# posgraph/coupe.DVSG

Hardware: AMD Instinct MI355X
Metric: stabilized frames/sec (1280x720 RGB) (higher is better)
Workload: dtype f32

## Files before the change

### coupe/dvsg_amd/_lib.py

```python
import ctypes
import os

_HERE = os.path.dirname(os.path.abspath(__file__))
LIB_PATH = os.environ.get("DVSG_AMD_LIB") or os.path.join(_HERE, "libdvsg_amd.so")
ABI_VERSION = 1

c_float_p = ctypes.POINTER(ctypes.c_float)
_vp = ctypes.c_void_p
_i = ctypes.c_int

SIGNATURES = {
    "dvsg_tps_solve_f32": [_vp, _vp, _i, _i, _i, _vp, _vp],
    "dvsg_tps_solve_checked_f32": [_vp, _vp, _i, _i, _i, _vp, _vp, _vp],
    "dvsg_tps_warp_f32": [_vp, _vp, _vp, _i, _i, _i, _i, _i, _i, _i, _vp, _vp, _vp, _vp],
    "dvsg_flow_warp_f32": [_vp, _vp, _i, _i, _i, _i, _vp, _vp],
    "dvsg_stn_sample_f32": [_vp, _vp, _vp, _i, _i, _i, _i, _i, _i, _vp, _vp],
    "dvsg_grid_affine_f32": [_vp, _vp, _i, _i, _i, _i, _i, _i, _vp, _vp, _vp, _vp],
    "dvsg_grid_projective_f32": [_vp, _vp, _i, _i, _i, _i, _i, _i, _vp, _vp, _vp, _vp],
    "dvsg_elastic_constants_f32": [_i, _vp, _vp],
    "dvsg_grid_elastic_f32": [_vp, _vp, _vp, _i, _vp, _i, _i, _i, _i, _i, _i, _vp, _vp, _vp, _vp],
    "dvsg_scale_rgb_f32": [_vp, _i, _i, _i, _i, _vp, _vp],
    "dvsg_locnet_create": [_i, ctypes.POINTER(ctypes.c_char_p), ctypes.POINTER(_vp),
                           ctypes.POINTER(_i), ctypes.POINTER(ctypes.c_int64), ctypes.POINTER(_vp)],
    "dvsg_locnet_destroy": [_vp],
    "dvsg_locnet_in_channels": [_vp],
    "dvsg_locnet_workspace_bytes": [_vp, _i, _i, _i, ctypes.POINTER(ctypes.c_size_t)],
    "dvsg_locnet_forward_f32": [_vp, _vp, _i, _i, _i, _vp, _vp, ctypes.c_size_t, _vp],
    "dvsg_locnet_forward_tap_f32": [_vp, _vp, _i, _i, _i, _i, _vp, ctypes.c_size_t,
                                    ctypes.POINTER(_i), _vp, ctypes.c_size_t, _vp],
    "dvsg_stabilize_f32": [_vp, _vp, _vp, _i, _i, _i, _vp, _vp, _vp, _vp, _vp, ctypes.c_size_t, _vp],
    "dvsg_locnet_forward_f32s": [_vp, _vp, _i, _i, _i, _vp, _vp, ctypes.c_size_t, _vp],
    "dvsg_locnet_forward_tap_f32s": [_vp, _vp, _i, _i, _i, _i, _vp, ctypes.c_size_t,
                                     ctypes.POINTER(_i), _vp, ctypes.c_size_t, _vp],
    "dvsg_stabilize_f32s": [_vp, _vp, _vp, _i, _i, _i, _vp, _vp, _vp, _vp, _vp, ctypes.c_size_t, _vp],
    "dvsg_conv_gemm_f32s": [_vp, _vp, _vp, _vp, _vp, _i, _i, _i, _i, _i, _i, _i, _i, _i, _vp, ctypes.c_size_t, _vp],
    "dvsg_locnet_forward_f32x3": [_vp, _vp, _i, _i, _i, _vp, _vp, ctypes.c_size_t, _vp],
    "dvsg_locnet_forward_tap_f32x3": [_vp, _vp, _i, _i, _i, _i, _vp, ctypes.c_size_t,
                                      ctypes.POINTER(_i), _vp, ctypes.c_size_t, _vp],
    "dvsg_stabilize_f32x3": [_vp, _vp, _vp, _i, _i, _i, _vp, _vp, _vp, _vp, _vp, ctypes.c_size_t, _vp],
    "dvsg_conv_gemm_f32x3": [_vp, _vp, _vp, _vp, _vp, _i, _i, _i, _i, _i, _i, _i, _i, _i, _vp, ctypes.c_size_t, _vp],
    "dvsg_pack_weights_f32x3": [_vp, _vp, _i, _i, _vp],
    "dvsg_conv3x3_1x1_f32x3": [_vp, _vp, _vp, _vp, _vp, _vp, _vp, _i, _i, _i, _i, _i, _i, _i, _vp],
    "dvsg_f32_to_pieces": [_vp, _vp, ctypes.c_size_t, _vp],
    "dvsg_pieces_to_f32": [_vp, _vp, ctypes.c_size_t, _vp],
    "dvsg_locnet_forward_f16": [_vp, _vp, _i, _i, _i, _vp, _vp, ctypes.c_size_t, _vp],
    "dvsg_locnet_forward_tap_f16": [_vp, _vp, _i, _i, _i, _i, _vp, ctypes.c_size_t,
                                    ctypes.POINTER(_i), _vp, ctypes.c_size_t, _vp],
    "dvsg_stabilize_f16": [_vp, _vp, _vp, _i, _i, _i, _vp, _vp, _vp, _vp, _vp, ctypes.c_size_t, _vp],
    "dvsg_conv_gemm_f16": [_vp, _vp, _vp, _vp, _vp, _i, _i, _i, _i, _i, _i, _i, _i, _i, _vp, ctypes.c_size_t, _vp],
    "dvsg_conv_gemm_f16s": [_vp, _vp, _vp, _vp, _vp, _i, _i, _i, _i, _i, _i, _i, _i, _i, _vp, ctypes.c_size_t, _vp],
    "dvsg_conv_gemm_f32": [_vp, _vp, _vp, _vp, _vp, _i, _i, _i, _i, _i, _i, _i, _i, _i, _vp, ctypes.c_size_t, _vp],
    "dvsg_conv3x3_1x1_f32": [_vp, _vp, _vp, _vp, _vp, _vp, _vp, _i, _i, _i, _i, _i, _i, _i, _vp],
    "dvsg_frames_u8_to_f32": [_vp, ctypes.c_size_t, _i, _vp, _vp],
    "dvsg_frames_resize_u8_f32": [_vp, _i, _i, _i, _i, _vp, _i, _i, _vp, _i, _i, _vp],
    "dvsg_window_gather_f32": [_vp, _i, _i, _i, _vp, _i, _i, _vp, _vp],
    "dvsg_stabilize_ring_f32": [_vp, _i, _vp, _i, _vp, _i, _i, _i, _vp, _vp, _vp, _vp, _vp, ctypes.c_size_t, _vp],
    "dvsg_stabilize_ring_u8": [_vp, _i, _vp, _i, _vp, _i, _i, _i, _vp, _vp, _vp, _vp, _vp, ctypes.c_size_t, _vp],
    "dvsg_locnet_forward_ring": [_vp, _i, _vp, _i, _i, _vp, _i, _i, _i, _i, _vp, ctypes.c_size_t, ctypes.POINTER(_i), _vp,
                                 ctypes.c_size_t, _vp],
    "dvsg_random_mask_plane_f32": [_vp, _i, _i, _i, _vp, _vp],
    "dvsg_stabilize_masked_f32": [_vp, _i, _vp, _vp, _vp, _i, _i, _i, _vp, _vp, _vp, _vp, _vp, ctypes.c_size_t, _vp],
    "dvsg_stabilize_ring_masked_f32": [_vp, _i, _vp, _i, _vp, _vp, _i, _i, _i, _vp, _vp, _vp, _vp, _vp, ctypes.c_size_t, _vp],
    "dvsg_stabilize_ring_masked_u8": [_vp, _i, _vp, _i, _vp, _vp, _i, _i, _i, _vp, _vp, _vp, _vp, _vp, ctypes.c_size_t, _vp],
    "dvsg_locnet_forward_masked": [_vp, _i, _vp, _i, _i, _vp, _vp, _i, _i, _i, _i, _vp, ctypes.c_size_t, ctypes.POINTER(_i),
                                   _vp, ctypes.c_size_t, _vp],
    "dvsg_frames_f32_to_u8": [_vp, _i, _i, _i, _i, _vp, _i, _i, _vp],
    "dvsg_frames_f64_to_u8": [_vp, _i, _i, _i, _i, _vp, _i, _i, _vp],
    "dvsg_debug_set_option": [ctypes.c_char_p, _i],
    "dvsg_debug_calibrate_f16_weights": [_vp, _vp, _i, _i, _i, _i, _vp, ctypes.c_size_t, _vp],
    "dvsg_locnet_calibrate_f16": [_vp, _vp, _i, _i, _i, _vp, ctypes.c_size_t, _vp],
    "dvsg_markers_enabled": [],
    "dvsg_prof_begin": [_i],
    "dvsg_prof_end": [ctypes.POINTER(ctypes.c_double), ctypes.POINTER(_i), ctypes.POINTER(ctypes.c_double),
                      ctypes.POINTER(ctypes.c_double)],
}
QUERIES = ("dvsg_abi_version", "dvsg_last_error_string", "dvsg_target_arch")

_lib = None


class DvsgError(RuntimeError):
    pass


def load():
    global _lib
    if _lib is not None:
        return _lib
    if not os.path.isfile(LIB_PATH):
        raise DvsgError(
            "libdvsg_amd.so not found at %s: build it with ./build.sh (hipcc --offload-arch=gfx950). "
            "coupe.dvsg_amd has no CPU or PyTorch fallback." % LIB_PATH)
    lib = ctypes.CDLL(LIB_PATH)
    lib.dvsg_abi_version.restype = ctypes.c_int
    lib.dvsg_last_error_string.restype = ctypes.c_char_p
    lib.dvsg_target_arch.restype = ctypes.c_char_p
    if lib.dvsg_abi_version() != ABI_VERSION:
        raise DvsgError("libdvsg_amd.so ABI %d != expected %d" % (lib.dvsg_abi_version(), ABI_VERSION))
    for name, argtypes in SIGNATURES.items():
        fn = getattr(lib, name)
        fn.argtypes = argtypes
        fn.restype = ctypes.c_int
    _lib = lib
    for env, opt in (("DVSG_CONV_VARIANT", b"conv_variant"), ("DVSG_FUSE_CONV", b"fuse_conv"),
                     ("DVSG_F16_SPLIT", b"f16_split"), ("DVSG_FUSE_SHORTCUT", b"fuse_shortcut"),
                     ("DVSG_CONV1_VARIANT", b"conv1_variant"), ("DVSG_F16_PAIR_MASK", b"f16_pair_mask"),
                     ("DVSG_WIDE16_PACKED", b"wide16_packed"), ("DVSG_WIDE16_AROWS", b"wide16_arows"),
                     ("DVSG_WIDE16_HREUSE", b"wide16_hreuse"), ("DVSG_FUSED_HREUSE", b"fused_hreuse"),
                     ("DVSG_CONCAT_SC", b"concat_sc"), ("DVSG_FLOW_TILED", b"flow_tiled")):
        if os.environ.get(env) and os.environ.get("DVSG_DEBUG") == "1":
            check(lib.dvsg_debug_set_option(opt, int(os.environ[env])), "dvsg_debug_set_option")
    return lib


def check(status, what):
    if status != 0:
        msg = load().dvsg_last_error_string().decode("utf-8", "replace")
        raise DvsgError("%s failed (status %d): %s" % (what, status, msg))


def call(name, *args):
    check(getattr(load(), name)(*args), name)
```

### coupe/dvsg_amd/csrc/cnn_kernels.h

```cpp
#pragma once
#include "common.h"

namespace dvsg {

enum Precision { kF32 = 0, kF16 = 1, kF32S = 2, kF32X = 3 };
inline size_t elem_size(int prec) { return prec == kF16 ? 2 : 4; }

struct ConvGemm {
  int prec;
  const void *x;
  const void *wt;
  const float *bias;
  const void *res;
  void *y;
  int B, H, W, Cin, Ho, Wo, Cout;
  int ksize, stride, pad;
  int res_H, res_W, res_stride;
  int relu;
  int ldx = 0, res_ld = 0, relu_from = -1;
  const void *wt_packed = nullptr;
  const void *wt_packed_a = nullptr;
  const void *wt_packed_h = nullptr;
  int x3 = 0;
  int wsplit = 0;
  void *splitk_scratch = nullptr;
  size_t splitk_scratch_bytes = 0;
  int *splitk_counters = nullptr;
};
constexpr int kSplitKMaxTiles = 512;
constexpr size_t kSplitKSlabBytes = (size_t)512 * 2 * 128 * 128 * 4;
int launch_conv_gemm(const ConvGemm &p, hipStream_t s);
inline size_t x3_packed_bytes(int rows, int K) { return (size_t)rows * K * 6; }
int launch_pack_x3(const float *wt, void *out, int rows, int K, hipStream_t s);
int launch_conv_wide16(const ConvGemm &p, hipStream_t s);
void set_wide16_min_tiles(int v);
size_t wide16_packed_bytes(int rows, int Cin, int ksize);
int launch_pack_wide16(const void *wt, void *out, int rows, int Cin, int ksize, int order, hipStream_t s);
void set_wide16_arows(int v);
void set_wide16_hreuse(int v);
void set_wide16_packed(int v);
int launch_zero_tickets(int *tickets, size_t n, hipStream_t s);
struct ConvFused {
  const float *x;
  const float *wt2;
  const float *bias2;
  const float *wt3;
  const float *bias3;
  const float *res;
  float *y;
  int B, H, W, Cin, Ho, Wo, Cout;
  int stride;
  int res_H, res_W, res_stride;
  const float *sc_x = nullptr;
  const float *sc_wt = nullptr;
  const float *sc_bias = nullptr;
  int sc_cin = 0;
  int pieces = 0;
  int f16 = 0;
  int x3 = 0;
};
int launch_conv3x3_1x1_x3(const ConvFused &p, hipStream_t s);
bool conv_fusable(int prec, int Cin, int Cmid, int Cout, int ksize);
int launch_conv3x3_1x1(const ConvFused &p, hipStream_t s);
void set_fuse_conv(int v);
int get_fuse_conv();
void set_fused_hreuse(int v);
void set_conv_variant(int v);
void set_conv1_variant(int v);

constexpr int kConv1Cin = 21;
constexpr int kConv1K = 7 * kConv1Cin;
constexpr int kConv1Kpad = 148;
constexpr int kConv1Ld = 150;
constexpr int kConv1LdH = 168;
constexpr int kConv1X3Ld = 88;
constexpr int kConv1X3StageElems = 3 * 64 * kConv1X3Ld;
enum Conv1SrcKind { kSrcWindow = 0, kSrcRingF32 = 1, kSrcRingU8 = 2 };
struct Conv1Src {
  const void *base;
  const int *table;
  int n_pool;
  const float *mask = nullptr;
};
int launch_conv1(int out_prec, const Conv1Src &src, int src_kind, const float *wt1, const void *wt1h, const void *wt1s,
                 const void *wt1x, const float *bias, void *y, int B, int H, int W, int Ho, int Wo, hipStream_t s);

int launch_maxpool(int prec, const void *x, void *y, int B, int H, int W, int C, int Ho, int Wo, int pad_top,
                   int pad_left, hipStream_t s);

constexpr int kPoolSplits = 8;
int launch_avgpool_partial(int prec, const void *x, float *part, int B, int HW, int C, hipStream_t s);

int launch_f16_to_f32(const void *x, float *y, size_t n, hipStream_t s);
int launch_p_to_f32(const void *x, float *y, size_t n, hipStream_t s);
int launch_f32_to_p(const float *x, void *y, size_t n, hipStream_t s);

constexpr int kDenseSplits = 8;
int launch_dense(const float *xin, int s_in, const float *bias_in, float scale_in, int lrelu_in,
                 const float *W, float *out_part, int B, int K, int N, hipStream_t s);
int launch_dense_finalize(const float *part, int s_in, float scale, const float *bias, float *out, int B,
                          int N, hipStream_t s);

}
```

### coupe/dvsg_amd/csrc/conv1_pool.hip

```cpp
#include <cstdint>
#include <type_traits>

#include "cnn_device.h"
#include "cnn_kernels.h"

namespace dvsg {
namespace {

constexpr int C1_TILE = 128;
constexpr int C1_SEG_PAD = 5488;
constexpr int C1_WELEMS = 64 * kConv1Ld;
constexpr int C1_LDC = 68;

template <int NT, int GROUPS, bool ALIGNED, bool MASKED = false>
struct Conv1Row {
  static constexpr bool kRing = false;
  typedef float floatx4_u __attribute__((ext_vector_type(4), aligned(4)));
  floatx4 nmean[GROUPS];
  long idx[GROUPS];
  unsigned col_ok, full;
  bool fast;
  struct Data {
    floatx4 reg[GROUPS];
    float m0[MASKED ? GROUPS : 1], m1[MASKED ? GROUPS : 1];
    bool row_ok;
  };
  const float *img;
  long row_elems;
  int H;
  const float *mplane;
  int mW;
  int mcol0[MASKED ? GROUPS : 1], mcol1[MASKED ? GROUPS : 1];
  unsigned m_first, m_second;

  __device__ __forceinline__ void init(const Conv1Src &src, int tid, int b, int wo0, int H_, int W, int seg_elems) {
    H = H_;
    row_elems = (long)W * kConv1Cin;
    img = static_cast<const float *>(src.base) + (long)b * H * row_elems;
    const long seg0 = (long)(2 * wo0 - 3) * kConv1Cin - 1;
    col_ok = full = 0;
    if constexpr (MASKED) {
      mplane = src.mask + (long)b * H * W;
      mW = W;
      m_first = m_second = 0;
    }
    bool mine = true;
#pragma unroll
    for (int i = 0; i < GROUPS; ++i) {
      const int e0 = 4 * (tid + NT * i);
      unsigned m = 0;
      if constexpr (MASKED) {
        const long ge0 = seg0 + e0;
        const int c0 = (int)(ge0 >= 0 ? ge0 / kConv1Cin : -((-ge0 + kConv1Cin - 1) / kConv1Cin));
        mcol0[i] = c0 < 0 ? 0 : (c0 >= W ? W - 1 : c0);
        mcol1[i] = c0 + 1 < 0 ? 0 : (c0 + 1 >= W ? W - 1 : c0 + 1);
#pragma unroll
        for (int j = 0; j < 4; ++j) {
          const long ge = ge0 + j;
          if (ge < 0 || ge >= row_elems) continue;
          const int col = (int)(ge / kConv1Cin), ch = (int)(ge - (long)col * kConv1Cin);
          if (ch >= kConv1Cin - 3) continue;
          if (col == c0) m_first |= 1u << (4 * i + j); else m_second |= 1u << (4 * i + j);
        }
      }
#pragma unroll
      for (int j = 0; j < 4; ++j) {
        const int e = e0 + j;
        const long ge = seg0 + e;
        const int g = ((e + kConv1Cin - 1) % kConv1Cin) / (kConv1Cin / 3);
        nmean[i][j] = g == 0 ? -123.68f : (g == 1 ? -116.779f : -103.939f);
        if (e < seg_elems && ge >= 0 && ge < row_elems) m |= 1u << j;
        if (e < seg_elems && !(ge >= 0 && ge < row_elems)) mine = false;
      }
      col_ok |= m << (4 * i);
      if (m == 15u) full |= 1u << i;
      idx[i] = (ALIGNED && m != 15u) ? 0 : seg0 + e0;
    }
    fast = ALIGNED && __builtin_amdgcn_ballot_w64(!mine) == 0;
  }
  __device__ __forceinline__ void load(Data &d, int hi) const {
    d.row_ok = hi >= 0 && hi < H;
    const int hc = hi < 0 ? 0 : (hi >= H ? H - 1 : hi);
    const float *xrow = img + (long)hc * row_elems;
    if constexpr (MASKED) {
      const float *mrow = mplane + (long)hc * mW;
#pragma unroll
      for (int i = 0; i < GROUPS; ++i) {
        d.m0[i] = mrow[mcol0[i]];
        d.m1[i] = mrow[mcol1[i]];
      }
    }
#pragma unroll
    for (int i = 0; i < GROUPS; ++i) {
      if constexpr (ALIGNED) {
        d.reg[i] = *reinterpret_cast<const floatx4 *>(xrow + idx[i]);
      } else if ((full >> i) & 1u) {
        d.reg[i] = *reinterpret_cast<const floatx4_u *>(xrow + idx[i]);
      } else {
#pragma unroll
        for (int j = 0; j < 4; ++j) d.reg[i][j] = ((col_ok >> (4 * i + j)) & 1u) ? xrow[idx[i] + j] : 0.f;
      }
    }
  }
  __device__ __forceinline__ floatx4 scaled(const Data &d, int i) const {
    floatx4 x = d.reg[i];
    if constexpr (MASKED) {
      floatx4 m4;
#pragma unroll
      for (int j = 0; j < 4; ++j)
        m4[j] = ((m_first >> (4 * i + j)) & 1u) ? d.m0[i] : (((m_second >> (4 * i + j)) & 1u) ? d.m1[i] : 1.0f);
      x = x * m4;
    }
    if (fast) {
      if (!d.row_ok) return floatx4{0.f, 0.f, 0.f, 0.f};
      return x * 255.0f + nmean[i];
    }
    const unsigned ok = d.row_ok ? col_ok : 0u;
    floatx4 v;
#pragma unroll
    for (int j = 0; j < 4; ++j) v[j] = ((ok >> (4 * i + j)) & 1u) ? x[j] * 255.0f + nmean[i][j] : 0.f;
    return v;
  }
};

constexpr int C1_RING_PX = 2 * (C1_TILE - 1) + 7;
constexpr int C1_RING_RG = (3 * (C1_RING_PX + 1) + 3) / 4;
constexpr int C1_RING_GROUPS = 7 * C1_RING_RG;

template <int NT, int GROUPS, typename TS, bool ALIGNED, bool MASKED = false>
struct Conv1RingRow {
  static constexpr bool kRing = true;
  static constexpr bool kU8 = sizeof(TS) == 1;
  static_assert(NT * GROUPS >= C1_RING_GROUPS, "not enough threads x groups for 7 frame runs");
  static_assert(GROUPS <= 8, "per-element masks are 32 bits wide");
  typedef float floatx4_u __attribute__((ext_vector_type(4), aligned(4)));
  floatx4 nmean[GROUPS];
  bool fast;
  long off[GROUPS];
  int l0[GROUPS];
  unsigned phase;
  unsigned col_ok, st_ok;
  unsigned no_frame;
  struct Data {
    floatx4 regf[kU8 ? 1 : GROUPS];
    unsigned regu[kU8 ? GROUPS : 1];
    float m0[MASKED ? GROUPS : 1], m1[MASKED ? GROUPS : 1];
    bool row_ok;
  };
  const TS *pool;
  long row_elems;
  int H;
  const float *mplane;
// ... 18 lines not shown
    for (int i = 0; i < GROUPS; ++i) {
      const int q = tid + NT * i;
      const int f = q / C1_RING_RG, g = q - f * C1_RING_RG;
      const bool in_range = q < C1_RING_GROUPS;
      const int fi = in_range ? src.table[b * 7 + f] : -1;
      const bool frame_ok = fi >= 0 && fi < src.n_pool;
      const long r0 = r_first + 4 * g;
      unsigned mc = 0, ms = 0;
      if constexpr (MASKED) {
        const int c0 = (int)(r0 >= 0 ? r0 / 3 : -((-r0 + 2) / 3));
        mcol0[i] = c0 < 0 ? 0 : (c0 >= W ? W - 1 : c0);
        mcol1[i] = c0 + 1 < 0 ? 0 : (c0 + 1 >= W ? W - 1 : c0 + 1);
        if (in_range && f < 6) {
#pragma unroll
          for (int j = 0; j < 4; ++j) {
            const long r = r0 + j;
            if (r < 0 || r >= row_elems) continue;
            if ((int)(r / 3) == c0) m_first |= 1u << (4 * i + j); else m_second |= 1u << (4 * i + j);
          }
        }
      }
#pragma unroll
      for (int j = 0; j < 4; ++j) {
        const int t = 4 * g + j;
        const int c = 3 * f + t % 3;
        const int grp = c / (kConv1Cin / 3);
        nmean[i][j] = grp == 0 ? -123.68f : (grp == 1 ? -116.779f : -103.939f);
        if (in_range && t >= 3 && t < 3 * (C1_RING_PX + 1)) ms |= 1u << j;
        if (in_range && r0 + j >= 0 && r0 + j < row_elems) mc |= 1u << j;
      }
      if (in_range && !frame_ok) no_frame |= 1u << i;
      if ((ms & ~mc) != 0 || (in_range && !frame_ok)) mine = false;
      const bool whole = mc == 15u;
      if (ALIGNED && !whole) mc = 0;
      col_ok |= mc << (4 * i);
      st_ok |= ms << (4 * i);
      off[i] = (ALIGNED && !whole) ? 0 : (frame_ok ? (long)fi * frame_elems : 0) + r0;
      l0[i] = 1 + kConv1Cin * ((4 * g) / 3 - 1) + 3 * f;
      phase |= (unsigned)((4 * g) % 3) << (2 * i);
    }
    fast = __builtin_amdgcn_ballot_w64(!mine) == 0;
  }
  __device__ __forceinline__ void load(Data &d, int hi) const {
    d.row_ok = hi >= 0 && hi < H;
    const int hc = hi < 0 ? 0 : (hi >= H ? H - 1 : hi);
    const long roff = (long)hc * row_elems;
    if constexpr (MASKED) {
      const float *mrow = mplane + (long)hc * mW;
#pragma unroll
      for (int i = 0; i < GROUPS; ++i) {
        d.m0[i] = mrow[mcol0[i]];
        d.m1[i] = mrow[mcol1[i]];
      }
    }
#pragma unroll
    for (int i = 0; i < GROUPS; ++i) {
      const TS *p = pool + off[i] + roff;
      if constexpr (kU8) {
        if constexpr (ALIGNED) {
          d.regu[i] = *reinterpret_cast<const unsigned *>(p);
        } else {
          unsigned w = 0;
#pragma unroll
          for (int j = 0; j < 4; ++j)
            if ((col_ok >> (4 * i + j)) & 1u) w |= (unsigned)p[j] << (8 * j);
          d.regu[i] = w;
        }
      } else {
        if constexpr (ALIGNED) {
          d.regf[i] = *reinterpret_cast<const floatx4 *>(p);
        } else if (((col_ok >> (4 * i)) & 15u) == 15u) {
          d.regf[i] = *reinterpret_cast<const floatx4_u *>(p);
        } else {
#pragma unroll
          for (int j = 0; j < 4; ++j) d.regf[i][j] = ((col_ok >> (4 * i + j)) & 1u) ? (float)p[j] : 0.f;
        }
      }
    }
  }
  template <typename PUT>
  __device__ __forceinline__ void scatter(const Data &d, PUT put) const {
    const unsigned ok = d.row_ok ? col_ok : 0u;
    const bool plain = fast && d.row_ok;
#pragma unroll
    for (int i = 0; i < GROUPS; ++i) {
      const int ph = (phase >> (2 * i)) & 3u;
      floatx4 raw4;
      if constexpr (MASKED) {
        floatx4 m4, x;
#pragma unroll
        for (int j = 0; j < 4; ++j)
          m4[j] = ((m_first >> (4 * i + j)) & 1u) ? d.m0[i] : (((m_second >> (4 * i + j)) & 1u) ? d.m1[i] : 1.0f);
        if constexpr (kU8) {
#pragma unroll
          for (int j = 0; j < 4; ++j) {
            const float v = (float)((d.regu[i] >> (8 * j)) & 255u);
            const float q = v * (1.0f / 255.0f);
            x[j] = __builtin_fmaf(__builtin_fmaf(-q, 255.0f, v), 1.0f / 255.0f, q);
          }
        } else {
          x = d.regf[i];
        }
        raw4 = (x * m4) * 255.0f;
      } else if constexpr (kU8) {
#pragma unroll
        for (int j = 0; j < 4; ++j) raw4[j] = (float)((d.regu[i] >> (8 * j)) & 255u);
      } else {
        raw4 = d.regf[i] * 255.0f;
      }
      const floatx4 sc4 = raw4 + nmean[i];
#pragma unroll
      for (int j = 0; j < 4; ++j) {
        float v;
        if (plain) {
          v = sc4[j];
        } else {
          const float raw = ((no_frame >> i) & 1u) ? 0.f : raw4[j];
          v = ((ok >> (4 * i + j)) & 1u) ? raw + nmean[i][j] : 0.f;
        }
        const int t = ph + j, step = t / 3;
        if ((st_ok >> (4 * i + j)) & 1u) put(l0[i] + kConv1Cin * step + (t - 3 * step), v);
      }
    }
  }
};

template <int NT, int GROUPS, int SRC>
struct Conv1RowSel {
  static_assert((SRC & 6) == 0, "ring sources are specialised below");
  typedef Conv1Row<NT, GROUPS, (SRC & 1) != 0, (SRC & 8) != 0> type;
};
template <int NT, int GROUPS>
struct Conv1RowSel<NT, GROUPS, 10> { typedef Conv1RingRow<NT, (C1_RING_GROUPS + NT - 1) / NT, float, false, true> type; };
template <int NT, int GROUPS>
struct Conv1RowSel<NT, GROUPS, 11> { typedef Conv1RingRow<NT, (C1_RING_GROUPS + NT - 1) / NT, float, true, true> type; };
template <int NT, int GROUPS>
struct Conv1RowSel<NT, GROUPS, 12> { typedef Conv1RingRow<NT, (C1_RING_GROUPS + NT - 1) / NT, uint8_t, false, true> type; };
template <int NT, int GROUPS>
struct Conv1RowSel<NT, GROUPS, 13> { typedef Conv1RingRow<NT, (C1_RING_GROUPS + NT - 1) / NT, uint8_t, true, true> type; };
template <int NT, int GROUPS>
struct Conv1RowSel<NT, GROUPS, 2> { typedef Conv1RingRow<NT, (C1_RING_GROUPS + NT - 1) / NT, float, false> type; };
template <int NT, int GROUPS>
struct Conv1RowSel<NT, GROUPS, 3> { typedef Conv1RingRow<NT, (C1_RING_GROUPS + NT - 1) / NT, float, true> type; };
template <int NT, int GROUPS>
struct Conv1RowSel<NT, GROUPS, 4> { typedef Conv1RingRow<NT, (C1_RING_GROUPS + NT - 1) / NT, uint8_t, false> type; };
template <int NT, int GROUPS>
struct Conv1RowSel<NT, GROUPS, 5> { typedef Conv1RingRow<NT, (C1_RING_GROUPS + NT - 1) / NT, uint8_t, true> type; };

#ifdef DVSG_STAMPS
__device__ unsigned long long g_c1_stamps[8 * 65536];
#define C1_STAMP() __builtin_amdgcn_s_memtime()
#endif

template <int NW, typename TO, int SRC>
__global__ __launch_bounds__(64 * NW) __attribute__((amdgpu_waves_per_eu(NW / 2, NW / 2)))
void conv1_kernel(const Conv1Src src, const float *__restrict__ wt1, const float *__restrict__ bias,
                  TO *__restrict__ y, int H, int W, int Ho, int Wo, int wtiles) {
  constexpr int NT = 64 * NW;
  constexpr int MI = 4 / (NW / 2);
  constexpr int IN4 = (C1_SEG_PAD / 4 + NT - 1) / NT;
  constexpr int WLOADS = (C1_WELEMS / 4 + NT - 1) / NT;
  static_assert(C1_TILE * C1_LDC <= C1_WELEMS, "epilogue tile must fit in the weight stage");
  __shared__ __attribute__((aligned(16))) float w_s[C1_WELEMS];
  __shared__ __attribute__((aligned(16))) float in_s[C1_SEG_PAD];
  const int tid = threadIdx.x;
  const int lane = tid & 63, wave = tid >> 6;
  const int wm = wave >> 1, wn = wave & 1;
  const int r = lane & 31, h = lane >> 5;

  int blk = xcd_remap(blockIdx.x, gridDim.x);
  const int wt_i = blk % wtiles;
  blk /= wtiles;
  const int ho = blk % Ho;
  const int b = blk / Ho;
  const int wo0 = wt_i * C1_TILE;

  typedef typename Conv1RowSel<NT, IN4, SRC>::type Row;
  Row row;
  row.init(src, tid, b, wo0, H, W, C1_SEG_PAD);
  if constexpr (Row::kRing) {
    for (int e = tid; e < C1_SEG_PAD; e += NT) in_s[e] = 0.f;
  }
  typename Row::Data rd;
  floatx4 w_reg[WLOADS];
  auto load_stage = [&](int kh) __attribute__((always_inline)) {
    row.load(rd, 2 * ho + kh - 3);
    const floatx4 *wsrc = reinterpret_cast<const floatx4 *>(wt1 + (size_t)kh * C1_WELEMS);
#pragma unroll
    for (int i = 0; i < WLOADS; ++i) {
      const int q = tid + NT * i;
      w_reg[i] = wsrc[q < C1_WELEMS / 4 ? q : 0];
    }
  };
  auto store_stage = [&]() __attribute__((always_inline)) {
    if constexpr (Row::kRing) {
      row.scatter(rd, [&](int e, float v) __attribute__((always_inline)) { in_s[e] = v; });
    } else {
#pragma unroll
      for (int i = 0; i < IN4; ++i) {
        const int q = tid + NT * i;
        const floatx4 v = row.scaled(rd, i);
        if (q < C1_SEG_PAD / 4) reinterpret_cast<floatx4 *>(in_s)[q] = v;
      }
    }
#pragma unroll
    for (int i = 0; i < WLOADS; ++i) {
      const int q = tid + NT * i;
      if (q < C1_WELEMS / 4) reinterpret_cast<floatx4 *>(w_s)[q] = w_reg[i];
    }
  };

  floatx16 acc[MI];
#pragma unroll
  for (int mi = 0; mi < MI; ++mi)
#pragma unroll
    for (int q = 0; q < 16; ++q) acc[mi][q] = 0.f;

#ifdef DVSG_STAMPS
  unsigned long long st[8] = {0, 0, 0, 0, 0, 0, 0, 0};
  const unsigned long long t_begin = C1_STAMP(), r_begin = __builtin_amdgcn_s_memrealtime();
#endif
  load_stage(0);
#ifdef DVSG_STAMPS
  st[0] = C1_STAMP() - t_begin;
#endif
  for (int kh = 0; kh < 7; ++kh) {
#ifdef DVSG_STAMPS
    const unsigned long long s0 = C1_STAMP();
    __syncthreads();
    const unsigned long long s1 = C1_STAMP();
    store_stage();
    const unsigned long long s2 = C1_STAMP();
    __syncthreads();
    const unsigned long long s3 = C1_STAMP();
    if (kh + 1 < 7) load_stage(kh + 1);
    const unsigned long long s4 = C1_STAMP();
    st[1] += s1 - s0;
    st[2] += s2 - s1;
    st[3] += s3 - s2;
    st[4] += s4 - s3;
#else
    __syncthreads();
    store_stage();
    __syncthreads();
    if (kh + 1 < 7) load_stage(kh + 1);
#endif
    __builtin_amdgcn_sched_barrier(0);
    const float *a0 = in_s + 2 * kConv1Cin * (wm * 32 * MI + r) + 2 * h;
    const float *bp = w_s + (wn * 32 + r) * kConv1Ld + 2 * h;
    constexpr int STEPS = kConv1Kpad / 4, PAIRS = (STEPS + 1) / 2;
    float2 va[2][2][MI], vb[2][2];
    auto read_pair = [&](int slot, int g) __attribute__((always_inline)) {
#pragma unroll
      for (int j = 0; j < 2; ++j) {
        if (2 * g + j >= STEPS) break;
#pragma unroll
        for (int mi = 0; mi < MI; ++mi)
          va[slot][j][mi] = *reinterpret_cast<const float2 *>(a0 + mi * (2 * kConv1Cin * 32) + 4 * (2 * g + j));
        vb[slot][j] = *reinterpret_cast<const float2 *>(bp + 4 * (2 * g + j));
      }
    };
    read_pair(0, 0);
#pragma unroll
    for (int g = 0; g < PAIRS; ++g) {
      if (g + 1 < PAIRS) read_pair((g + 1) & 1, g + 1);
      __builtin_amdgcn_sched_barrier(0);
#pragma unroll
      for (int j = 0; j < 2; ++j) {
        if (2 * g + j >= STEPS) break;
#pragma unroll
        for (int mi = 0; mi < MI; ++mi) acc[mi] = mfma32(va[g & 1][j][mi].x, vb[g & 1][j].x, acc[mi]);
#pragma unroll
        for (int mi = 0; mi < MI; ++mi) acc[mi] = mfma32(va[g & 1][j][mi].y, vb[g & 1][j].y, acc[mi]);
      }
      __builtin_amdgcn_sched_barrier(0);
    }
  }

#ifdef DVSG_STAMPS
  const unsigned long long t_loop_end = C1_STAMP();
#endif
  float *Cs = w_s;
  __syncthreads();
#pragma unroll
  for (int mi = 0; mi < MI; ++mi)
#pragma unroll
    for (int q = 0; q < 16; ++q)
      Cs[(wm * 32 * MI + mi * 32 + (q & 3) + 8 * (q >> 2) + 4 * h) * C1_LDC + wn * 32 + r] = acc[mi][q];
  __syncthreads();
  const int col4 = tid & 15, row0 = tid >> 4;
  const float4 b4 = *reinterpret_cast<const float4 *>(bias + 4 * col4);
  TO *yrow = y + (((size_t)b * Ho + ho) * Wo + wo0) * 64 + 4 * col4;
#pragma unroll 4
  for (int row = row0; row < C1_TILE; row += NT / 16) {
    if (wo0 + row >= Wo) break;
    float4 v = *reinterpret_cast<const float4 *>(Cs + row * C1_LDC + 4 * col4);
    v.x = fmaxf(v.x + b4.x, 0.f);
    v.y = fmaxf(v.y + b4.y, 0.f);
    v.z = fmaxf(v.z + b4.z, 0.f);
    v.w = fmaxf(v.w + b4.w, 0.f);
    store4(yrow + (size_t)row * 64, v);
  }
#ifdef DVSG_STAMPS
  if (tid == 0 && blockIdx.x < 65536) {
    unsigned long long *o = g_c1_stamps + (size_t)blockIdx.x * 8;
    const unsigned long long t_end = C1_STAMP();
    o[0] = st[0]; o[1] = st[1]; o[2] = st[2]; o[3] = st[3]; o[4] = st[4];
    o[5] = t_loop_end - t_begin;
    o[6] = t_end - t_begin;
    o[7] = __builtin_amdgcn_s_memrealtime() - r_begin;
  }
#endif
}

template <typename T>
__global__ __launch_bounds__(256) void maxpool_kernel(const T *__restrict__ x, T *__restrict__ y, int H, int W,
                                                     int C4, int Ho, int Wo, int pad_top, int pad_left,
                                                     size_t total) {
  {
    const size_t e = (size_t)xcd_remap(blockIdx.x, gridDim.x) * 256 + threadIdx.x;
    if (e >= total) return;
    const int c4 = (int)(e % C4);
    size_t t = e / C4;
    const int wo = (int)(t % Wo);
    t /= Wo;
    const int ho = (int)(t % Ho);
    const size_t b = t / Ho;
    float4 m = make_float4(-INFINITY, -INFINITY, -INFINITY, -INFINITY);
#pragma unroll
    for (int i = 0; i < 3; ++i) {
      const int hi = 2 * ho - pad_top + i;
      if (hi < 0 || hi >= H) continue;
#pragma unroll
      for (int j = 0; j < 3; ++j) {
        const int wi = 2 * wo - pad_left + j;
        if (wi < 0 || wi >= W) continue;
        const float4 v = load4(x + (((b * H + hi) * W + wi) * C4 + c4) * 4);
        m.x = fmaxf(m.x, v.x);
        m.y = fmaxf(m.y, v.y);
        m.z = fmaxf(m.z, v.z);
        m.w = fmaxf(m.w, v.w);
      }
    }
    store4(y + e * 4, m);
  }
}

__global__ __launch_bounds__(256) void maxpool_h8_kernel(const _Float16 *__restrict__ x, _Float16 *__restrict__ y, int H,
                                                         int W, int C8, int Ho, int Wo, int pad_top, int pad_left,
                                                         size_t total) {
  const size_t e = (size_t)xcd_remap(blockIdx.x, gridDim.x) * 256 + threadIdx.x;
  if (e >= total) return;
  const int c8 = (int)(e % C8);
  size_t t = e / C8;
  const int wo = (int)(t % Wo);
  t /= Wo;
  const int ho = (int)(t % Ho);
  const size_t b = t / Ho;
  halfx8 m;
#pragma unroll
  for (int q = 0; q < 8; ++q) m[q] = (_Float16)(-INFINITY);
#pragma unroll
  for (int i = 0; i < 3; ++i) {
    const int hi = 2 * ho - pad_top + i;
    if (hi < 0 || hi >= H) continue;
#pragma unroll
    for (int j = 0; j < 3; ++j) {
      const int wi = 2 * wo - pad_left + j;
      if (wi < 0 || wi >= W) continue;
      const halfx8 v = *reinterpret_cast<const halfx8 *>(x + (((b * H + hi) * W + wi) * C8 + c8) * 8);
#pragma unroll
      for (int q = 0; q < 8; ++q) m[q] = v[q] > m[q] ? v[q] : m[q];
    }
  }
  *reinterpret_cast<halfx8 *>(y + e * 8) = m;
}

constexpr int C1H_STEPS = 10;
constexpr int C1H_LD = 168;
constexpr int C1H_WBYTES = 64 * C1H_LD * 2;
constexpr int C1H_SEG = 5504;
constexpr int C1H_IN4 = (C1H_SEG / 4 + 255) / 256;

template <typename TO, int SRC>
__global__ __launch_bounds__(256) __attribute__((amdgpu_waves_per_eu(2, 2)))
void conv1_f16_kernel(const Conv1Src src, const _Float16 *__restrict__ wt1h, const float *__restrict__ bias,
                      TO *__restrict__ y, int H, int W, int Ho, int Wo, int wtiles) {
  static_assert(C1_TILE * C1_LDC * 4 <= 2 * C1H_WBYTES, "epilogue tile must fit in the weight stages");
  __shared__ __attribute__((aligned(16))) char lds[2 * C1H_WBYTES + 2 * C1H_SEG * 2];
  char *w_s = lds;
  char *in_s = lds + 2 * C1H_WBYTES;
  const int tid = threadIdx.x;
  const int lane = tid & 63, wave = tid >> 6;
  const int r = lane & 31, h = lane >> 5;

  int blk = xcd_remap(blockIdx.x, gridDim.x);
  const int wt_i = blk % wtiles;
  blk /= wtiles;
  const int ho = blk % Ho;
  const int b = blk / Ho;
  const int wo0 = wt_i * C1_TILE;

  typedef typename Conv1RowSel<256, C1H_IN4, SRC>::type Row;
  Row row;
  row.init(src, tid, b, wo0, H, W, C1H_SEG);
  if constexpr (Row::kRing) {
    for (int e = tid; e < C1H_SEG; e += 256) reinterpret_cast<unsigned *>(in_s)[e] = 0u;
    __syncthreads();
  }

  typedef const __attribute__((address_space(1))) void *gptr_t;
  typedef __attribute__((address_space(3))) void *lptr_t;
  typename Row::Data rd;
  auto load_stage = [&](int kh, int buf) __attribute__((always_inline)) {
    const char *wsrc = reinterpret_cast<const char *>(wt1h) + (size_t)kh * C1H_WBYTES;
    for (int j = wave; j < C1H_WBYTES / 1024; j += 4)
      __builtin_amdgcn_global_load_lds((gptr_t)(wsrc + j * 1024 + lane * 16), (lptr_t)(w_s + buf * C1H_WBYTES + j * 1024),
                                       16, 0, 0);
    row.load(rd, 2 * ho + kh - 3);
  };
  auto store_stage = [&](int buf) __attribute__((always_inline)) {
    typedef _Float16 half4_t __attribute__((ext_vector_type(4)));
    if constexpr (Row::kRing) {
      _Float16 *dsth = reinterpret_cast<_Float16 *>(in_s + buf * C1H_SEG * 2);
      row.scatter(rd, [&](int e, float v) __attribute__((always_inline)) { dsth[e] = (_Float16)v; });
    } else {
      half4_t *dst = reinterpret_cast<half4_t *>(in_s + buf * C1H_SEG * 2);
#pragma unroll
      for (int i = 0; i < C1H_IN4; ++i) {
        const int q = tid + 256 * i;
        const floatx4 v = row.scaled(rd, i);
        half4_t hv;
#pragma unroll
        for (int j = 0; j < 4; ++j) hv[j] = (_Float16)v[j];
        if (q < C1H_SEG / 4) dst[q] = hv;
      }
    }
  };

  floatx16 acc[2];
#pragma unroll
  for (int ni = 0; ni < 2; ++ni)
#pragma unroll
    for (int q = 0; q < 16; ++q) acc[ni][q] = 0.f;
// ... 845 lines not shown
    v.z = fmaxf(v.z + b4.z, 0.f);
    v.w = fmaxf(v.w + b4.w, 0.f);
    store4(y + (((size_t)b * Ho + ho) * Wo + wo0 + row) * 64 + 4 * col4, v);
  }
}

__global__ __launch_bounds__(256) void maxpool_p_kernel(const void *__restrict__ x, void *__restrict__ y, int H, int W,
                                                       int C4, int Ho, int Wo, int pad_top, int pad_left, size_t total) {
  const size_t e = (size_t)xcd_remap(blockIdx.x, gridDim.x) * 256 + threadIdx.x;
  if (e >= total) return;
  const int c4 = (int)(e % C4);
  size_t t = e / C4;
  const int wo = (int)(t % Wo);
  t /= Wo;
  const int ho = (int)(t % Ho);
  const size_t b = t / Ho;
  float4 m = make_float4(-INFINITY, -INFINITY, -INFINITY, -INFINITY);
#pragma unroll
  for (int i = 0; i < 3; ++i) {
    const int hi = 2 * ho - pad_top + i;
    if (hi < 0 || hi >= H) continue;
#pragma unroll
    for (int j = 0; j < 3; ++j) {
      const int wi = 2 * wo - pad_left + j;
      if (wi < 0 || wi >= W) continue;
      const float4 v = load4_p(x, (((b * H + hi) * W + wi) * C4 + c4) * 4);
      m.x = fmaxf(m.x, v.x);
      m.y = fmaxf(m.y, v.y);
      m.z = fmaxf(m.z, v.z);
      m.w = fmaxf(m.w, v.w);
    }
  }
  store4_p(y, e * 4, m);
}

int march_bands(int B, int Ho, int wtiles, int *quads_per_band) {
  const int quads = (Ho + C1M_QUAD - 1) / C1M_QUAD;
  const long cols = (long)B * wtiles;
  for (int qpb = 8; qpb >= 4; --qpb) {
    const int bands = (quads + qpb - 1) / qpb;
    if (cols * bands >= 3 * 256) {
      if (quads_per_band) *quads_per_band = qpb;
      return bands;
    }
  }
  return 0;
}

int g_conv1_variant = 0;

}

void set_conv1_variant(int v) { g_conv1_variant = v; }

int launch_conv1(int out_prec, const Conv1Src &src, int src_kind, const float *wt1, const void *wt1h, const void *wt1s,
                 const void *wt1x, const float *bias, void *y, int B, int H, int W, int Ho, int Wo, hipStream_t s) {
  const int wtiles = ceil_div(Wo, C1_TILE);
  const long blocks = (long)wtiles * Ho * B;
  DVSG_REQUIRE(blocks > 0 && blocks < (1L << 31), "conv1: grid of %ld workgroups out of range", blocks);
  DVSG_REQUIRE((long)W * kConv1Cin < (1L << 31), "conv1: input row too long");
  DVSG_REQUIRE(src_kind == kSrcWindow || (src.table && src.n_pool > 0), "conv1: a frame ring needs its index table");
  const double in_bytes = src_kind == kSrcRingU8 ? 1.0 : 4.0;
  ProfScope prof(kClsConv1, s, 2.0 * (double)B * Ho * Wo * 64 * 49 * kConv1Cin,
                 in_bytes * (double)B * H * W * kConv1Cin + (double)elem_size(out_prec) * B * Ho * Wo * 64);
  const dim3 grid((unsigned)blocks);
  const bool aligned = W % 4 == 0 && reinterpret_cast<uintptr_t>(src.base) % (src_kind == kSrcRingU8 ? 4 : 16) == 0;
  const int SRC = 2 * src_kind + (aligned ? 1 : 0) + (src.mask ? 8 : 0);
  if (out_prec == kF32S && !wt1s) return fail(DVSG_ERR_UNSUPPORTED, "conv1: the f32s precision needs the piece weights");
#define DVSG_K_F32(SRC) conv1_kernel<4, float, SRC>
#define DVSG_K_F16(SRC) conv1_f16_kernel<_Float16, (SRC) & 7>
#define DVSG_K_SPLIT(SRC) conv1_split_kernel<float, SRC>
#define DVSG_K_X3(SRC) conv1_x3_kernel<SRC>
#define DVSG_C1(KERNEL, NTHREADS, WPTR, YPTR)                                                                            \
  do {                                                                                                                   \
    switch (SRC) {                                                                                                       \
      case 0: hipLaunchKernelGGL((KERNEL(0)), grid, dim3(NTHREADS), 0, s, src, WPTR, bias, YPTR, H, W, Ho, Wo, wtiles); break; \
      case 1: hipLaunchKernelGGL((KERNEL(1)), grid, dim3(NTHREADS), 0, s, src, WPTR, bias, YPTR, H, W, Ho, Wo, wtiles); break; \
      case 2: hipLaunchKernelGGL((KERNEL(2)), grid, dim3(NTHREADS), 0, s, src, WPTR, bias, YPTR, H, W, Ho, Wo, wtiles); break; \
      case 3: hipLaunchKernelGGL((KERNEL(3)), grid, dim3(NTHREADS), 0, s, src, WPTR, bias, YPTR, H, W, Ho, Wo, wtiles); break; \
      case 4: hipLaunchKernelGGL((KERNEL(4)), grid, dim3(NTHREADS), 0, s, src, WPTR, bias, YPTR, H, W, Ho, Wo, wtiles); break; \
      case 5: hipLaunchKernelGGL((KERNEL(5)), grid, dim3(NTHREADS), 0, s, src, WPTR, bias, YPTR, H, W, Ho, Wo, wtiles); break; \
      case 8: hipLaunchKernelGGL((KERNEL(8)), grid, dim3(NTHREADS), 0, s, src, WPTR, bias, YPTR, H, W, Ho, Wo, wtiles); break; \
      case 9: hipLaunchKernelGGL((KERNEL(9)), grid, dim3(NTHREADS), 0, s, src, WPTR, bias, YPTR, H, W, Ho, Wo, wtiles); break; \
      case 10: hipLaunchKernelGGL((KERNEL(10)), grid, dim3(NTHREADS), 0, s, src, WPTR, bias, YPTR, H, W, Ho, Wo, wtiles); break; \
      case 11: hipLaunchKernelGGL((KERNEL(11)), grid, dim3(NTHREADS), 0, s, src, WPTR, bias, YPTR, H, W, Ho, Wo, wtiles); break; \
      case 12: hipLaunchKernelGGL((KERNEL(12)), grid, dim3(NTHREADS), 0, s, src, WPTR, bias, YPTR, H, W, Ho, Wo, wtiles); break; \
      default: hipLaunchKernelGGL((KERNEL(13)), grid, dim3(NTHREADS), 0, s, src, WPTR, bias, YPTR, H, W, Ho, Wo, wtiles); break; \
    }                                                                                                                    \
  } while (0)
  if (out_prec == kF32X && !wt1x) return fail(DVSG_ERR_UNSUPPORTED, "conv1: the f32x3 precision needs the bfloat16 piece weights");
  if (out_prec == kF32X) {
    DVSG_C1(DVSG_K_X3, 256, static_cast<const unsigned short *>(wt1x), static_cast<float *>(y));
  } else if (out_prec == kF32S) {
    DVSG_C1(DVSG_K_SPLIT, 256, static_cast<const _Float16 *>(wt1s), static_cast<float *>(y));
  } else if (out_prec == kF16 && wt1h && g_conv1_variant == 3 && !src.mask) {
    DVSG_C1(DVSG_K_F16, 256, static_cast<const _Float16 *>(wt1h), static_cast<_Float16 *>(y));
  } else if (out_prec == kF16 && wt1h && g_conv1_variant != 2 && g_conv1_variant != 4 && !src.mask &&
             (g_conv1_variant == 5 || march_bands(B, Ho, wtiles, nullptr) > 0)) {
    int qpb = 0;
    int bands = march_bands(B, Ho, wtiles, &qpb);
    if (g_conv1_variant == 5) {
      qpb = 3;
      bands = ((Ho + C1M_QUAD - 1) / C1M_QUAD + qpb - 1) / qpb;
    }
    const dim3 mgrid((unsigned)((long)wtiles * bands * B));
    const _Float16 *wp = static_cast<const _Float16 *>(wt1h);
    _Float16 *yp = static_cast<_Float16 *>(y);
    switch (SRC) {
      case 0: hipLaunchKernelGGL((conv1_f16_march_kernel<0>), mgrid, dim3(512), 0, s, src, wp, bias, yp, H, W, Ho, Wo, wtiles, bands, qpb); break;
      case 1: hipLaunchKernelGGL((conv1_f16_march_kernel<1>), mgrid, dim3(512), 0, s, src, wp, bias, yp, H, W, Ho, Wo, wtiles, bands, qpb); break;
      case 2: hipLaunchKernelGGL((conv1_f16_march_kernel<2>), mgrid, dim3(512), 0, s, src, wp, bias, yp, H, W, Ho, Wo, wtiles, bands, qpb); break;
      case 3: hipLaunchKernelGGL((conv1_f16_march_kernel<3>), mgrid, dim3(512), 0, s, src, wp, bias, yp, H, W, Ho, Wo, wtiles, bands, qpb); break;
      case 4: hipLaunchKernelGGL((conv1_f16_march_kernel<4>), mgrid, dim3(512), 0, s, src, wp, bias, yp, H, W, Ho, Wo, wtiles, bands, qpb); break;
      default: hipLaunchKernelGGL((conv1_f16_march_kernel<5>), mgrid, dim3(512), 0, s, src, wp, bias, yp, H, W, Ho, Wo, wtiles, bands, qpb); break;
    }
  } else if (out_prec == kF16 && wt1h && g_conv1_variant != 2) {
    const int hpairs = (Ho + 1) / 2;
    const long pblocks = (long)wtiles * hpairs * B;
    const dim3 pgrid((unsigned)pblocks);
    const _Float16 *wp = static_cast<const _Float16 *>(wt1h);
    _Float16 *yp = static_cast<_Float16 *>(y);
    switch (SRC) {
      case 0: hipLaunchKernelGGL((conv1_f16_pair_kernel<_Float16, 0>), pgrid, dim3(256), 0, s, src, wp, bias, yp, H, W, Ho, Wo, wtiles, hpairs); break;
      case 1: hipLaunchKernelGGL((conv1_f16_pair_kernel<_Float16, 1>), pgrid, dim3(256), 0, s, src, wp, bias, yp, H, W, Ho, Wo, wtiles, hpairs); break;
      case 2: hipLaunchKernelGGL((conv1_f16_pair_kernel<_Float16, 2>), pgrid, dim3(256), 0, s, src, wp, bias, yp, H, W, Ho, Wo, wtiles, hpairs); break;
      case 3: hipLaunchKernelGGL((conv1_f16_pair_kernel<_Float16, 3>), pgrid, dim3(256), 0, s, src, wp, bias, yp, H, W, Ho, Wo, wtiles, hpairs); break;
      case 4: hipLaunchKernelGGL((conv1_f16_pair_kernel<_Float16, 4>), pgrid, dim3(256), 0, s, src, wp, bias, yp, H, W, Ho, Wo, wtiles, hpairs); break;
      case 5: hipLaunchKernelGGL((conv1_f16_pair_kernel<_Float16, 5>), pgrid, dim3(256), 0, s, src, wp, bias, yp, H, W, Ho, Wo, wtiles, hpairs); break;
      case 8: hipLaunchKernelGGL((conv1_f16_pair_kernel<_Float16, 8>), pgrid, dim3(256), 0, s, src, wp, bias, yp, H, W, Ho, Wo, wtiles, hpairs); break;
      case 9: hipLaunchKernelGGL((conv1_f16_pair_kernel<_Float16, 9>), pgrid, dim3(256), 0, s, src, wp, bias, yp, H, W, Ho, Wo, wtiles, hpairs); break;
      case 10: hipLaunchKernelGGL((conv1_f16_pair_kernel<_Float16, 10>), pgrid, dim3(256), 0, s, src, wp, bias, yp, H, W, Ho, Wo, wtiles, hpairs); break;
      case 11: hipLaunchKernelGGL((conv1_f16_pair_kernel<_Float16, 11>), pgrid, dim3(256), 0, s, src, wp, bias, yp, H, W, Ho, Wo, wtiles, hpairs); break;
      case 12: hipLaunchKernelGGL((conv1_f16_pair_kernel<_Float16, 12>), pgrid, dim3(256), 0, s, src, wp, bias, yp, H, W, Ho, Wo, wtiles, hpairs); break;
      default: hipLaunchKernelGGL((conv1_f16_pair_kernel<_Float16, 13>), pgrid, dim3(256), 0, s, src, wp, bias, yp, H, W, Ho, Wo, wtiles, hpairs); break;
    }
  } else if (out_prec == kF16) {
    DVSG_REQUIRE(src_kind == kSrcWindow && !src.mask, "conv1: conv1_variant 2 takes an unmasked window tensor");
    hipLaunchKernelGGL((conv1_kernel<4, _Float16, 0>), grid, dim3(256), 0, s, src, wt1, bias, static_cast<_Float16 *>(y), H, W,
                       Ho, Wo, wtiles);
  } else if (g_conv1_variant != 0 && src_kind == kSrcWindow && !src.mask) {
    hipLaunchKernelGGL((conv1_kernel<8, float, 0>), grid, dim3(512), 0, s, src, wt1, bias, static_cast<float *>(y), H, W, Ho,
                       Wo, wtiles);
  } else {
    DVSG_C1(DVSG_K_F32, 256, wt1, static_cast<float *>(y));
  }
#undef DVSG_C1
#undef DVSG_K_F32
#undef DVSG_K_F16
#undef DVSG_K_SPLIT
#undef DVSG_K_X3
  return check_launch("conv1_kernel");
}

#ifdef DVSG_STAMPS
extern "C" int dvsg_debug_read_conv1_stamps(void *host, size_t bytes) {
  return hipMemcpyFromSymbol(host, HIP_SYMBOL(g_c1_stamps), bytes) == hipSuccess ? 0 : -3;
}
#endif

int launch_maxpool(int prec, const void *x, void *y, int B, int H, int W, int C, int Ho, int Wo, int pad_top,
                   int pad_left, hipStream_t s) {
  DVSG_REQUIRE(C % 4 == 0 && (prec != kF32S || C % 32 == 0), "maxpool: C=%d must be a multiple of 4 (32 in the f32s format)", C);
  const size_t total = (size_t)B * Ho * Wo * (C / 4);
  const size_t want = (total + 255) / 256;
  DVSG_REQUIRE(want < (1u << 31), "maxpool: %zu blocks do not fit a grid", want);
  const int blocks = (int)want;
  ProfScope prof(kClsMaxpool, s, 0.0, (double)elem_size(prec) * C * ((double)B * H * W + (double)B * Ho * Wo));
  if (prec == kF32S)
    hipLaunchKernelGGL(maxpool_p_kernel, dim3(blocks), dim3(256), 0, s, x, y, H, W, C / 4, Ho, Wo, pad_top, pad_left, total);
  else if (prec == kF16 && C % 8 == 0) {
    const size_t total8 = total / 2;
    hipLaunchKernelGGL(maxpool_h8_kernel, dim3((unsigned)((total8 + 255) / 256)), dim3(256), 0, s, static_cast<const _Float16 *>(x),
                       static_cast<_Float16 *>(y), H, W, C / 8, Ho, Wo, pad_top, pad_left, total8);
  } else if (prec == kF16)
    hipLaunchKernelGGL(maxpool_kernel<_Float16>, dim3(blocks), dim3(256), 0, s, static_cast<const _Float16 *>(x),
                       static_cast<_Float16 *>(y), H, W, C / 4, Ho, Wo, pad_top, pad_left, total);
  else
    hipLaunchKernelGGL(maxpool_kernel<float>, dim3(blocks), dim3(256), 0, s, static_cast<const float *>(x),
                       static_cast<float *>(y), H, W, C / 4, Ho, Wo, pad_top, pad_left, total);
  return check_launch("maxpool_kernel");
}

}
```

### coupe/dvsg_amd/csrc/conv_fused.hip

```cpp
#include <algorithm>

#include "cnn_device.h"
#include "cnn_kernels.h"

#include <type_traits>

namespace dvsg {
namespace {

constexpr int BM = 128;
constexpr int ROWB = 128;
constexpr int CMID = 64;

__device__ const floatx4 g_zero16f = {0.f, 0.f, 0.f, 0.f};

struct ConvFusedDev {
  const float *x;
  const float *wt2;
  const float *bias2;
  const float *wt3;
  const float *bias3;
  const float *res;
  const float *wts;
  const float *biass;
// ... 161 lines not shown
  floatx16 &acc1 = acc1v[0];
#pragma unroll
  for (int q = 0; q < 16; ++q) acc1[q] = 0.f;
  auto compute_stage = [&](int buf) __attribute__((always_inline)) {
    const char *a_base = As + (buf * BM + wm * 32 + r) * ROWB;
    const char *b_base = Bs + (buf * CMID + wn * 32 + r) * ROWB;
    stage_mma<PS, 1>(a_base, b_base, sw, h, acc1v);
  };
  auto w3_issue = [&](int half, int s2) __attribute__((always_inline)) {
#pragma unroll
    for (int i = 0; i < 2; ++i) {
      const int row = 8 * (wave + NW * i) + lrow8;
      const float *src = p.wt3 + (size_t)(128 * half + row) * CMID + 32 * s2 + 4 * (lpos ^ ((row >> 1) & 7));
      __builtin_amdgcn_global_load_lds((gptr_t)src, (lptr_t)(lds + (s2 == 0 ? 49152 : 32768) + 8 * (wave + NW * i) * ROWB),
                                       16, 0, 0);
    }
  };
  issue_stage(0);
  issue_stage(1);
  asm volatile("s_waitcnt vmcnt(%0)" ::"n"(AG + 1) : "memory");
  __builtin_amdgcn_s_barrier();
  asm volatile("" ::: "memory");
  __builtin_amdgcn_sched_barrier(0);
  compute_stage(0);
  __builtin_amdgcn_sched_barrier(0);
  for (int kt = 1; kt < KT - 1; ++kt) {
    __syncthreads();
    issue_stage((kt + 1) & 1);
    __builtin_amdgcn_sched_barrier(0);
    compute_stage(kt & 1);
    __builtin_amdgcn_sched_barrier(0);
  }
  __syncthreads();
  w3_issue(0, 0);
  __builtin_amdgcn_sched_barrier(0);
  compute_stage((KT - 1) & 1);

  const float bmid = p.bias2[32 * wn + r];
  __syncthreads();
#pragma unroll
  for (int q = 0; q < 16; ++q) {
    const int R = wm * 32 + (q & 3) + 8 * (q >> 2) + 4 * h;
    const float v = fmaxf(acc1[q] + bmid, 0.f);
    if (PS) {
      const _Float16 hi = (_Float16)v, lo = (_Float16)(v - (float)hi);
      char *row = lds + (wn * BM + R) * ROWB + 2 * (r & 7);
      *reinterpret_cast<_Float16 *>(row + 16 * ((r >> 3) ^ ((R >> 1) & 7))) = hi;
      *reinterpret_cast<_Float16 *>(row + 16 * ((4 + (r >> 3)) ^ ((R >> 1) & 7))) = lo;
    } else {
      *reinterpret_cast<float *>(lds + (wn * BM + R) * ROWB + 16 * ((r >> 2) ^ ((R >> 1) & 7)) + 4 * (r & 3)) = v;
    }
  }
  w3_issue(0, 1);

  float *Cs = reinterpret_cast<float *>(lds + 32768);
  const int col4 = tid & 31, row0 = tid >> 5;
  auto lds_barrier = [&]() __attribute__((always_inline)) {
    asm volatile("s_waitcnt lgkmcnt(0)" ::: "memory");
    __builtin_amdgcn_s_barrier();
    asm volatile("" ::: "memory");
  };
  auto compute2 = [&](int s2, floatx16 (&acc2)[2]) __attribute__((always_inline)) {
    const char *a_base = lds + (s2 * BM + wm * 32 + r) * ROWB;
    const char *b_base = lds + (s2 == 0 ? 49152 : 32768) + (wn * 64 + r) * ROWB;
    stage_mma<PS, 2>(a_base, b_base, sw, h, acc2);
  };
  const int nhalves = p.Cout / 128;
  auto do_half = [&](int half, floatx16 (&acc2)[2]) __attribute__((always_inline)) {
    asm volatile("s_waitcnt vmcnt(2) lgkmcnt(0)" ::: "memory");
    __builtin_amdgcn_s_barrier();
    asm volatile("" ::: "memory");
    compute2(0, acc2);
    __syncthreads();
    compute2(1, acc2);
    const int n = 128 * half + 4 * col4;
    float4 bias4 = *reinterpret_cast<const float4 *>(p.bias3 + n);
    if (RES == 3) {
      const float4 bs = *reinterpret_cast<const float4 *>(p.biass + n);
      bias4.x += bs.x; bias4.y += bs.y; bias4.z += bs.z; bias4.w += bs.w;
    }
#pragma unroll
    for (int rho = 0; rho < 2; ++rho) {
      float4 rv[4];
      if (RES != 3) {
#pragma unroll
        for (int i = 0; i < 4; ++i) {
          const int mr = m0 + 64 * rho + row0 + 16 * i;
          const int m = mr < p.M ? mr : p.M - 1;
          size_t roff;
          if (RES == 1) {
            roff = (size_t)m * p.Cout + n;
          } else {
            const int wo = m % p.Wo;
            const int t = m / p.Wo;
            const int ho = t % p.Ho;
            const int b = t / p.Ho;
            roff = (((size_t)b * p.res_H + (size_t)ho * p.res_stride) * p.res_W + (size_t)wo * p.res_stride) * p.Cout + n;
          }
          rv[i] = PS ? load4_p_pair(p.res, roff, col4 & 1) : load4(p.res + roff);
        }
      }
      lds_barrier();
      if ((wm >> 1) == rho) {
#pragma unroll
        for (int ni = 0; ni < 2; ++ni)
#pragma unroll
          for (int q = 0; q < 16; ++q)
            Cs[((wm & 1) * 32 + (q & 3) + 8 * (q >> 2) + 4 * h) * 128 + wn * 64 + ni * 32 + r] = acc2[ni][q];
      }
      lds_barrier();
#pragma unroll
      for (int i = 0; i < 4; ++i) {
        const int row = row0 + 16 * i;
        const int m = m0 + 64 * rho + row;
        if (m < p.M) {
          float4 v = *reinterpret_cast<const float4 *>(Cs + row * 128 + 4 * col4);
          if (RES == 3) {
            v.x = fmaxf(v.x + bias4.x, 0.f);
            v.y = fmaxf(v.y + bias4.y, 0.f);
            v.z = fmaxf(v.z + bias4.z, 0.f);
            v.w = fmaxf(v.w + bias4.w, 0.f);
          } else {
            v.x = fmaxf(v.x + bias4.x + rv[i].x, 0.f);
            v.y = fmaxf(v.y + bias4.y + rv[i].y, 0.f);
            v.z = fmaxf(v.z + bias4.z + rv[i].z, 0.f);
            v.w = fmaxf(v.w + bias4.w + rv[i].w, 0.f);
          }
          if (PS) store4_p_pair(p.y, (size_t)m * p.Cout + n, v, col4 & 1, true);
          else store4(p.y + (size_t)m * p.Cout + n, v);
        }
      }
    }
    if (half + 1 < nhalves) {
      lds_barrier();
      w3_issue(half + 1, 0);
      w3_issue(half + 1, 1);
    }
  };
  if (RES == 3) {
    do_half(0, acc_sc[0]);
    do_half(1, acc_sc[1]);
  } else {
    for (int half = 0; half < nhalves; ++half) {
      floatx16 acc2[2];
#pragma unroll
      for (int ni = 0; ni < 2; ++ni)
#pragma unroll
        for (int q = 0; q < 16; ++q) acc2[ni][q] = 0.f;
      do_half(half, acc2);
    }
  }
}

struct ConvFusedF16Dev {
  const _Float16 *x;
  const _Float16 *wt2;
  const float *bias2;
  const _Float16 *wt3;
  const float *bias3;
  const _Float16 *res;
  const _Float16 *wts;
  const float *biass;
  _Float16 *y;
  int H, W, Cin, Ho, Wo, Cout;
  int stride;
  int res_H, res_W, res_stride;
  int M, mtiles;
};

template <int RES>
__global__ __launch_bounds__(512) __attribute__((amdgpu_waves_per_eu(4, 4)))
void conv3x3_1x1_f16_kernel(ConvFusedF16Dev p) {
  constexpr int NW = 8;
  constexpr float kLoScale = 1.0f / 2048.0f;
  __shared__ __attribute__((aligned(16))) char lds[65536];
  char *As = lds;
  char *Bs = lds + 32768;
  const int tid = threadIdx.x;
  const int lane = tid & 63, wave = tid >> 6;
  const int wm = wave >> 1, wn = wave & 1;
  const int r = lane & 31, h = lane >> 5;
  const int lrow8 = lane >> 3, lpos = lane & 7;
  const int sw = (r >> 1) & 7;
  const int K1 = 9 * p.Cin;
  const int KT = K1 / 64;

  typedef const __attribute__((address_space(1))) void *gptr_t;
  typedef __attribute__((address_space(3))) void *lptr_t;

  const int m0 = xcd_remap(blockIdx.x, p.mtiles) * BM;

  long a_off[2];
  unsigned a_mask[2];
  const _Float16 *wsrc[2];
#pragma unroll
  for (int i = 0; i < 2; ++i) {
    const int row = 8 * (wave + NW * i) + lrow8;
    const int chunk = lpos ^ ((row >> 1) & 7);
    const int m = m0 + row;
    const int mm = m < p.M ? m : 0;
    const int wo = mm % p.Wo;
    const int t = mm / p.Wo;
    const int ho = t % p.Ho;
    const int b = t / p.Ho;
    const int hi0 = ho * p.stride - 1, wi0 = wo * p.stride - 1;
    a_off[i] = (((long)b * p.H + hi0) * p.W + wi0) * p.Cin + 8 * chunk;
    unsigned mk = 0;
    if (m < p.M) {
#pragma unroll
      for (int q = 0; q < 3; ++q) {
        if (hi0 + q >= 0 && hi0 + q < p.H) mk |= 1u << q;
        if (wi0 + q >= 0 && wi0 + q < p.W) mk |= 16u << q;
      }
    }
    a_mask[i] = mk;
    wsrc[i] = p.wt2 + (size_t)row * K1 + 8 * chunk;
  }
  int s_kh = 0, s_kw = 0, s_c0 = 0;
  auto issue_stage = [&](int buf) __attribute__((always_inline)) {
    const _Float16 *xa = p.x + ((long)s_kh * p.W + s_kw) * p.Cin + s_c0;
    const int wk = (s_kh * 3 + s_kw) * p.Cin + s_c0;
#pragma unroll
    for (int i = 0; i < 2; ++i) {
      const bool ok = ((a_mask[i] >> s_kh) & (a_mask[i] >> (4 + s_kw)) & 1u) != 0;
      const void *src = ok ? static_cast<const void *>(xa + a_off[i]) : static_cast<const void *>(&g_zero16f);
      __builtin_amdgcn_global_load_lds((gptr_t)src, (lptr_t)(As + (buf * BM + 8 * (wave + NW * i)) * ROWB), 16, 0, 0);
    }
#pragma unroll
    for (int i = 0; i < 2; ++i)
      __builtin_amdgcn_global_load_lds((gptr_t)(wsrc[i] + wk), (lptr_t)(Bs + (buf * 128 + 8 * (wave + NW * i)) * ROWB), 16, 0, 0);
    if (++s_kw == 3) {
      s_kw = 0;
      if (++s_kh == 3) {
        s_kh = 0;
        s_c0 += 64;
      }
    }
  };
  floatx16 acc_hi, acc_lo;
#pragma unroll
  for (int q = 0; q < 16; ++q) acc_hi[q] = acc_lo[q] = 0.f;
  auto mma_stage = [&](const char *a_row, const char *b_row) __attribute__((always_inline)) {
#pragma unroll
    for (int kb = 0; kb < 4; ++kb) {
      const int co = 16 * ((2 * kb + h) ^ sw);
      const halfx8 a = *reinterpret_cast<const halfx8 *>(a_row + co);
      const halfx8 bh = *reinterpret_cast<const halfx8 *>(b_row + co);
      const halfx8 bl = *reinterpret_cast<const halfx8 *>(b_row + 64 * ROWB + co);
      acc_hi = __builtin_amdgcn_mfma_f32_32x32x16_f16(a, bh, acc_hi, 0, 0, 0);
      acc_lo = __builtin_amdgcn_mfma_f32_32x32x16_f16(a, bl, acc_lo, 0, 0, 0);
    }
  };
  auto compute_stage = [&](int buf) __attribute__((always_inline)) {
    mma_stage(As + (buf * BM + wm * 32 + r) * ROWB, Bs + (buf * 128 + wn * 32 + r) * ROWB);
  };
  auto issue_rows = [&](const _Float16 *src, size_t row_elems, int dst, bool by_pixel) __attribute__((always_inline)) {
#pragma unroll
    for (int i = 0; i < 2; ++i) {
      const int row = 8 * (wave + NW * i) + lrow8;
      size_t rr = row;
      if (by_pixel) rr = m0 + row < p.M ? m0 + row : p.M - 1;
      __builtin_amdgcn_global_load_lds((gptr_t)(src + rr * row_elems + 8 * (lpos ^ ((row >> 1) & 7))),
                                       (lptr_t)(lds + dst + 8 * (wave + NW * i) * ROWB), 16, 0, 0);
    }
  };
  issue_stage(0);
  issue_stage(1);
  asm volatile("s_waitcnt vmcnt(4)" ::: "memory");
  __builtin_amdgcn_s_barrier();
  asm volatile("" ::: "memory");
  __builtin_amdgcn_sched_barrier(0);
  compute_stage(0);
  __builtin_amdgcn_sched_barrier(0);
  for (int kt = 1; kt < KT - 1; ++kt) {
    __syncthreads();
    issue_stage((kt + 1) & 1);
    __builtin_amdgcn_sched_barrier(0);
    compute_stage(kt & 1);
    __builtin_amdgcn_sched_barrier(0);
  }
  __syncthreads();
  const int last = (KT - 1) & 1;
  if (RES == 3) {
    issue_rows(p.res, 64, last == 0 ? 16384 : 0, true);
    issue_rows(p.wts, 64, last == 0 ? 49152 : 32768, false);
  }
  __builtin_amdgcn_sched_barrier(0);
  compute_stage(last);

  const float bmid = p.bias2[32 * wn + r];
  __syncthreads();
  const int T2 = last == 0 ? 0 : 16384, SX = last == 0 ? 16384 : 0;
  const int W3 = last == 0 ? 32768 : 49152, WS = last == 0 ? 49152 : 32768;
  issue_rows(p.wt3, 64, W3, false);
#pragma unroll
  for (int q = 0; q < 16; ++q) {
    const int R = wm * 32 + (q & 3) + 8 * (q >> 2) + 4 * h;
    const int k2 = 32 * wn + r;
    const float v = fmaxf(acc_hi[q] + acc_lo[q] * kLoScale + bmid, 0.f);
    *reinterpret_cast<_Float16 *>(lds + T2 + R * ROWB + 16 * ((k2 >> 3) ^ ((R >> 1) & 7)) + 2 * (k2 & 7)) = (_Float16)v;
  }

  float *Cs = reinterpret_cast<float *>(lds + 32768);
  const int col4 = tid & 15, row0 = tid >> 4;
  const int ngroups = p.Cout / 64;
  for (int g = 0; g < ngroups; ++g) {
// ... 158 lines not shown
      const halfx8 bh = *reinterpret_cast<const halfx8 *>(b_row + 16 * ((2 * kb + h) ^ swb));
      const halfx8 bl = *reinterpret_cast<const halfx8 *>(b_row + 64 * ROWB + 16 * ((2 * kb + h) ^ swb));
      acc_hi = __builtin_amdgcn_mfma_f32_32x32x16_f16(a, bh, acc_hi, 0, 0, 0);
      acc_lo = __builtin_amdgcn_mfma_f32_32x32x16_f16(a, bl, acc_lo, 0, 0, 0);
    }
  };

  issue_a(0, A0);
  issue_q(0);
  issue_q(1);
  auto tap_stage = [&](auto T) __attribute__((always_inline)) {
    constexpr int t = decltype(T)::value;
    constexpr int kh = t / 3, kw = t % 3;
    if (t == 1 || t == 4 || (RES == 3 && t == 7)) asm volatile("s_waitcnt vmcnt(4) lgkmcnt(0)" ::: "memory");
    else asm volatile("s_waitcnt vmcnt(2) lgkmcnt(0)" ::: "memory");
    __builtin_amdgcn_s_barrier();
    asm volatile("" ::: "memory");
    if (kw == 0 && kh < 2) issue_a(kh + 1, (kh + 1) & 1 ? A1 : A0);
    if (RES == 3 && t == 6) {
#pragma unroll
      for (int i = 0; i < 2; ++i) {
        const int row = 8 * (wave + NW * i) + lrow8;
        const int mr = m0 + row;
        const int m = mr < 0 ? 0 : (mr < p.M ? mr : p.M - 1);
        __builtin_amdgcn_global_load_lds((gptr_t)(p.res + (size_t)m * CSC + 8 * (lpos ^ ((row >> 1) & 7))),
                                         (lptr_t)(lds + A1 + 8 * (wave + NW * i) * ROWB), 16, 0, 0);
      }
    }
    issue_q(t + 2);
    __builtin_amdgcn_sched_barrier(0);
    mma_tap(kh & 1 ? A1 : A0, kw, t % 3);
    __builtin_amdgcn_sched_barrier(0);
  };
  tap_stage(std::integral_constant<int, 0>{});
  tap_stage(std::integral_constant<int, 1>{});
  tap_stage(std::integral_constant<int, 2>{});
  tap_stage(std::integral_constant<int, 3>{});
  tap_stage(std::integral_constant<int, 4>{});
  tap_stage(std::integral_constant<int, 5>{});
  tap_stage(std::integral_constant<int, 6>{});
  tap_stage(std::integral_constant<int, 7>{});
  tap_stage(std::integral_constant<int, 8>{});

  const float bmid = p.bias2[32 * wn + r];
  asm volatile("s_waitcnt lgkmcnt(0)" ::: "memory");
  __builtin_amdgcn_s_barrier();
  asm volatile("" ::: "memory");
#pragma unroll
  for (int q = 0; q < 16; ++q) {
    const int R = wm * 32 + (q & 3) + 8 * (q >> 2) + 4 * h;
    const int k2 = 32 * wn + r;
    const float v = fmaxf(acc_hi[q] + acc_lo[q] * kLoScale + bmid, 0.f);
    *reinterpret_cast<_Float16 *>(lds + A0 + R * ROWB + 16 * ((k2 >> 3) ^ ((R >> 1) & 7)) + 2 * (k2 & 7)) = (_Float16)v;
  }

  float *Cs = reinterpret_cast<float *>(lds + (RES == 1 ? A1 : RING + 2 * SLOT));
  const int col4 = tid & 15, row0 = tid >> 4;
  const int ngroups = p.Cout / 64;
  for (int g = 0; g < ngroups; ++g) {
    const int n = 64 * g + 4 * col4;
    float4 bias4 = *reinterpret_cast<const float4 *>(p.bias3 + n);
    if (RES == 3) {
      const float4 bs = *reinterpret_cast<const float4 *>(p.biass + n);
      bias4.x += bs.x; bias4.y += bs.y; bias4.z += bs.z; bias4.w += bs.w;
    }
    float4 rv[2][2];
    if (RES == 1) {
#pragma unroll
      for (int rho = 0; rho < 2; ++rho)
#pragma unroll
        for (int i = 0; i < 2; ++i) {
          const int mr = m0 + 64 * rho + row0 + 32 * i;
          const int m = mr < 0 ? 0 : (mr < p.M ? mr : p.M - 1);
          rv[rho][i] = load4(p.res + (size_t)m * p.Cout + n);
        }
      asm volatile("s_waitcnt vmcnt(4) lgkmcnt(0)" ::: "memory");
    } else {
      asm volatile("s_waitcnt vmcnt(0) lgkmcnt(0)" ::: "memory");
    }
    __builtin_amdgcn_s_barrier();
    asm volatile("" ::: "memory");
#pragma unroll
    for (int q = 0; q < 16; ++q) acc_hi[q] = acc_lo[q] = 0.f;
    {
      const int slot = RES == 1 ? (g & 1) : 0;
      const char *a_row = lds + A0 + (wm * 32 + r) * ROWB;
      const char *b_row = lds + RING + slot * SLOT + (wn * 32 + r) * ROWB;
      const int sw = (r >> 1) & 7;
#pragma unroll
      for (int kb = 0; kb < 4; ++kb) {
        const int co = 16 * ((2 * kb + h) ^ sw);
        const halfx8 a = *reinterpret_cast<const halfx8 *>(a_row + co);
        acc_hi = __builtin_amdgcn_mfma_f32_32x32x16_f16(a, *reinterpret_cast<const halfx8 *>(b_row + co), acc_hi, 0, 0, 0);
        acc_lo = __builtin_amdgcn_mfma_f32_32x32x16_f16(a, *reinterpret_cast<const halfx8 *>(b_row + 64 * ROWB + co), acc_lo, 0, 0, 0);
      }
      if (RES == 3) {
        const char *x_row = lds + A1 + (wm * 32 + r) * ROWB;
        const char *s_row = lds + RING + SLOT + (wn * 32 + r) * ROWB;
#pragma unroll
        for (int kb = 0; kb < 4; ++kb) {
          const int co = 16 * ((2 * kb + h) ^ sw);
          const halfx8 a = *reinterpret_cast<const halfx8 *>(x_row + co);
          acc_hi = __builtin_amdgcn_mfma_f32_32x32x16_f16(a, *reinterpret_cast<const halfx8 *>(s_row + co), acc_hi, 0, 0, 0);
          acc_lo = __builtin_amdgcn_mfma_f32_32x32x16_f16(a, *reinterpret_cast<const halfx8 *>(s_row + 64 * ROWB + co), acc_lo, 0, 0, 0);
        }
      }
    }
    asm volatile("s_waitcnt lgkmcnt(0)" ::: "memory");
    __builtin_amdgcn_s_barrier();
    asm volatile("" ::: "memory");
    if (RES == 1) {
      if (g + 2 < ngroups) issue_w(p.wt3 + (size_t)(g + 2) * 128 * 64, 64, g & 1);
    } else if (g + 1 < ngroups) {
      issue_w(p.wt3 + (size_t)(g + 1) * 128 * 64, 64, 0);
      issue_w(p.wts + (size_t)(g + 1) * 128 * 64, 64, 1);
    }
#pragma unroll
    for (int rho = 0; rho < 2; ++rho) {
      if (rho == 1) {
        asm volatile("s_waitcnt lgkmcnt(0)" ::: "memory");
        __builtin_amdgcn_s_barrier();
        asm volatile("" ::: "memory");
      }
      if ((wm >> 1) == rho) {
#pragma unroll
        for (int q = 0; q < 16; ++q)
          Cs[((wm & 1) * 32 + (q & 3) + 8 * (q >> 2) + 4 * h) * 64 + wn * 32 + r] = acc_hi[q] + acc_lo[q] * kLoScale;
      }
      asm volatile("s_waitcnt lgkmcnt(0)" ::: "memory");
      __builtin_amdgcn_s_barrier();
      asm volatile("" ::: "memory");
#pragma unroll
      for (int i = 0; i < 2; ++i) {
        const int row = row0 + 32 * i;
        const int prow = 64 * rho + row;
        const int m = m0 + prow;
        if (prow >= 1 && prow <= FHM && m < p.M) {
          float4 o = *reinterpret_cast<const float4 *>(Cs + row * 64 + 4 * col4);
          o.x += bias4.x; o.y += bias4.y; o.z += bias4.z; o.w += bias4.w;
          if (RES == 1) {
            o.x += rv[rho][i].x; o.y += rv[rho][i].y; o.z += rv[rho][i].z; o.w += rv[rho][i].w;
          }
          o.x = fmaxf(o.x, 0.f); o.y = fmaxf(o.y, 0.f); o.z = fmaxf(o.z, 0.f); o.w = fmaxf(o.w, 0.f);
          store4(p.y + (size_t)m * p.Cout + n, o);
        }
      }
    }
  }
}

int g_fused_hreuse = 1;

int g_fuse_conv = 1;

}

void set_fuse_conv(int v) { g_fuse_conv = v; }
int get_fuse_conv() { return g_fuse_conv; }
void set_fused_hreuse(int v) { g_fused_hreuse = v; }
bool conv_fusable(int prec, int Cin, int Cmid, int Cout, int ksize) {
  if (prec == kF16) return g_fuse_conv != 0 && ksize == 3 && Cmid == CMID && Cin % 64 == 0 && Cout % 64 == 0;
  return g_fuse_conv != 0 && (prec == kF32 || prec == kF32S) && ksize == 3 && Cmid == CMID && Cin % 32 == 0 && Cin >= 64 && Cout % 128 == 0;
}

static int launch_conv3x3_1x1_f16(const ConvFused &p, hipStream_t s) {
  DVSG_REQUIRE(p.Cin % 64 == 0 && p.Cin >= 64 && p.Cout % 64 == 0, "conv3x3_1x1 (float16): Cin=%d and Cout=%d must be multiples of 64",
               p.Cin, p.Cout);
  const bool sc = p.sc_x != nullptr;
  DVSG_REQUIRE(p.res || sc, "conv3x3_1x1: the unit output needs its residual");
  DVSG_REQUIRE(!sc || (p.sc_wt && p.sc_bias && p.sc_cin == CSC && p.stride == 1),
               "conv3x3_1x1 (float16): fused shortcut needs %d input channels and stride 1 (got %d, %d)", CSC, p.sc_cin, p.stride);
  const long M = (long)p.B * p.Ho * p.Wo;
  DVSG_REQUIRE(M > 0 && M < (1L << 31) - BM, "conv3x3_1x1: M=%ld out of range", M);
  ConvFusedF16Dev d;
  d.x = reinterpret_cast<const _Float16 *>(p.x);
  d.wt2 = reinterpret_cast<const _Float16 *>(p.wt2); d.bias2 = p.bias2;
  d.wt3 = reinterpret_cast<const _Float16 *>(p.wt3); d.bias3 = p.bias3;
  d.res = reinterpret_cast<const _Float16 *>(sc ? p.sc_x : p.res);
  d.wts = reinterpret_cast<const _Float16 *>(p.sc_wt); d.biass = p.sc_bias;
  d.y = reinterpret_cast<_Float16 *>(p.y);
  d.H = p.H; d.W = p.W; d.Cin = p.Cin; d.Ho = p.Ho; d.Wo = p.Wo; d.Cout = p.Cout;
  d.stride = p.stride;
  d.res_H = p.res_H; d.res_W = p.res_W; d.res_stride = p.res_stride;
  d.M = (int)M;
  d.mtiles = (int)((M + BM - 1) / BM);
  const int res = sc ? 3 : (p.res_stride == 1 && p.res_H == p.Ho && p.res_W == p.Wo ? 1 : 2);
  ProfScope prof(kClsFused, s,
                 2.0 * (double)M * CMID * (9.0 * p.Cin) + 2.0 * (double)M * p.Cout * CMID + (sc ? 2.0 * (double)M * p.Cout * CSC : 0.0),
                 2.0 * ((double)p.B * p.H * p.W * p.Cin + 2.0 * CMID * 9 * p.Cin + 2.0 * p.Cout * CMID +
                        (sc ? (double)M * CSC + 2.0 * p.Cout * CSC + (double)M * p.Cout : 2.0 * (double)M * p.Cout)));
  if (g_fused_hreuse && p.stride == 1 && p.Cin == 64 && p.Cout >= 128 && p.H == p.Ho && p.W == p.Wo && (res == 1 || res == 3)) {
    d.mtiles = (int)((M + FHM - 1) / FHM);
    const dim3 gridh(d.mtiles), blockh(512);
    if (res == 1) hipLaunchKernelGGL((conv3x3_1x1_f16h_kernel<1>), gridh, blockh, 0, s, d);
    else hipLaunchKernelGGL((conv3x3_1x1_f16h_kernel<3>), gridh, blockh, 0, s, d);
    return check_launch("conv3x3_1x1_f16h_kernel");
  }
  const dim3 grid(d.mtiles), block(512);
  if (res == 1) hipLaunchKernelGGL((conv3x3_1x1_f16_kernel<1>), grid, block, 0, s, d);
  else if (res == 2) hipLaunchKernelGGL((conv3x3_1x1_f16_kernel<2>), grid, block, 0, s, d);
  else hipLaunchKernelGGL((conv3x3_1x1_f16_kernel<3>), grid, block, 0, s, d);
  return check_launch("conv3x3_1x1_f16_kernel");
}

int launch_conv3x3_1x1(const ConvFused &p, hipStream_t s) {
  if (p.f16) return launch_conv3x3_1x1_f16(p, s);
  if (p.x3) return launch_conv3x3_1x1_x3(p, s);
  DVSG_REQUIRE(p.Cin % 32 == 0 && p.Cin >= 64 && p.Cout % 128 == 0, "conv3x3_1x1: Cin=%d must be a multiple of 32 (>= 64), Cout=%d of 128",
               p.Cin, p.Cout);
  const bool sc = p.sc_x != nullptr;
  DVSG_REQUIRE(p.res || sc, "conv3x3_1x1: the unit output needs its residual");
  DVSG_REQUIRE(!sc || (p.sc_wt && p.sc_bias && p.sc_cin == CSC && p.Cout == 256 && p.stride == 1),
               "conv3x3_1x1: fused shortcut needs %d input channels, 256 output channels and stride 1 (got %d, %d, %d)",
               CSC, p.sc_cin, p.Cout, p.stride);
  const long M = (long)p.B * p.Ho * p.Wo;
  DVSG_REQUIRE(M > 0 && M < (1L << 31) - BM, "conv3x3_1x1: M=%ld out of range", M);
  ConvFusedDev d;
  d.x = p.x; d.wt2 = p.wt2; d.bias2 = p.bias2; d.wt3 = p.wt3; d.bias3 = p.bias3; d.y = p.y;
  d.res = sc ? p.sc_x : p.res; d.wts = p.sc_wt; d.biass = p.sc_bias;
  d.H = p.H; d.W = p.W; d.Cin = p.Cin; d.Ho = p.Ho; d.Wo = p.Wo; d.Cout = p.Cout;
  d.stride = p.stride;
  d.res_H = p.res_H; d.res_W = p.res_W; d.res_stride = p.res_stride;
  d.M = (int)M;
  d.mtiles = (int)((M + BM - 1) / BM);
  const int res = sc ? 3 : (p.res_stride == 1 && p.res_H == p.Ho && p.res_W == p.Wo ? 1 : 2);
  ProfScope prof(kClsFused, s,
                 2.0 * (double)M * CMID * (9.0 * p.Cin) + 2.0 * (double)M * p.Cout * CMID + (sc ? 2.0 * (double)M * p.Cout * CSC : 0.0),
                 4.0 * ((double)p.B * p.H * p.W * p.Cin + (double)CMID * 9 * p.Cin + (double)p.Cout * CMID +
                        (sc ? (double)M * CSC + (double)p.Cout * CSC + (double)M * p.Cout : 2.0 * (double)M * p.Cout)));
  const dim3 grid(d.mtiles), block(512);
  if (p.pieces) {
    if (res == 1) hipLaunchKernelGGL((conv3x3_1x1_kernel<1, true>), grid, block, 0, s, d);
    else if (res == 2) hipLaunchKernelGGL((conv3x3_1x1_kernel<2, true>), grid, block, 0, s, d);
    else hipLaunchKernelGGL((conv3x3_1x1_kernel<3, true>), grid, block, 0, s, d);
  } else {
    if (res == 1) hipLaunchKernelGGL((conv3x3_1x1_kernel<1>), grid, block, 0, s, d);
    else if (res == 2) hipLaunchKernelGGL((conv3x3_1x1_kernel<2>), grid, block, 0, s, d);
    else hipLaunchKernelGGL((conv3x3_1x1_kernel<3>), grid, block, 0, s, d);
  }
  return check_launch("conv3x3_1x1_kernel");
}

}
```

### coupe/dvsg_amd/csrc/locnet.hip

```cpp
#include <cmath>
#include <cstring>
#include <map>
#include <string>
#include <vector>

#include "cnn_kernels.h"

namespace dvsg {
namespace {

constexpr float kBnEps = 1e-5f;
const char *kPrefix = "stabNet/localizationNet/";

struct HostArray {
  const float *data;
  int nd;
  int64_t dims[4];
  size_t size() const {
    size_t n = 1;
    for (int i = 0; i < nd; ++i) n *= (size_t)dims[i];
    return n;
  }
};

// ... 128 lines not shown
  const HostArray *w;
  if (int rc = find(m, scope + "/weights", {L->ksize, L->ksize, L->cin, L->cout}, &w)) return rc;
  std::vector<float> scale, shift;
  if (int rc = bn_fold(m, scope, L->cout, &scale, &shift)) return rc;
  const int K = L->ksize * L->ksize * L->cin;
  std::vector<float> wt((size_t)L->cout * K);
  for (int k = 0; k < K; ++k)
    for (int n = 0; n < L->cout; ++n) wt[(size_t)n * K + k] = w->data[(size_t)k * L->cout + n] * scale[n];
  std::vector<_Float16> wt16(wt.size());
  for (size_t i = 0; i < wt.size(); ++i) wt16[i] = (_Float16)wt[i];
  std::vector<_Float16> wt16s(2 * wt.size());
  for (int n = 0; n < L->cout; ++n)
    for (int k = 0; k < K; ++k) {
      const float w32 = wt[(size_t)n * K + k];
      const _Float16 hi = (_Float16)w32;
      const _Float16 lo = (_Float16)((w32 - (float)hi) * 2048.0f);
      const size_t row = (size_t)(n / 64) * 128 + n % 64;
      wt16s[row * K + k] = hi;
      wt16s[(row + 64) * K + k] = lo;
    }
  std::vector<_Float16> wt32s(2 * wt.size());
  for (int n = 0; n < L->cout; ++n)
    for (int k = 0; k < K; ++k) {
      const float w32 = wt[(size_t)n * K + k];
      const _Float16 hi = (_Float16)w32;
      const size_t base = ((size_t)n * (K / 32) + k / 32) * 64;
      wt32s[base + k % 32] = hi;
      wt32s[base + 32 + k % 32] = (_Float16)(w32 - (float)hi);
    }
  if (int rc = upload(net, wt, &L->wt)) return rc;
  if (int rc = upload(net, wt16, &L->wt16)) return rc;
  if (int rc = upload(net, wt16s, &L->wt16s)) return rc;
  if (L->cin % 64 == 0 && L->cout % 64 == 0) {
    auto pack = [&](int order, _Float16 **out) -> int {
      void *pk = nullptr;
      DVSG_HIP(hipMalloc(&pk, wide16_packed_bytes(2 * L->cout, L->cin, L->ksize)));
      net->allocs.push_back(pk);
      if (int rc = launch_pack_wide16(L->wt16s, pk, 2 * L->cout, L->cin, L->ksize, order, nullptr)) return rc;
      *out = static_cast<_Float16 *>(pk);
      return DVSG_OK;
    };
    if (int rc = pack(0, &L->wt16p)) return rc;
    if (L->ksize == 1) {
      L->wt16pa = L->wt16p;
    } else {
      if (int rc = pack(1, &L->wt16pa)) return rc;
      if (int rc = pack(2, &L->wt16ph)) return rc;
    }
    DVSG_HIP(hipStreamSynchronize(nullptr));
  }
  if (int rc = pack_plain(net, L)) return rc;
  if (int rc = upload(net, wt32s, &L->wt32s)) return rc;
  if (K % 32 == 0 && L->cout % 64 == 0) {
    void *pk = nullptr;
    DVSG_HIP(hipMalloc(&pk, x3_packed_bytes(L->cout, K)));
    net->allocs.push_back(pk);
    if (int rc = launch_pack_x3(L->wt, pk, L->cout, K, nullptr)) return rc;
    DVSG_HIP(hipStreamSynchronize(nullptr));
    L->wt3x = static_cast<unsigned short *>(pk);
  }
  return upload(net, shift, &L->bias);
}

int make_conv1(dvsg_locnet *net, const ArrayMap &m, const std::string &scope, ConvLayer *L) {
  const HostArray *w;
  if (int rc = find(m, scope + "/weights", {7, 7, L->cin, 64}, &w)) return rc;
  std::vector<float> scale, shift;
  if (int rc = bn_fold(m, scope, 64, &scale, &shift)) return rc;
  const int cin = L->cin, G = cin / 3;
  std::vector<float> wt((size_t)7 * 64 * kConv1Ld, 0.f);
  for (int kh = 0; kh < 7; ++kh)
    for (int kw = 0; kw < 7; ++kw)
      for (int c = 0; c < cin; ++c) {
        const int cs = (2 - c / G) * G + c % G;
        for (int n = 0; n < 64; ++n)
          wt[((size_t)kh * 64 + n) * kConv1Ld + 1 + kw * cin + c] =
              w->data[(((size_t)kh * 7 + kw) * cin + cs) * 64 + n] * scale[n];
      }
  std::vector<_Float16> wth((size_t)7 * 64 * kConv1LdH, (_Float16)0.f);
  for (int kh = 0; kh < 7; ++kh)
    for (int n = 0; n < 64; ++n)
      for (int k = 0; k < kConv1K; ++k)
        wth[((size_t)kh * 64 + n) * kConv1LdH + k + 1] = (_Float16)wt[((size_t)kh * 64 + n) * kConv1Ld + k + 1];
  std::vector<_Float16> wts((size_t)7 * 2 * 64 * kConv1LdH, (_Float16)0.f);
  for (int kh = 0; kh < 7; ++kh)
    for (int n = 0; n < 64; ++n)
      for (int k = 0; k < kConv1K; ++k) {
        const float w32 = wt[((size_t)kh * 64 + n) * kConv1Ld + k + 1];
        const _Float16 hi = (_Float16)w32;
        wts[(((size_t)kh * 2 + 0) * 64 + n) * kConv1LdH + k + 1] = hi;
        wts[(((size_t)kh * 2 + 1) * 64 + n) * kConv1LdH + k + 1] = (_Float16)((w32 - (float)hi) * 2048.0f);
      }
  auto bf16_rn = [](float f) -> unsigned short {
    uint32_t u;
    std::memcpy(&u, &f, 4);
    u += 0x7fffu + ((u >> 16) & 1u);
    return (unsigned short)(u >> 16);
  };
  auto bf16_val = [](unsigned short hbits) -> float {
    const uint32_t u = (uint32_t)hbits << 16;
    float f;
    std::memcpy(&f, &u, 4);
    return f;
  };
  std::vector<unsigned short> wtx((size_t)14 * kConv1X3StageElems, 0);
  for (int kh = 0; kh < 7; ++kh)
    for (int n = 0; n < 64; ++n)
      for (int pos = 1; pos <= kConv1K; ++pos) {
        const float w32 = wt[((size_t)kh * 64 + n) * kConv1Ld + pos];
        const unsigned short p1 = bf16_rn(w32);
        const float r1 = w32 - bf16_val(p1);
        const unsigned short p2 = bf16_rn(r1);
        const unsigned short p3 = bf16_rn(r1 - bf16_val(p2));
        const size_t base = (size_t)(2 * kh + pos / 80) * kConv1X3StageElems + (size_t)n * kConv1X3Ld + pos % 80;
        wtx[base] = p1;
        wtx[base + 64 * kConv1X3Ld] = p2;
        wtx[base + 2 * 64 * kConv1X3Ld] = p3;
      }
  if (int rc = upload(net, wt, &L->wt)) return rc;
  if (int rc = upload(net, wth, &L->wt16)) return rc;
  if (int rc = upload(net, wts, &L->wt32s)) return rc;
  if (int rc = upload(net, wtx, &L->wt3x)) return rc;
  return upload(net, shift, &L->bias);
}

struct Dims {
  int H1, W1, Hp, Wp, pad_top, pad_left;
};

Dims root_dims(int H, int W) {
  Dims d;
  d.H1 = (H - 1) / 2 + 1;
  d.W1 = (W - 1) / 2 + 1;
  d.Hp = (d.H1 + 1) / 2;
  d.Wp = (d.W1 + 1) / 2;
  const int pth = std::max((d.Hp - 1) * 2 + 3 - d.H1, 0), ptw = std::max((d.Wp - 1) * 2 + 3 - d.W1, 0);
  d.pad_top = pth / 2;
  d.pad_left = ptw / 2;
  return d;
}

size_t align256(size_t n) { return (n + 255) & ~(size_t)255; }

int g_f16_split = 1;
int g_f16_pair_mask = 0xFFFF;
enum LayerKind { kKindC1 = 0, kKindC2 = 1, kKindC3 = 2, kKindSc = 3 };
inline bool f16_pairs(const dvsg_locnet *net, int block, int kind) {
  return g_f16_split && ((g_f16_pair_mask & net->f16_pair_mask) >> (4 * kind + block)) & 1;
}
int g_fuse_shortcut = 1;
int g_x3_conv1 = 1;
int g_x3_fuse = 3;
int g_concat_sc = 1;

struct Workspace {
  char *bufA, *bufB, *bufS, *r1, *r2;
  float *pool_part, *dpart0, *dpart1, *T, *Ft;
  char *splitk_slabs;
  int *splitk_counters;
  size_t total;
};
constexpr int kMaxConvLaunches = 64;

Workspace plan(char *base, int B, int H, int W) {
  const Dims d = root_dims(H, W);
  size_t big_el = std::max((size_t)d.H1 * d.W1 * 64, (size_t)d.Hp * d.Wp * 64);
  size_t small_el = 0;
  {
    int h = d.Hp, w = d.Wp;
    for (const BlockSpec &bs : kBlocks)
      for (int u = 1; u <= bs.units; ++u) {
        const int stride = u == bs.units ? bs.last_stride : 1;
        const int ho = (h - 1) / stride + 1, wo = (w - 1) / stride + 1;
        small_el = std::max(small_el, (size_t)h * w * bs.base);
        big_el = std::max(big_el, (size_t)ho * wo * bs.base * 4);
        if (u == 1) big_el = std::max(big_el, (size_t)h * w * bs.base * 5);
        h = ho; w = wo;
      }
  }
  const size_t big = align256((size_t)B * big_el * sizeof(float));
  const size_t small = align256((size_t)B * small_el * sizeof(float));
  Workspace w;
  size_t off = 0;
  auto take = [&](size_t bytes) {
    char *p = base + off;
    off += align256(bytes);
    return p;
  };
  w.bufA = take(big);
  w.bufB = take(big);
  w.bufS = take(big);
  w.r1 = take(small);
  w.r2 = take(small);
  w.pool_part = reinterpret_cast<float *>(take((size_t)kPoolSplits * B * 2048 * sizeof(float)));
  w.dpart0 = reinterpret_cast<float *>(take((size_t)kDenseSplits * 16 * 2048 * sizeof(float)));
  w.dpart1 = reinterpret_cast<float *>(take((size_t)kDenseSplits * 16 * 2048 * sizeof(float)));
  w.T = reinterpret_cast<float *>(take((size_t)B * 2 * 28 * sizeof(float)));
  w.Ft = reinterpret_cast<float *>(take((size_t)B * 50 * sizeof(float)));
  w.splitk_slabs = take(kSplitKSlabBytes);
  w.splitk_counters = reinterpret_cast<int *>(take((size_t)kMaxConvLaunches * kSplitKMaxTiles * sizeof(int)));
  w.total = off;
  return w;
}

int run_conv(int prec, const ConvLayer &L, bool pairs, const void *x, int B, int H, int W, void *y, int Ho, int Wo,
             const void *res, int res_H, int res_W, int res_stride, bool relu, const Workspace &ws, int *launch_idx,
             hipStream_t s, int ldx = 0, int res_ld = 0, int relu_from = -1) {
  ConvGemm p;
  p.ldx = ldx; p.res_ld = res_ld; p.relu_from = relu_from;
  p.splitk_scratch = ws.splitk_slabs;
  p.splitk_scratch_bytes = kSplitKSlabBytes;
  p.splitk_counters = ws.splitk_counters + (size_t)((*launch_idx)++ % kMaxConvLaunches) * kSplitKMaxTiles;
  p.prec = prec == kF32S || prec == kF32X ? kF32 : prec;
  p.wsplit = prec == kF32S || (prec == kF16 && pairs);
  p.x3 = prec == kF32X;
  if (prec == kF32X && !L.wt3x)
    return fail(DVSG_ERR_UNSUPPORTED, "f32x3: layer %d -> %d (k = %d) has no packed bfloat16 pieces (K %% 32, Cout %% 64)", L.cin, L.cout, L.ksize);
  p.x = x; p.wt = L.weights(prec, p.wsplit != 0); p.bias = L.bias; p.res = res; p.y = y;
  if (prec == kF16 && pairs) {
    p.wt_packed = L.wt16p;
    p.wt_packed_a = L.wt16pa;
    p.wt_packed_h = L.wt16ph;
  } else if (prec == kF16) {
    p.wt_packed = L.wt16q;
    p.wt_packed_a = L.wt16qa;
    p.wt_packed_h = L.wt16qh;
  }
  p.B = B; p.H = H; p.W = W; p.Cin = L.cin; p.Ho = Ho; p.Wo = Wo; p.Cout = L.cout;
  p.ksize = L.ksize; p.stride = L.stride; p.pad = L.ksize == 3 ? 1 : 0;
  p.res_H = res_H; p.res_W = res_W; p.res_stride = res_stride;
  p.relu = relu;
  return launch_conv_gemm(p, s);
}

struct Calib {
  double *sums = nullptr;
  float *part = nullptr;
  double rows[48] = {0};
  bool on = false;
} g_calib;

constexpr int kCalibBlocks = 512;
__global__ __launch_bounds__(256) void channel_sum_kernel(const float *__restrict__ x, long M, int C, long chunk,
                                                         float *__restrict__ part) {
  const long r0 = (long)blockIdx.x * chunk, r1 = r0 + chunk < M ? r0 + chunk : M;
  for (int c = threadIdx.x; c < C; c += 256) {
    float acc = 0.f;
    for (long r = r0; r < r1; ++r) acc += x[r * C + c];
    part[(size_t)blockIdx.x * 2048 + c] = acc;
  }
}
__global__ __launch_bounds__(256) void channel_sum_final(const float *__restrict__ part, int nblk, int C, double *__restrict__ out) {
  const int c = blockIdx.x * 256 + threadIdx.x;
  if (c >= C) return;
  double acc = out[c];
  for (int b = 0; b < nblk; ++b) acc += (double)part[(size_t)b * 2048 + c];
  out[c] = acc;
}

int calib_record(int slot, const void *x, long M, int C, hipStream_t s) {
  if (!g_calib.on) return DVSG_OK;
  const long chunk = (M + kCalibBlocks - 1) / kCalibBlocks;
  const int nblk = (int)((M + chunk - 1) / chunk);
  hipLaunchKernelGGL(channel_sum_kernel, dim3(nblk), dim3(256), 0, s, static_cast<const float *>(x), M, C, chunk, g_calib.part);
  hipLaunchKernelGGL(channel_sum_final, dim3((C + 255) / 256), dim3(256), 0, s, g_calib.part, nblk, C,
                     g_calib.sums + (size_t)slot * 2048);
  g_calib.rows[slot] += (double)M;
  return check_launch("channel_sum_kernel");
}

int forward(const dvsg_locnet *net, int prec, const Conv1Src &src, int src_kind, int B, int H, int W, float *F_t, int stop_stage,
            float *act_out, size_t act_out_bytes, int *act_dims, void *workspace, size_t workspace_bytes,
            hipStream_t s) {
  DVSG_REQUIRE(net && src.base && workspace, "locnet forward: NULL pointer");
  DVSG_REQUIRE(B > 0 && H >= 1 && W >= 1, "locnet forward: bad shape B=%d H=%d W=%d", B, H, W);
  DVSG_REQUIRE(((uintptr_t)workspace & 255) == 0, "locnet forward: workspace must be 256-byte aligned");
  const Workspace ws = plan(static_cast<char *>(workspace), B, H, W);
  if (ws.total > workspace_bytes)
    return fail(DVSG_ERR_WORKSPACE, "locnet forward: workspace %zu bytes < required %zu", workspace_bytes, ws.total);
  const Dims d = root_dims(H, W);
  const int gprec = prec;
  if (prec == kF32X) prec = kF32;

  auto tap = [&](int stage, const void *act, int h, int w, int c) -> int {
    if (stage != stop_stage) return 0;
    const size_t n = (size_t)B * h * w * c;
    if (n * sizeof(float) > act_out_bytes)
      return fail(DVSG_ERR_INVALID_ARG, "tap buffer %zu bytes < %zu", act_out_bytes, n * sizeof(float));
    if (prec == kF16) {
      if (int rc = launch_f16_to_f32(act, act_out, n, s)) return rc;
    } else if (prec == kF32S) {
      if (int rc = launch_p_to_f32(act, act_out, n, s)) return rc;
    } else {
      DVSG_HIP(hipMemcpyAsync(act_out, act, n * sizeof(float), hipMemcpyDeviceToDevice, s));
    }
    act_dims[0] = h; act_dims[1] = w; act_dims[2] = c;
    return 1;
  };
#define DVSG_TAP(stage, act, h, w, c)          \
  do {                                         \
    int t_ = tap(stage, act, h, w, c);         \
    if (t_ < 0) return t_;                     \
    if (t_ > 0) return DVSG_OK;                \
  } while (0)
#define DVSG_RUN(call)             \
  do {                             \
    if (int rc_ = (call)) return rc_; \
  } while (0)

  DVSG_RUN(launch_zero_tickets(ws.splitk_counters, (size_t)kMaxConvLaunches * kSplitKMaxTiles, s));
  int launch_idx = 0;
  {
  MarkerRange mr("dvsg/conv1");
  DVSG_RUN(launch_conv1(gprec == kF32X && g_x3_conv1 ? kF32X : prec, src, src_kind, net->conv1.wt, net->conv1.wt16, net->conv1.wt32s,
                        net->conv1.wt3x, net->conv1.bias, ws.bufA, B, H, W, d.H1, d.W1, s));
  }
  DVSG_TAP(0, ws.bufA, d.H1, d.W1, 64);
  {
  MarkerRange mr("dvsg/pool1");
  DVSG_RUN(launch_maxpool(prec, ws.bufA, ws.bufB, B, d.H1, d.W1, 64, d.Hp, d.Wp, d.pad_top, d.pad_left, s));
  }
  DVSG_TAP(1, ws.bufB, d.Hp, d.Wp, 64);

  char *X = ws.bufB, *Y = ws.bufA;
  int h = d.Hp, w = d.Wp;
  int stage = 2;
  int unit_in_block = 0, last_block = -1;
  for (const Unit &u : net->units) {
    unit_in_block = u.block == last_block ? unit_in_block + 1 : 1;
    last_block = u.block;
    char range_name[40];
    std::snprintf(range_name, sizeof(range_name), "dvsg/block%d/unit_%d", u.block + 1, unit_in_block);
    MarkerRange mr(range_name);
    const int ho = (h - 1) / u.stride + 1, wo = (w - 1) / u.stride + 1;
    const void *res = X;
    int res_h = h, res_w = w, res_stride = u.stride;
    const int calib_slot = 3 * (stage - 2);
    DVSG_RUN(calib_record(calib_slot, X, (long)B * h * w, u.c1.cin, s));
    const bool x3_fused = gprec == kF32X && g_x3_fuse == 3;
    const bool x3_unfused = gprec == kF32X && (g_x3_fuse == 0 || (g_x3_fuse == 1 && !u.has_shortcut));
    const bool fuse23 = !x3_unfused && conv_fusable(prec, u.c2.cin, u.c2.cout, u.c3.cout, u.c2.ksize) &&
                        (prec != kF16 || (f16_pairs(net, u.block, kKindC2) && f16_pairs(net, u.block, kKindC3) &&
                                          (!u.has_shortcut || f16_pairs(net, u.block, kKindSc))));
    const bool fuse_sc = fuse23 && !x3_fused && u.has_shortcut && u.stride == 1 && u.shortcut.cin == 64 && u.shortcut.cout == 256 &&
                         g_fuse_shortcut;
    const bool cat = u.has_shortcut && !fuse_sc && u.has_cat && prec != kF16 && g_concat_sc && !g_calib.on && u.stride == 1;
    const void *c2_in = ws.r1;
    int c2_ldx = 0, res_ld = 0;
    if (cat) {
      DVSG_RUN(run_conv(gprec, u.cat, false, X, B, h, w, ws.bufS, h, w, nullptr, 0, 0, 1, false, ws, &launch_idx, s, 0, 0,
                        u.shortcut.cout));
      res = ws.bufS;
      res_h = ho; res_w = wo; res_stride = 1;
      res_ld = u.cat.cout;
      c2_in = ws.bufS + (size_t)u.shortcut.cout * sizeof(float);
      c2_ldx = u.cat.cout;
    } else {
    if (u.has_shortcut && !fuse_sc) {
      DVSG_RUN(run_conv(gprec, u.shortcut, f16_pairs(net, u.block, kKindSc), X, B, h, w, ws.bufS, ho, wo, nullptr, 0, 0, 1, false, ws,
                        &launch_idx, s));
      res = ws.bufS;
      res_h = ho; res_w = wo; res_stride = 1;
    }
    DVSG_RUN(run_conv(gprec, u.c1, f16_pairs(net, u.block, kKindC1), X, B, h, w, ws.r1, h, w, nullptr, 0, 0, 1, true, ws, &launch_idx, s));
    }
    if (fuse23) {
      ConvFused f;
      const bool pcs = prec == kF32S;
      auto wts_of = [&](const ConvLayer &L) {
        if (x3_fused) return reinterpret_cast<const float *>(L.wt3x);
        return pcs ? reinterpret_cast<const float *>(L.wt32s) : prec == kF16 ? reinterpret_cast<const float *>(L.wt16s) : L.wt;
      };
      f.pieces = pcs;
      f.f16 = prec == kF16;
      f.x3 = x3_fused;
      f.x = reinterpret_cast<const float *>(ws.r1); f.wt2 = wts_of(u.c2); f.bias2 = u.c2.bias; f.wt3 = wts_of(u.c3); f.bias3 = u.c3.bias;
      f.res = static_cast<const float *>(res); f.y = reinterpret_cast<float *>(Y);
      f.B = B; f.H = h; f.W = w; f.Cin = u.c2.cin; f.Ho = ho; f.Wo = wo; f.Cout = u.c3.cout;
      f.stride = u.c2.stride; f.res_H = res_h; f.res_W = res_w; f.res_stride = res_stride;
      if (fuse_sc) {
        f.res = nullptr;
        f.sc_x = reinterpret_cast<const float *>(X); f.sc_wt = wts_of(u.shortcut); f.sc_bias = u.shortcut.bias;
        f.sc_cin = u.shortcut.cin;
      }
      DVSG_RUN(launch_conv3x3_1x1(f, s));
    } else {
      DVSG_RUN(calib_record(calib_slot + 1, ws.r1, (long)B * h * w, u.c2.cin, s));
      DVSG_RUN(run_conv(gprec, u.c2, f16_pairs(net, u.block, kKindC2), c2_in, B, h, w, ws.r2, ho, wo, nullptr, 0, 0, 1, true, ws,
                        &launch_idx, s, c2_ldx));
      DVSG_RUN(calib_record(calib_slot + 2, ws.r2, (long)B * ho * wo, u.c3.cin, s));
      DVSG_RUN(run_conv(gprec, u.c3, f16_pairs(net, u.block, kKindC3), ws.r2, B, ho, wo, Y, ho, wo, res, res_h, res_w, res_stride, true,
                        ws, &launch_idx, s, 0, res_ld));
    }
    h = ho; w = wo;
    DVSG_TAP(stage, Y, h, w, u.depth);
    ++stage;
    char *tmp = X; X = Y; Y = tmp;
  }

  MarkerRange mr_head("dvsg/head");
  DVSG_RUN(launch_avgpool_partial(prec, X, ws.pool_part, B, h * w, 2048, s));
  const float inv_hw = 1.0f / (float)(h * w);
  if (stop_stage == 18) {
    const size_t bytes = (size_t)B * 2048 * sizeof(float);
    if (bytes > act_out_bytes) return fail(DVSG_ERR_INVALID_ARG, "tap buffer %zu bytes < %zu", act_out_bytes, bytes);
    DVSG_RUN(launch_dense_finalize(ws.pool_part, kPoolSplits, inv_hw, nullptr, act_out, B, 2048, s));
    act_dims[0] = 1; act_dims[1] = 1; act_dims[2] = 2048;
    return DVSG_OK;
  }
  for (int b0 = 0; b0 < B; b0 += 16) {
    const int bc = std::min(16, B - b0);
    float *pa = ws.dpart0, *pb = ws.dpart1;
    DVSG_RUN(launch_dense(ws.pool_part + (size_t)b0 * kPoolSplits * 2048, kPoolSplits, nullptr, inv_hw, 0,
                          net->dense_w[0], pa, bc, 2048, 2048, s));
    DVSG_RUN(launch_dense(pa, kDenseSplits, net->dense_b[0], 1.0f, 1, net->dense_w[1], pb, bc, 2048, 1024, s));
    DVSG_RUN(launch_dense(pb, kDenseSplits, net->dense_b[1], 1.0f, 1, net->dense_w[2], pa, bc, 1024, 512, s));
    DVSG_RUN(launch_dense(pa, kDenseSplits, net->dense_b[2], 1.0f, 1, net->dense_w[3], pb, bc, 512, 50, s));
    DVSG_RUN(launch_dense_finalize(pb, kDenseSplits, 1.0f, net->dense_b[3], F_t + (size_t)b0 * 50, bc, 50, s));
  }
  return DVSG_OK;
#undef DVSG_TAP
#undef DVSG_RUN
}

int forward(const dvsg_locnet *net, int prec, const float *patches, int B, int H, int W, float *F_t, int stop_stage,
            float *act_out, size_t act_out_bytes, int *act_dims, void *workspace, size_t workspace_bytes,
            hipStream_t s) {
  const Conv1Src src{patches, nullptr, 0};
  return forward(net, prec, src, kSrcWindow, B, H, W, F_t, stop_stage, act_out, act_out_bytes, act_dims, workspace,
                 workspace_bytes, s);
}

int stabilize(const dvsg_locnet *net, int prec, const float *patches_t, const float *u_t, const float *mask, int B, int H,
              int W, float *s_t_pred, float *F_t, float *x_s, float *y_s, void *workspace, size_t workspace_bytes,
              void *stream) {
  DVSG_REQUIRE(net && patches_t && u_t && s_t_pred && workspace, "dvsg_stabilize: NULL pointer");
  DVSG_REQUIRE(B > 0 && B <= 65535, "dvsg_stabilize: B=%d out of range", B);
  DVSG_REQUIRE(prec == kF32 || prec == kF16 || prec == kF32S || prec == kF32X, "dvsg_stabilize: unknown precision %d", prec);
  DVSG_REQUIRE(!mask || net->c_in == 21, "dvsg_stabilize_masked: the mask covers the 18 history channels of a 7-frame window");
  const Workspace ws = plan(static_cast<char *>(workspace), B, H, W);
  if (ws.total > workspace_bytes)
    return fail(DVSG_ERR_WORKSPACE, "dvsg_stabilize: workspace %zu bytes < required %zu", workspace_bytes, ws.total);
  float *F = F_t ? F_t : ws.Ft;
  Conv1Src src{patches_t, nullptr, 0};
  src.mask = mask;
  if (int rc = forward(net, prec, src, kSrcWindow, B, H, W, F, -1, nullptr, 0, nullptr, workspace, workspace_bytes,
                       as_stream(stream)))
    return rc;
  MarkerRange mr("dvsg/tps");
  if (int rc = tps_apply_impl(net->winv, net->v_src, F, 1, B, 25, ws.T, stream)) return rc;
  return tps_warp_impl(u_t, net->v_src, 0, ws.T, B, H, W, 3, 25, H, W, s_t_pred, x_s, y_s, stream);
}

int stabilize_ring(const dvsg_locnet *net, int prec, const void *pool, int pool_is_u8, int n_pool, const int32_t *table,
                   const float *mask, int B, int H, int W, float *s_t_pred, float *F_t, float *x_s, float *y_s, void *workspace,
                   size_t workspace_bytes, void *stream) {
  DVSG_REQUIRE(net && pool && table && s_t_pred && workspace, "dvsg_stabilize_ring: NULL pointer");
  DVSG_REQUIRE(B > 0 && B <= 65535 && n_pool > 0, "dvsg_stabilize_ring: B=%d n_pool=%d out of range", B, n_pool);
  DVSG_REQUIRE(prec == kF32 || prec == kF16 || prec == kF32S || prec == kF32X, "dvsg_stabilize_ring: unknown precision %d", prec);
  DVSG_REQUIRE(net->c_in == 21, "dvsg_stabilize_ring: the ring holds RGB frames, 7 per window");
  const Workspace ws = plan(static_cast<char *>(workspace), B, H, W);
  if (ws.total > workspace_bytes)
    return fail(DVSG_ERR_WORKSPACE, "dvsg_stabilize_ring: workspace %zu bytes < required %zu", workspace_bytes, ws.total);
  float *F = F_t ? F_t : ws.Ft;
  Conv1Src src{pool, table, n_pool};
  src.mask = mask;
  if (int rc = forward(net, prec, src, pool_is_u8 ? kSrcRingU8 : kSrcRingF32, B, H, W, F, -1, nullptr, 0, nullptr, workspace,
                       workspace_bytes, as_stream(stream)))
    return rc;
  MarkerRange mr("dvsg/tps");
  if (int rc = tps_apply_impl(net->winv, net->v_src, F, 1, B, 25, ws.T, stream)) return rc;
  return tps_warp_ring_impl(pool, pool_is_u8, n_pool, table + 6, 7, net->v_src, 0, ws.T, B, H, W, 25, s_t_pred, x_s, y_s,
                            stream);
}

int conv_gemm_op(int prec, int wsplit, const void *x, const void *wt, const float *bias, const void *res, void *y, int B,
                 int H, int W, int Cin, int Cout, int ksize, int stride, int relu, int res_stride, void *scratch,
                 size_t scratch_bytes, void *stream) {
  DVSG_REQUIRE(x && wt && bias && y, "dvsg_conv_gemm: NULL pointer");
  DVSG_REQUIRE(!scratch || ((uintptr_t)scratch & 255) == 0, "dvsg_conv_gemm: scratch must be 256-byte aligned");
  DVSG_REQUIRE(B > 0 && H > 0 && W > 0 && stride >= 1 && res_stride >= 1, "dvsg_conv_gemm: bad shape");
  ConvGemm p;
  p.prec = prec;
  p.wsplit = wsplit == 1;
  p.x3 = wsplit == 2;
  p.x = x; p.wt = wt; p.bias = bias; p.res = res; p.y = y;
  p.B = B; p.H = H; p.W = W; p.Cin = Cin; p.Cout = Cout;
  p.Ho = (H - 1) / stride + 1; p.Wo = (W - 1) / stride + 1;
  p.ksize = ksize; p.stride = stride; p.pad = ksize == 3 ? 1 : 0;
  p.res_H = (p.Ho - 1) * res_stride + 1; p.res_W = (p.Wo - 1) * res_stride + 1;
  p.res_stride = res_stride;
  p.relu = relu;
  const size_t cbytes = align256((size_t)kSplitKMaxTiles * sizeof(int));
  if (scratch && scratch_bytes > cbytes) {
    if (int rc = launch_zero_tickets(static_cast<int *>(scratch), cbytes / sizeof(int), as_stream(stream))) return rc;
    p.splitk_counters = static_cast<int *>(scratch);
    p.splitk_scratch = static_cast<char *>(scratch) + cbytes;
    p.splitk_scratch_bytes = std::min(scratch_bytes - cbytes, align256(kSplitKSlabBytes));
  }
  if (prec == kF16 && Cin % 64 == 0 && Cout % (wsplit ? 64 : 128) == 0 && (ksize == 1 || ksize == 3) && scratch) {
    const int rows = wsplit ? 2 * Cout : Cout;
    const size_t need = align256(wide16_packed_bytes(rows, Cin, ksize));
    const size_t base = cbytes + align256(kSplitKSlabBytes);
    if (scratch_bytes >= base + 3 * need) {
      char *pk = static_cast<char *>(scratch) + base;
      if (int rc = launch_pack_wide16(wt, pk, rows, Cin, ksize, 0, as_stream(stream))) return rc;
      p.wt_packed = pk;
      if (ksize == 1) {
        p.wt_packed_a = pk;
      } else {
        if (int rc = launch_pack_wide16(wt, pk + need, rows, Cin, ksize, 1, as_stream(stream))) return rc;
        if (int rc = launch_pack_wide16(wt, pk + 2 * need, rows, Cin, ksize, 2, as_stream(stream))) return rc;
        p.wt_packed_a = pk + need;
        p.wt_packed_h = pk + 2 * need;
      }
    }
  }
  return launch_conv_gemm(p, as_stream(stream));
}

}
}

extern "C" {

int dvsg_locnet_create(int n_arrays, const char *const *names, const float *const *host_data, const int *ndims,
                       const int64_t *dims, dvsg_locnet_t **out) {
  DVSG_REQUIRE(names && host_data && ndims && dims && out && n_arrays > 0, "dvsg_locnet_create: bad arguments");
  *out = nullptr;
// ... 98 lines not shown
    rc = tps_inverse_columns(net->v_src, 25, static_cast<double *>(w), static_cast<float *>(scratch), nullptr);
    (void)hipFree(scratch);
    if (rc) return bail(rc);
    net->winv = static_cast<double *>(w);
  }
  *out = net;
  return DVSG_OK;
}

int dvsg_locnet_destroy(dvsg_locnet_t *net) {
  if (!net) return DVSG_OK;
  for (void *p : net->allocs) (void)hipFree(p);
  delete net;
  return DVSG_OK;
}

int dvsg_locnet_in_channels(const dvsg_locnet_t *net) { return net ? net->c_in : 0; }

int dvsg_locnet_workspace_bytes(const dvsg_locnet_t *net, int B, int H, int W, size_t *bytes) {
  DVSG_REQUIRE(net && bytes, "dvsg_locnet_workspace_bytes: NULL pointer");
  DVSG_REQUIRE(B > 0 && H > 0 && W > 0, "dvsg_locnet_workspace_bytes: bad shape B=%d H=%d W=%d", B, H, W);
  *bytes = plan(nullptr, B, H, W).total;
  return DVSG_OK;
}

int dvsg_locnet_forward_f32(const dvsg_locnet_t *net, const float *patches, int B, int H, int W, float *F_t,
                            void *workspace, size_t workspace_bytes, void *stream) {
  DVSG_REQUIRE(F_t, "dvsg_locnet_forward_f32: NULL F_t");
  return forward(net, kF32, patches, B, H, W, F_t, -1, nullptr, 0, nullptr, workspace, workspace_bytes,
                 as_stream(stream));
}

int dvsg_locnet_forward_f16(const dvsg_locnet_t *net, const float *patches, int B, int H, int W, float *F_t,
                            void *workspace, size_t workspace_bytes, void *stream) {
  DVSG_REQUIRE(F_t, "dvsg_locnet_forward_f16: NULL F_t");
  return forward(net, kF16, patches, B, H, W, F_t, -1, nullptr, 0, nullptr, workspace, workspace_bytes,
                 as_stream(stream));
}

int dvsg_locnet_forward_f32s(const dvsg_locnet_t *net, const float *patches, int B, int H, int W, float *F_t,
                             void *workspace, size_t workspace_bytes, void *stream) {
  DVSG_REQUIRE(F_t, "dvsg_locnet_forward_f32s: NULL F_t");
  return forward(net, kF32S, patches, B, H, W, F_t, -1, nullptr, 0, nullptr, workspace, workspace_bytes,
                 as_stream(stream));
}

int dvsg_locnet_forward_f32x3(const dvsg_locnet_t *net, const float *patches, int B, int H, int W, float *F_t,
                              void *workspace, size_t workspace_bytes, void *stream) {
  DVSG_REQUIRE(F_t, "dvsg_locnet_forward_f32x3: NULL F_t");
  return forward(net, kF32X, patches, B, H, W, F_t, -1, nullptr, 0, nullptr, workspace, workspace_bytes,
                 as_stream(stream));
}

int dvsg_locnet_forward_tap_f32x3(const dvsg_locnet_t *net, const float *patches, int B, int H, int W, int stage,
                                  float *act_out, size_t act_out_bytes, int *act_dims_host, void *workspace,
                                  size_t workspace_bytes, void *stream) {
  DVSG_REQUIRE(act_out && act_dims_host, "dvsg_locnet_forward_tap_f32x3: NULL pointer");
  DVSG_REQUIRE(stage >= 0 && stage <= 18, "dvsg_locnet_forward_tap_f32x3: stage %d outside [0,18]", stage);
  return forward(net, kF32X, patches, B, H, W, nullptr, stage, act_out, act_out_bytes, act_dims_host, workspace,
                 workspace_bytes, as_stream(stream));
}

int dvsg_locnet_forward_tap_f32s(const dvsg_locnet_t *net, const float *patches, int B, int H, int W, int stage,
                                 float *act_out, size_t act_out_bytes, int *act_dims_host, void *workspace,
                                 size_t workspace_bytes, void *stream) {
  DVSG_REQUIRE(act_out && act_dims_host, "dvsg_locnet_forward_tap_f32s: NULL pointer");
  DVSG_REQUIRE(stage >= 0 && stage <= 18, "dvsg_locnet_forward_tap_f32s: stage %d outside [0,18]", stage);
  return forward(net, kF32S, patches, B, H, W, nullptr, stage, act_out, act_out_bytes, act_dims_host, workspace,
                 workspace_bytes, as_stream(stream));
}

int dvsg_locnet_forward_tap_f32(const dvsg_locnet_t *net, const float *patches, int B, int H, int W, int stage,
                                float *act_out, size_t act_out_bytes, int *act_dims_host, void *workspace,
                                size_t workspace_bytes, void *stream) {
  DVSG_REQUIRE(act_out && act_dims_host, "dvsg_locnet_forward_tap_f32: NULL pointer");
  DVSG_REQUIRE(stage >= 0 && stage <= 18, "dvsg_locnet_forward_tap_f32: stage %d outside [0,18]", stage);
  return forward(net, kF32, patches, B, H, W, nullptr, stage, act_out, act_out_bytes, act_dims_host, workspace,
                 workspace_bytes, as_stream(stream));
}

int dvsg_locnet_forward_tap_f16(const dvsg_locnet_t *net, const float *patches, int B, int H, int W, int stage,
                                float *act_out, size_t act_out_bytes, int *act_dims_host, void *workspace,
                                size_t workspace_bytes, void *stream) {
  DVSG_REQUIRE(act_out && act_dims_host, "dvsg_locnet_forward_tap_f16: NULL pointer");
  DVSG_REQUIRE(stage >= 0 && stage <= 18, "dvsg_locnet_forward_tap_f16: stage %d outside [0,18]", stage);
  return forward(net, kF16, patches, B, H, W, nullptr, stage, act_out, act_out_bytes, act_dims_host, workspace,
                 workspace_bytes, as_stream(stream));
}

int dvsg_conv_gemm_f32(const float *x, const float *wt, const float *bias, const float *res, float *y, int B, int H,
                       int W, int Cin, int Cout, int ksize, int stride, int relu, int res_stride, void *scratch,
                       size_t scratch_bytes, void *stream) {
  return conv_gemm_op(kF32, 0, x, wt, bias, res, y, B, H, W, Cin, Cout, ksize, stride, relu, res_stride, scratch,
                      scratch_bytes, stream);
}

int dvsg_conv_gemm_f16(const void *x, const void *wt, const float *bias, const void *res, void *y, int B, int H,
                       int W, int Cin, int Cout, int ksize, int stride, int relu, int res_stride, void *scratch,
                       size_t scratch_bytes, void *stream) {
  return conv_gemm_op(kF16, 0, x, wt, bias, res, y, B, H, W, Cin, Cout, ksize, stride, relu, res_stride, scratch,
                      scratch_bytes, stream);
}

int dvsg_conv_gemm_f32s(const void *x, const void *wt_pieces, const float *bias, const void *res, void *y, int B, int H,
                        int W, int Cin, int Cout, int ksize, int stride, int relu, int res_stride, void *scratch,
                        size_t scratch_bytes, void *stream) {
  return conv_gemm_op(kF32, 1, x, wt_pieces, bias, res, y, B, H, W, Cin, Cout, ksize, stride, relu, res_stride, scratch,
                      scratch_bytes, stream);
}

int dvsg_conv_gemm_f32x3(const float *x, const void *wt_packed, const float *bias, const float *res, float *y, int B, int H,
                         int W, int Cin, int Cout, int ksize, int stride, int relu, int res_stride, void *scratch,
                         size_t scratch_bytes, void *stream) {
  return conv_gemm_op(kF32, 2, x, wt_packed, bias, res, y, B, H, W, Cin, Cout, ksize, stride, relu, res_stride, scratch,
                      scratch_bytes, stream);
}

int dvsg_pack_weights_f32x3(const float *wt, void *wt_packed, int Cout, int K, void *stream) {
  return launch_pack_x3(wt, wt_packed, Cout, K, as_stream(stream));
}

int dvsg_f32_to_pieces(const float *x, void *y, size_t n, void *stream) {
  DVSG_REQUIRE(x && y, "dvsg_f32_to_pieces: NULL pointer");
  return launch_f32_to_p(x, y, n, as_stream(stream));
}

int dvsg_pieces_to_f32(const void *x, float *y, size_t n, void *stream) {
  DVSG_REQUIRE(x && y, "dvsg_pieces_to_f32: NULL pointer");
  return launch_p_to_f32(x, y, n, as_stream(stream));
}

int dvsg_conv_gemm_f16s(const void *x, const void *wt_split, const float *bias, const void *res, void *y, int B, int H,
                        int W, int Cin, int Cout, int ksize, int stride, int relu, int res_stride, void *scratch,
                        size_t scratch_bytes, void *stream) {
  return conv_gemm_op(kF16, 1, x, wt_split, bias, res, y, B, H, W, Cin, Cout, ksize, stride, relu, res_stride, scratch,
                      scratch_bytes, stream);
}

int dvsg_conv3x3_1x1_f32(const float *x, const float *wt2, const float *bias2, const float *wt3, const float *bias3,
                         const float *res, float *y, int B, int H, int W, int Cin, int Cout, int stride, int res_stride,
                         void *stream) {
  DVSG_REQUIRE(x && wt2 && bias2 && wt3 && bias3 && res && y, "dvsg_conv3x3_1x1_f32: NULL pointer");
  DVSG_REQUIRE(B > 0 && H > 0 && W > 0 && (stride == 1 || stride == 2) && res_stride >= 1,
               "dvsg_conv3x3_1x1_f32: bad shape B=%d H=%d W=%d stride=%d res_stride=%d", B, H, W, stride, res_stride);
  ConvFused f;
  f.x = x; f.wt2 = wt2; f.bias2 = bias2; f.wt3 = wt3; f.bias3 = bias3; f.res = res; f.y = y;
  f.B = B; f.H = H; f.W = W; f.Cin = Cin; f.Cout = Cout;
  f.Ho = (H - 1) / stride + 1; f.Wo = (W - 1) / stride + 1;
  f.stride = stride;
  f.res_H = (f.Ho - 1) * res_stride + 1; f.res_W = (f.Wo - 1) * res_stride + 1; f.res_stride = res_stride;
  return launch_conv3x3_1x1(f, as_stream(stream));
}

int dvsg_conv3x3_1x1_f32x3(const float *x, const void *wt2_packed, const float *bias2, const void *wt3_packed, const float *bias3,
                           const float *res, float *y, int B, int H, int W, int Cin, int Cout, int stride, int res_stride,
                           void *stream) {
  DVSG_REQUIRE(x && wt2_packed && bias2 && wt3_packed && bias3 && res && y, "dvsg_conv3x3_1x1_f32x3: NULL pointer");
  DVSG_REQUIRE(B > 0 && H > 0 && W > 0 && (stride == 1 || stride == 2) && res_stride >= 1,
               "dvsg_conv3x3_1x1_f32x3: bad shape B=%d H=%d W=%d stride=%d res_stride=%d", B, H, W, stride, res_stride);
  ConvFused f;
  f.x = x; f.wt2 = static_cast<const float *>(wt2_packed); f.bias2 = bias2; f.wt3 = static_cast<const float *>(wt3_packed);
  f.bias3 = bias3; f.res = res; f.y = y;
  f.B = B; f.H = H; f.W = W; f.Cin = Cin; f.Cout = Cout;
  f.Ho = (H - 1) / stride + 1; f.Wo = (W - 1) / stride + 1;
  f.stride = stride;
  f.res_H = (f.Ho - 1) * res_stride + 1; f.res_W = (f.Wo - 1) * res_stride + 1; f.res_stride = res_stride;
  f.x3 = 1;
  return launch_conv3x3_1x1(f, as_stream(stream));
}

int dvsg_debug_set_option(const char *name, int value) {
  DVSG_REQUIRE(name, "dvsg_debug_set_option: NULL name");
  if (std::strcmp(name, "conv_variant") == 0) {
    set_conv_variant(value);
    return DVSG_OK;
  }
  if (std::strcmp(name, "wide16_min_tiles") == 0) {
    set_wide16_min_tiles(value);
    return DVSG_OK;
  }
  if (std::strcmp(name, "fused_hreuse") == 0) {
    set_fused_hreuse(value);
    return DVSG_OK;
  }
  if (std::strcmp(name, "wide16_hreuse") == 0) {
    set_wide16_hreuse(value);
    return DVSG_OK;
  }
  if (std::strcmp(name, "wide16_arows") == 0) {
    set_wide16_arows(value);
    return DVSG_OK;
  }
  if (std::strcmp(name, "wide16_packed") == 0) {
    set_wide16_packed(value);
    return DVSG_OK;
  }
  if (std::strcmp(name, "flow_tiled") == 0) {
    set_flow_tiled(value);
    return DVSG_OK;
  }
  if (std::strcmp(name, "flow_rounds") == 0) {
    set_flow_rounds(value);
    return DVSG_OK;
  }
  if (std::strcmp(name, "warp_xcd") == 0) {
    set_warp_xcd(value);
    return DVSG_OK;
  }
  if (std::strcmp(name, "conv1_variant") == 0) {
    set_conv1_variant(value);
    return DVSG_OK;
  }
  if (std::strcmp(name, "fuse_conv") == 0) {
    set_fuse_conv(value);
    return DVSG_OK;
  }
  if (std::strcmp(name, "concat_sc") == 0) {
    g_concat_sc = value != 0;
    return DVSG_OK;
  }
  if (std::strcmp(name, "x3_conv1") == 0) {
    g_x3_conv1 = value;
    return DVSG_OK;
  }
  if (std::strcmp(name, "x3_fuse") == 0) {
    g_x3_fuse = value;
    return DVSG_OK;
  }
  if (std::strcmp(name, "fuse_shortcut") == 0) {
    g_fuse_shortcut = value != 0;
    return DVSG_OK;
  }
  if (std::strcmp(name, "f16_split") == 0) {
    g_f16_split = value != 0;
    return DVSG_OK;
  }
  if (std::strcmp(name, "f16_pair_mask") == 0) {
    g_f16_pair_mask = value & 0xFFFF;
    return DVSG_OK;
  }
  return fail(DVSG_ERR_INVALID_ARG, "dvsg_debug_set_option: unknown option %s", name);
}

static int calibrate_f16(dvsg_locnet *net, const float *patches, int B, int H, int W, int mode, void *workspace,
                         size_t workspace_bytes, hipStream_t s) {
  std::vector<double> mu((size_t)48 * 2048, 1.0);
  if (mode == 2) {
    void *sums = nullptr, *part = nullptr, *F = nullptr;
    hipError_t e = hipMalloc(&sums, 48 * 2048 * sizeof(double));
    if (e == hipSuccess) e = hipMalloc(&part, (size_t)kCalibBlocks * 2048 * sizeof(float));
    if (e == hipSuccess) e = hipMalloc(&F, (size_t)B * 50 * sizeof(float));
    if (e == hipSuccess) e = hipMemsetAsync(sums, 0, 48 * 2048 * sizeof(double), s);
    int rc = e == hipSuccess ? DVSG_OK : fail(DVSG_ERR_HIP, "calibration: %s", hipGetErrorString(e));
    if (rc == DVSG_OK) {
      g_calib.sums = static_cast<double *>(sums);
      g_calib.part = static_cast<float *>(part);
      for (double &r : g_calib.rows) r = 0;
      const int fuse_was = get_fuse_conv();
      set_fuse_conv(0);
      g_calib.on = true;
      rc = forward(net, kF32, patches, B, H, W, static_cast<float *>(F), -1, nullptr, 0, nullptr, workspace, workspace_bytes, s);
      g_calib.on = false;
      set_fuse_conv(fuse_was);
      if (rc == DVSG_OK && hipMemcpyAsync(mu.data(), sums, mu.size() * sizeof(double), hipMemcpyDeviceToHost, s) != hipSuccess)
        rc = fail(DVSG_ERR_HIP, "copy of the calibration sums failed");
      if (rc == DVSG_OK && hipStreamSynchronize(s) != hipSuccess) rc = fail(DVSG_ERR_HIP, "calibration pass failed");
    }
    (void)hipFree(sums);
    (void)hipFree(part);
    (void)hipFree(F);
    if (rc) return rc;
    for (int slot = 0; slot < 48; ++slot)
      for (int c = 0; c < 2048; ++c) mu[(size_t)slot * 2048 + c] = g_calib.rows[slot] > 0 ? mu[(size_t)slot * 2048 + c] / g_calib.rows[slot] : 1.0;
  }
  auto f16_bits = [](_Float16 v) { unsigned short b; std::memcpy(&b, &v, 2); return b; };
  auto f16_from = [](unsigned short b) { _Float16 v; std::memcpy(&v, &b, 2); return v; };
  auto neighbour = [&](_Float16 q, bool up) -> _Float16 {
    unsigned short b = f16_bits(q);
    if ((b & 0x7fff) == 0) return f16_from(up ? 0x0001 : 0x8001);
    const bool neg = (b & 0x8000) != 0;
    b = (unsigned short)((up != neg) ? b + 1 : b - 1);
    return f16_from(b);
  };
  auto redo = [&](ConvLayer &L, const double *m) -> int {
    const int K = L.ksize * L.ksize * L.cin;
    std::vector<float> wt((size_t)L.cout * K);
    DVSG_HIP(hipMemcpy(wt.data(), L.wt, wt.size() * sizeof(float), hipMemcpyDeviceToHost));
    std::vector<_Float16> q16(wt.size());
    for (int n = 0; n < L.cout; ++n) {
      double E = 0.0;
      for (int k = 0; k < K; ++k) {
        const float w32 = wt[(size_t)n * K + k];
        const _Float16 q0 = (_Float16)w32;
        _Float16 q = q0;
        if (mode != 0 && (float)q0 != w32) {
          const _Float16 other = neighbour(q0, (float)q0 < w32);
          const double mk = m[k % L.cin];
          const double e0 = E + ((double)(float)q0 - w32) * mk, e1 = E + ((double)(float)other - w32) * mk;
          const bool take = std::fabs(e1) < std::fabs(e0) && std::isfinite((float)other);
          q = take ? other : q0;
          E = take ? e1 : e0;
        }
        q16[(size_t)n * K + k] = q;
      }
    }
    DVSG_HIP(hipMemcpy(L.wt16, q16.data(), q16.size() * sizeof(_Float16), hipMemcpyHostToDevice));
    return pack_plain(net, &L);
  };
  int ui = 0;
  for (Unit &u : net->units) {
    const double *mx = mu.data() + (size_t)(3 * ui) * 2048;
    if (u.has_shortcut) if (int rc = redo(u.shortcut, mx)) return rc;
    if (int rc = redo(u.c1, mx)) return rc;
    if (int rc = redo(u.c2, mx + 2048)) return rc;
    if (int rc = redo(u.c3, mx + 2 * 2048)) return rc;
    ++ui;
  }
  return DVSG_OK;
}

int dvsg_locnet_calibrate_f16(dvsg_locnet_t *net, const float *patches, int B, int H, int W, void *workspace,
                              size_t workspace_bytes, void *stream) {
  DVSG_REQUIRE(net && workspace, "dvsg_locnet_calibrate_f16: NULL pointer");
  if (!patches) {
    net->f16_pair_mask = 0xFFFF;
    return calibrate_f16(net, nullptr, 0, 0, 0, 0, workspace, workspace_bytes, as_stream(stream));
  }
  DVSG_REQUIRE(B > 0 && H > 0 && W > 0, "dvsg_locnet_calibrate_f16: bad shape B=%d H=%d W=%d", B, H, W);
  if (int rc = calibrate_f16(net, patches, B, H, W, 2, workspace, workspace_bytes, as_stream(stream))) return rc;
  net->f16_pair_mask = 0x1111;
  return DVSG_OK;
}

int dvsg_debug_calibrate_f16_weights(dvsg_locnet_t *net, const float *patches, int B, int H, int W, int mode, void *workspace,
                                     size_t workspace_bytes, void *stream) {
  DVSG_REQUIRE(net && patches && workspace && mode >= 0 && mode <= 2, "dvsg_debug_calibrate_f16_weights: bad arguments");
  return calibrate_f16(net, patches, B, H, W, mode, workspace, workspace_bytes, as_stream(stream));
}

int dvsg_stabilize_f32(const dvsg_locnet_t *net, const float *patches_t, const float *u_t, int B, int H, int W,
                       float *s_t_pred, float *F_t, float *x_s, float *y_s, void *workspace, size_t workspace_bytes,
                       void *stream) {
  return stabilize(net, kF32, patches_t, u_t, nullptr, B, H, W, s_t_pred, F_t, x_s, y_s, workspace, workspace_bytes, stream);
}

int dvsg_stabilize_f32s(const dvsg_locnet_t *net, const float *patches_t, const float *u_t, int B, int H, int W,
                        float *s_t_pred, float *F_t, float *x_s, float *y_s, void *workspace, size_t workspace_bytes,
                        void *stream) {
  return stabilize(net, kF32S, patches_t, u_t, nullptr, B, H, W, s_t_pred, F_t, x_s, y_s, workspace, workspace_bytes, stream);
}

int dvsg_stabilize_f16(const dvsg_locnet_t *net, const float *patches_t, const float *u_t, int B, int H, int W,
                       float *s_t_pred, float *F_t, float *x_s, float *y_s, void *workspace, size_t workspace_bytes,
                       void *stream) {
  return stabilize(net, kF16, patches_t, u_t, nullptr, B, H, W, s_t_pred, F_t, x_s, y_s, workspace, workspace_bytes, stream);
}

int dvsg_stabilize_f32x3(const dvsg_locnet_t *net, const float *patches_t, const float *u_t, int B, int H, int W,
                         float *s_t_pred, float *F_t, float *x_s, float *y_s, void *workspace, size_t workspace_bytes,
                         void *stream) {
  return stabilize(net, kF32X, patches_t, u_t, nullptr, B, H, W, s_t_pred, F_t, x_s, y_s, workspace, workspace_bytes, stream);
}

static int ring_precision(int precision) {
  return precision == DVSG_PRECISION_F32 ? kF32 : precision == DVSG_PRECISION_F16 ? kF16 : precision == DVSG_PRECISION_F32S ? kF32S
         : precision == DVSG_PRECISION_F32X3 ? kF32X : -1;
}
// ... 71 lines not shown
```

### include/dvsg_amd.h

```cpp
#ifndef DVSG_AMD_H
#define DVSG_AMD_H

#include <stddef.h>
#include <stdint.h>

#ifdef __cplusplus
extern "C" {
#endif

#define DVSG_ABI_VERSION 1

typedef enum dvsg_status {
  DVSG_OK = 0,
  DVSG_ERR_INVALID_ARG = -1,
  DVSG_ERR_HIP = -2,
  DVSG_ERR_WORKSPACE = -3,
  DVSG_ERR_WEIGHTS = -4,
  DVSG_ERR_UNSUPPORTED = -5
} dvsg_status;

int dvsg_abi_version(void);
const char *dvsg_last_error_string(void);
const char *dvsg_target_arch(void);


int dvsg_tps_solve_f32(const float *coord, const float *rhs, int rhs_is_vector, int B, int P,
                       float *T, void *stream);

int dvsg_tps_solve_checked_f32(const float *coord, const float *rhs, int rhs_is_vector, int B, int P,
                               float *T, int *n_singular, void *stream);

int dvsg_tps_warp_f32(const float *U, const float *coord, const float *T, int B, int H, int W,
                      int C, int P, int out_h, int out_w, float *out, float *x_s, float *y_s,
                      void *stream);

int dvsg_flow_warp_f32(const float *im, const float *flow, int B, int H, int W, int C,
                       float *out, void *stream);


int dvsg_stn_sample_f32(const float *im, const float *x_s, const float *y_s, int B, int H,
                        int W, int C, int out_h, int out_w, float *out, void *stream);

int dvsg_grid_affine_f32(const float *theta, const float *im, int B, int H, int W, int C,
                         int out_h, int out_w, float *out, float *x_s, float *y_s, void *stream);

int dvsg_grid_projective_f32(const float *theta, const float *im, int B, int H, int W, int C,
                             int out_h, int out_w, float *out, float *x_s, float *y_s,
                             void *stream);

int dvsg_elastic_constants_f32(int grid_size, float *source_points_host, float *L_inv_host);

int dvsg_grid_elastic_f32(const float *theta_abs, const float *L_inv, const float *source_points,
                          int n, const float *im, int B, int H, int W, int C, int out_h,
                          int out_w, float *out, float *x_s, float *y_s, void *stream);

int dvsg_scale_rgb_f32(const float *rgb, int B, int H, int W, int C, float *out, void *stream);

typedef struct dvsg_locnet dvsg_locnet_t;

int dvsg_locnet_create(int n_arrays, const char *const *names, const float *const *host_data,
                       const int *ndims, const int64_t *dims, dvsg_locnet_t **net);
int dvsg_locnet_destroy(dvsg_locnet_t *net);
int dvsg_locnet_in_channels(const dvsg_locnet_t *net);
int dvsg_locnet_workspace_bytes(const dvsg_locnet_t *net, int B, int H, int W, size_t *bytes);

int dvsg_locnet_forward_f32(const dvsg_locnet_t *net, const float *patches, int B, int H, int W,
                            float *F_t, void *workspace, size_t workspace_bytes, void *stream);

int dvsg_locnet_forward_tap_f32(const dvsg_locnet_t *net, const float *patches, int B, int H,
                                int W, int stage, float *act_out, size_t act_out_bytes,
                                int *act_dims_host, void *workspace, size_t workspace_bytes,
                                void *stream);

int dvsg_stabilize_f32(const dvsg_locnet_t *net, const float *patches_t, const float *u_t, int B,
                       int H, int W, float *s_t_pred, float *F_t, float *x_s, float *y_s,
                       void *workspace, size_t workspace_bytes, void *stream);

int dvsg_conv_gemm_f32(const float *x, const float *wt, const float *bias, const float *res, float *y,
                       int B, int H, int W, int Cin, int Cout, int ksize, int stride, int relu,
                       int res_stride, void *scratch, size_t scratch_bytes, void *stream);

int dvsg_locnet_forward_f16(const dvsg_locnet_t *net, const float *patches, int B, int H, int W,
                            float *F_t, void *workspace, size_t workspace_bytes, void *stream);
int dvsg_locnet_forward_tap_f16(const dvsg_locnet_t *net, const float *patches, int B, int H,
                                int W, int stage, float *act_out, size_t act_out_bytes,
                                int *act_dims_host, void *workspace, size_t workspace_bytes,
                                void *stream);
int dvsg_stabilize_f16(const dvsg_locnet_t *net, const float *patches_t, const float *u_t, int B,
                       int H, int W, float *s_t_pred, float *F_t, float *x_s, float *y_s,
                       void *workspace, size_t workspace_bytes, void *stream);
int dvsg_locnet_calibrate_f16(dvsg_locnet_t *net, const float *patches, int B, int H, int W, void *workspace,
                              size_t workspace_bytes, void *stream);
int dvsg_locnet_forward_f32s(const dvsg_locnet_t *net, const float *patches, int B, int H, int W,
                             float *F_t, void *workspace, size_t workspace_bytes, void *stream);
int dvsg_locnet_forward_tap_f32s(const dvsg_locnet_t *net, const float *patches, int B, int H,
                                 int W, int stage, float *act_out, size_t act_out_bytes,
                                 int *act_dims_host, void *workspace, size_t workspace_bytes,
                                 void *stream);
int dvsg_stabilize_f32s(const dvsg_locnet_t *net, const float *patches_t, const float *u_t, int B,
                        int H, int W, float *s_t_pred, float *F_t, float *x_s, float *y_s,
                        void *workspace, size_t workspace_bytes, void *stream);
int dvsg_conv_gemm_f32s(const void *x, const void *wt_pieces, const float *bias, const void *res,
                        void *y, int B, int H, int W, int Cin, int Cout, int ksize, int stride,
                        int relu, int res_stride, void *scratch, size_t scratch_bytes, void *stream);
int dvsg_f32_to_pieces(const float *x, void *y, size_t n, void *stream);
int dvsg_pieces_to_f32(const void *x, float *y, size_t n, void *stream);

int dvsg_locnet_forward_f32x3(const dvsg_locnet_t *net, const float *patches, int B, int H, int W,
                              float *F_t, void *workspace, size_t workspace_bytes, void *stream);
int dvsg_locnet_forward_tap_f32x3(const dvsg_locnet_t *net, const float *patches, int B, int H,
                                  int W, int stage, float *act_out, size_t act_out_bytes,
                                  int *act_dims_host, void *workspace, size_t workspace_bytes,
                                  void *stream);
int dvsg_stabilize_f32x3(const dvsg_locnet_t *net, const float *patches_t, const float *u_t, int B,
                         int H, int W, float *s_t_pred, float *F_t, float *x_s, float *y_s,
                         void *workspace, size_t workspace_bytes, void *stream);
int dvsg_conv_gemm_f32x3(const float *x, const void *wt_packed, const float *bias, const float *res,
                         float *y, int B, int H, int W, int Cin, int Cout, int ksize, int stride,
                         int relu, int res_stride, void *scratch, size_t scratch_bytes, void *stream);
int dvsg_pack_weights_f32x3(const float *wt, void *wt_packed, int Cout, int K, void *stream);
int dvsg_conv3x3_1x1_f32x3(const float *x, const void *wt2_packed, const float *bias2, const void *wt3_packed,
                           const float *bias3, const float *res, float *y, int B, int H, int W, int Cin, int Cout,
                           int stride, int res_stride, void *stream);

int dvsg_conv_gemm_f16(const void *x, const void *wt, const float *bias, const void *res, void *y,
                       int B, int H, int W, int Cin, int Cout, int ksize, int stride, int relu,
                       int res_stride, void *scratch, size_t scratch_bytes, void *stream);
int dvsg_conv_gemm_f16s(const void *x, const void *wt_split, const float *bias, const void *res, void *y,
                        int B, int H, int W, int Cin, int Cout, int ksize, int stride, int relu,
                        int res_stride, void *scratch, size_t scratch_bytes, void *stream);

int dvsg_frames_u8_to_f32(const uint8_t *src, size_t n_pixels, int channel_flip, float *dst, void *stream);
int dvsg_frames_resize_u8_f32(const uint8_t *src, int n, int src_H, int src_W, int channel_flip, float *dst,
                              int dst_H, int dst_W, uint8_t *u8_dst, int u8_W, int u8_x0, void *stream);
int dvsg_window_gather_f32(const float *pool, int n_pool, int H, int W, const int32_t *idx, int B, int S,
                           float *patches, void *stream);

#define DVSG_PRECISION_F32 0
#define DVSG_PRECISION_F16 1
#define DVSG_PRECISION_F32S 2
#define DVSG_PRECISION_F32X3 3
int dvsg_stabilize_ring_f32(const dvsg_locnet_t *net, int precision, const float *pool, int n_pool,
                            const int32_t *table, int B, int H, int W, float *s_t_pred, float *F_t, float *x_s,
                            float *y_s, void *workspace, size_t workspace_bytes, void *stream);
int dvsg_stabilize_ring_u8(const dvsg_locnet_t *net, int precision, const uint8_t *pool, int n_pool,
                           const int32_t *table, int B, int H, int W, float *s_t_pred, float *F_t, float *x_s,
                           float *y_s, void *workspace, size_t workspace_bytes, void *stream);
int dvsg_locnet_forward_ring(const dvsg_locnet_t *net, int precision, const void *pool, int pool_is_u8, int n_pool,
                             const int32_t *table, int B, int H, int W, int stage, float *out, size_t out_bytes,
                             int *act_dims_host, void *workspace, size_t workspace_bytes, void *stream);
int dvsg_random_mask_plane_f32(const float *theta, int B, int H, int W, float *mask, void *stream);
int dvsg_stabilize_masked_f32(const dvsg_locnet_t *net, int precision, const float *patches_t, const float *u_t,
                              const float *mask, int B, int H, int W, float *s_t_pred, float *F_t, float *x_s, float *y_s,
                              void *workspace, size_t workspace_bytes, void *stream);
int dvsg_stabilize_ring_masked_f32(const dvsg_locnet_t *net, int precision, const float *pool, int n_pool,
                                   const int32_t *table, const float *mask, int B, int H, int W, float *s_t_pred, float *F_t,
                                   float *x_s, float *y_s, void *workspace, size_t workspace_bytes, void *stream);
int dvsg_stabilize_ring_masked_u8(const dvsg_locnet_t *net, int precision, const uint8_t *pool, int n_pool,
                                  const int32_t *table, const float *mask, int B, int H, int W, float *s_t_pred, float *F_t,
                                  float *x_s, float *y_s, void *workspace, size_t workspace_bytes, void *stream);
int dvsg_locnet_forward_masked(const dvsg_locnet_t *net, int precision, const void *src, int src_kind, int n_pool,
                               const int32_t *table, const float *mask, int B, int H, int W, int stage, float *out,
                               size_t out_bytes, int *act_dims_host, void *workspace, size_t workspace_bytes, void *stream);
int dvsg_frames_f32_to_u8(const float *src, int n, int H, int W, int channel_flip, uint8_t *dst, int dst_W,
                          int dst_x0, void *stream);
int dvsg_frames_f64_to_u8(const double *src, int n, int H, int W, int channel_flip, uint8_t *dst, int dst_W,
                          int dst_x0, void *stream);

int dvsg_conv3x3_1x1_f32(const float *x, const float *wt2, const float *bias2, const float *wt3, const float *bias3,
                         const float *res, float *y, int B, int H, int W, int Cin, int Cout, int stride, int res_stride,
                         void *stream);

int dvsg_debug_set_option(const char *name, int value);
int dvsg_debug_calibrate_f16_weights(dvsg_locnet_t *net, const float *patches, int B, int H, int W, int mode, void *workspace,
                                     size_t workspace_bytes, void *stream);

int dvsg_markers_enabled(void);
int dvsg_prof_begin(int kernel_class);
int dvsg_prof_end(double *total_ms, int *launches, double *flops, double *bytes);

#ifdef __cplusplus
}
#endif
#endif
```

Measured before the change: 744.2.

## Fuse conv1 with max pool and add fused 3x3+1x1 kernel for 128-wide middle

Adds a pooled epilogue to the conv1 kernel that applies bias+ReLU and writes 3x3/2 max-pool results directly via atomic max on a zero-initialised buffer, skipping the full-resolution conv1 activation write and the separate maxpool pass. Also adds fused conv3x3+1x1 kernels for blocks whose middle width is 128 (two tile variants), so block-2 bottlenecks in f32 can use the fused path with strided input and residual layouts. This cuts memory traffic and launches, at the cost of atomic contention, an extra zeroing pass, and large LDS usage that limits occupancy.

```diff
diff --git a/coupe/dvsg_amd/_lib.py b/coupe/dvsg_amd/_lib.py
--- a/coupe/dvsg_amd/_lib.py
+++ b/coupe/dvsg_amd/_lib.py
@@ -51,6 +51,7 @@
     "dvsg_conv_gemm_f16s": [_vp, _vp, _vp, _vp, _vp, _i, _i, _i, _i, _i, _i, _i, _i, _i, _vp, ctypes.c_size_t, _vp],
     "dvsg_conv_gemm_f32": [_vp, _vp, _vp, _vp, _vp, _i, _i, _i, _i, _i, _i, _i, _i, _i, _vp, ctypes.c_size_t, _vp],
     "dvsg_conv3x3_1x1_f32": [_vp, _vp, _vp, _vp, _vp, _vp, _vp, _i, _i, _i, _i, _i, _i, _i, _vp],
+    "dvsg_conv3x3_1x1_c128_f32": [_vp, _i, _vp, _vp, _vp, _vp, _vp, _i, _vp, _i, _i, _i, _i, _i, _i, _i, _vp],
     "dvsg_frames_u8_to_f32": [_vp, ctypes.c_size_t, _i, _vp, _vp],
     "dvsg_frames_resize_u8_f32": [_vp, _i, _i, _i, _i, _vp, _i, _i, _vp, _i, _i, _vp],
     "dvsg_window_gather_f32": [_vp, _i, _i, _i, _vp, _i, _i, _vp, _vp],
diff --git a/coupe/dvsg_amd/csrc/cnn_kernels.h b/coupe/dvsg_amd/csrc/cnn_kernels.h
--- a/coupe/dvsg_amd/csrc/cnn_kernels.h
+++ b/coupe/dvsg_amd/csrc/cnn_kernels.h
@@ -58,11 +58,15 @@
   int pieces = 0;
   int f16 = 0;
   int x3 = 0;
+  int cmid = 64;
+  int ldx = 0, res_ld = 0;
 };
 int launch_conv3x3_1x1_x3(const ConvFused &p, hipStream_t s);
 bool conv_fusable(int prec, int Cin, int Cmid, int Cout, int ksize);
 int launch_conv3x3_1x1(const ConvFused &p, hipStream_t s);
 void set_fuse_conv(int v);
+void set_fuse_block2(int v);
+void set_c128_tile(int v);
 int get_fuse_conv();
 void set_fused_hreuse(int v);
 void set_conv_variant(int v);
@@ -85,6 +89,9 @@
 int launch_conv1(int out_prec, const Conv1Src &src, int src_kind, const float *wt1, const void *wt1h, const void *wt1s,
                  const void *wt1x, const float *bias, void *y, int B, int H, int W, int Ho, int Wo, hipStream_t s);
 
+int launch_conv1_maxpool(const Conv1Src &src, int src_kind, const float *wt1, const float *bias, float *y, int B, int H, int W,
+                         int Ho, int Wo, int Hp, int Wp, int pad_top, int pad_left, hipStream_t s);
+
 int launch_maxpool(int prec, const void *x, void *y, int B, int H, int W, int C, int Ho, int Wo, int pad_top,
                    int pad_left, hipStream_t s);
 
diff --git a/coupe/dvsg_amd/csrc/conv1_pool.hip b/coupe/dvsg_amd/csrc/conv1_pool.hip
--- a/coupe/dvsg_amd/csrc/conv1_pool.hip
+++ b/coupe/dvsg_amd/csrc/conv1_pool.hip
@@ -1,3 +1,4 @@
+#include <algorithm>
 #include <cstdint>
 #include <type_traits>
 
@@ -322,10 +323,14 @@
 #define C1_STAMP() __builtin_amdgcn_s_memtime()
 #endif
 
-template <int NW, typename TO, int SRC>
+struct Conv1PoolDst {
+  int Hp, Wp, pad_top, pad_left;
+};
+
+template <int NW, typename TO, int SRC, bool POOL = false>
 __global__ __launch_bounds__(64 * NW) __attribute__((amdgpu_waves_per_eu(NW / 2, NW / 2)))
 void conv1_kernel(const Conv1Src src, const float *__restrict__ wt1, const float *__restrict__ bias,
-                  TO *__restrict__ y, int H, int W, int Ho, int Wo, int wtiles) {
+                  TO *__restrict__ y, int H, int W, int Ho, int Wo, int wtiles, Conv1PoolDst pd = {}) {
   constexpr int NT = 64 * NW;
   constexpr int MI = 4 / (NW / 2);
   constexpr int IN4 = (C1_SEG_PAD / 4 + NT - 1) / NT;
@@ -460,6 +465,33 @@
   __syncthreads();
   const int col4 = tid & 15, row0 = tid >> 4;
   const float4 b4 = *reinterpret_cast<const float4 *>(bias + 4 * col4);
+  if constexpr (POOL) {
+    static_assert(std::is_same<TO, float>::value, "the pooled epilogue is float32");
+    const int pr_lo = std::max((ho + pd.pad_top - 1) >> 1, 0), pr_hi = std::min((ho + pd.pad_top) >> 1, pd.Hp - 1);
+    const int wend = std::min(wo0 + C1_TILE, Wo);
+    const int pc_lo = std::max((wo0 + pd.pad_left - 1) >> 1, 0), pc_hi = std::min((wend - 1 + pd.pad_left) >> 1, pd.Wp - 1);
+    const int items = (pc_hi - pc_lo + 1) * 16;
+    for (int it = tid; it < items; it += NT) {
+      const int pc = pc_lo + (it >> 4);
+      const int wa = std::max(2 * pc - pd.pad_left, wo0), wb = std::min(2 * pc - pd.pad_left + 2, wend - 1);
+      float4 m = make_float4(0.f, 0.f, 0.f, 0.f);
+      for (int wc = wa; wc <= wb; ++wc) {
+        const float4 v = *reinterpret_cast<const float4 *>(Cs + (wc - wo0) * C1_LDC + 4 * col4);
+        m.x = fmaxf(m.x, fmaxf(v.x + b4.x, 0.f));
+        m.y = fmaxf(m.y, fmaxf(v.y + b4.y, 0.f));
+        m.z = fmaxf(m.z, fmaxf(v.z + b4.z, 0.f));
+        m.w = fmaxf(m.w, fmaxf(v.w + b4.w, 0.f));
+      }
+      const unsigned q[4] = {__float_as_uint(m.x + 0.f), __float_as_uint(m.y + 0.f), __float_as_uint(m.z + 0.f),
+                             __float_as_uint(m.w + 0.f)};
+      for (int pr = pr_lo; pr <= pr_hi; ++pr) {
+        unsigned *dst = reinterpret_cast<unsigned *>(y) + (((size_t)b * pd.Hp + pr) * pd.Wp + pc) * 64 + 4 * col4;
+#pragma unroll
+        for (int j = 0; j < 4; ++j) __hip_atomic_fetch_max(dst + j, q[j], __ATOMIC_RELAXED, __HIP_MEMORY_SCOPE_AGENT);
+      }
+    }
+    return;
+  }
   TO *yrow = y + (((size_t)b * Ho + ho) * Wo + wo0) * 64 + 4 * col4;
 #pragma unroll 4
   for (int row = row0; row < C1_TILE; row += NT / 16) {
@@ -1611,6 +1643,46 @@
   return check_launch("conv1_kernel");
 }
 
+namespace {
+__global__ __launch_bounds__(256) void zero4_kernel(float4 *__restrict__ y, size_t n4) {
+  for (size_t i = (size_t)blockIdx.x * 256 + threadIdx.x; i < n4; i += (size_t)gridDim.x * 256) y[i] = make_float4(0.f, 0.f, 0.f, 0.f);
+}
+}
+
+int launch_conv1_maxpool(const Conv1Src &src, int src_kind, const float *wt1, const float *bias, float *y, int B, int H, int W,
+                         int Ho, int Wo, int Hp, int Wp, int pad_top, int pad_left, hipStream_t s) {
+  const int wtiles = ceil_div(Wo, C1_TILE);
+  const long blocks = (long)wtiles * Ho * B;
+  DVSG_REQUIRE(blocks > 0 && blocks < (1L << 31), "conv1: grid of %ld workgroups out of range", blocks);
+  DVSG_REQUIRE((long)W * kConv1Cin < (1L << 31), "conv1: input row too long");
+  DVSG_REQUIRE(src_kind == kSrcWindow || (src.table && src.n_pool > 0), "conv1: a frame ring needs its index table");
+  DVSG_REQUIRE(Hp == (Ho + 1) / 2 && Wp == (Wo + 1) / 2 && (pad_top == 0 || pad_top == 1) && (pad_left == 0 || pad_left == 1),
+               "conv1 + max pool: %dx%d -> %dx%d with pads %d, %d is not a 3x3/2 SAME pool", Ho, Wo, Hp, Wp, pad_top, pad_left);
+  const size_t n4 = (size_t)B * Hp * Wp * 16;
+  {
+    ProfScope prof(kClsMaxpool, s, 0.0, 16.0 * (double)n4);
+    hipLaunchKernelGGL(zero4_kernel, dim3((unsigned)std::min<size_t>((n4 + 255) / 256, 16384)), dim3(256), 0, s,
+                       reinterpret_cast<float4 *>(y), n4);
+    if (int rc = check_launch("zero4_kernel")) return rc;
+  }
+  const double in_bytes = src_kind == kSrcRingU8 ? 1.0 : 4.0;
+  ProfScope prof(kClsConv1, s, 2.0 * (double)B * Ho * Wo * 64 * 49 * kConv1Cin,
+                 in_bytes * (double)B * H * W * kConv1Cin + 4.0 * (double)B * Hp * Wp * 64);
+  const dim3 grid((unsigned)blocks);
+  const bool aligned = W % 4 == 0 && reinterpret_cast<uintptr_t>(src.base) % (src_kind == kSrcRingU8 ? 4 : 16) == 0;
+  const int SRC = 2 * src_kind + (aligned ? 1 : 0) + (src.mask ? 8 : 0);
+  const Conv1PoolDst pd{Hp, Wp, pad_top, pad_left};
+#define DVSG_C1P(S) \
+  case S: hipLaunchKernelGGL((conv1_kernel<4, float, S, true>), grid, dim3(256), 0, s, src, wt1, bias, y, H, W, Ho, Wo, wtiles, pd); break
+  switch (SRC) {
+    DVSG_C1P(0); DVSG_C1P(1); DVSG_C1P(2); DVSG_C1P(3); DVSG_C1P(4); DVSG_C1P(5);
+    DVSG_C1P(8); DVSG_C1P(9); DVSG_C1P(10); DVSG_C1P(11); DVSG_C1P(12); DVSG_C1P(13);
+    default: return fail(DVSG_ERR_INVALID_ARG, "conv1: source kind %d", SRC);
+  }
+#undef DVSG_C1P
+  return check_launch("conv1_kernel (pooled)");
+}
+
 #ifdef DVSG_STAMPS
 extern "C" int dvsg_debug_read_conv1_stamps(void *host, size_t bytes) {
   return hipMemcpyFromSymbol(host, HIP_SYMBOL(g_c1_stamps), bytes) == hipSuccess ? 0 : -3;
diff --git a/coupe/dvsg_amd/csrc/conv_fused.hip b/coupe/dvsg_amd/csrc/conv_fused.hip
--- a/coupe/dvsg_amd/csrc/conv_fused.hip
+++ b/coupe/dvsg_amd/csrc/conv_fused.hip
@@ -337,6 +337,391 @@
   }
 }
 
+struct ConvFused128Dev {
+  const float *x, *wt2, *bias2, *wt3, *bias3, *res;
+  float *y;
+  int H, W, Cin, ldx, Ho, Wo, Cout, res_ld;
+  int stride;
+  int res_H, res_W, res_stride;
+  int M, mtiles;
+};
+
+template <int RES>
+__global__ __launch_bounds__(512) __attribute__((amdgpu_waves_per_eu(2, 2)))
+void conv3x3_1x1_c128_kernel(ConvFused128Dev p) {
+  constexpr int NW = 8;
+  constexpr int AG = 2;
+  constexpr int SB = 32768;
+  constexpr int W3B = 65536;
+  __shared__ __attribute__((aligned(16))) char lds[98304];
+  const int tid = threadIdx.x;
+  const int lane = tid & 63, wave = tid >> 6;
+  const int wm = wave >> 1, wn = wave & 1;
+  const int r = lane & 31, h = lane >> 5;
+  const int lrow8 = lane >> 3, lpos = lane & 7;
+  const int sw = (r >> 1) & 7;
+  const int K1 = 9 * p.Cin;
+  const int KT = K1 / 32;
+
+  typedef const __attribute__((address_space(1))) void *gptr_t;
+  typedef __attribute__((address_space(3))) void *lptr_t;
+
+  const int m0 = xcd_remap(blockIdx.x, p.mtiles) * BM;
+
+  long a_off[AG];
+  unsigned a_mask[AG];
+  const float *wsrc[2];
+#pragma unroll
+  for (int i = 0; i < AG; ++i) {
+    const int row = 8 * (wave + NW * i) + lrow8;
+    const int chunk = lpos ^ ((row >> 1) & 7);
+    const int m = m0 + row;
+    const int mm = m < p.M ? m : 0;
+    const int wo = mm % p.Wo;
+    const int t = mm / p.Wo;
+    const int ho = t % p.Ho;
+    const int b = t / p.Ho;
+    const int hi0 = ho * p.stride - 1, wi0 = wo * p.stride - 1;
+    a_off[i] = (((long)b * p.H + hi0) * p.W + wi0) * p.ldx + 4 * chunk;
+    unsigned mk = 0;
+    if (m < p.M) {
+#pragma unroll
+      for (int q = 0; q < 3; ++q) {
+        if (hi0 + q >= 0 && hi0 + q < p.H) mk |= 1u << q;
+        if (wi0 + q >= 0 && wi0 + q < p.W) mk |= 16u << q;
+      }
+    }
+    a_mask[i] = mk;
+    wsrc[i] = p.wt2 + (size_t)row * K1 + 4 * chunk;
+  }
+  int s_kh = 0, s_kw = 0, s_c0 = 0;
+  auto issue_stage = [&](int buf) __attribute__((always_inline)) {
+    const float *xa = p.x + ((long)s_kh * p.W + s_kw) * p.ldx + s_c0;
+    const int wk = (s_kh * 3 + s_kw) * p.Cin + s_c0;
+    char *As = lds + buf * SB, *Bs = As + 16384;
+#pragma unroll
+    for (int i = 0; i < AG; ++i) {
+      const bool ok = ((a_mask[i] >> s_kh) & (a_mask[i] >> (4 + s_kw)) & 1u) != 0;
+      const void *src = ok ? static_cast<const void *>(xa + a_off[i]) : static_cast<const void *>(&g_zero16f);
+      __builtin_amdgcn_global_load_lds((gptr_t)src, (lptr_t)(As + 8 * (wave + NW * i) * ROWB), 16, 0, 0);
+    }
+#pragma unroll
+    for (int i = 0; i < 2; ++i)
+      __builtin_amdgcn_global_load_lds((gptr_t)(wsrc[i] + wk), (lptr_t)(Bs + 8 * (wave + NW * i) * ROWB), 16, 0, 0);
+    if (++s_kw == 3) {
+      s_kw = 0;
+      if (++s_kh == 3) {
+        s_kh = 0;
+        s_c0 += 32;
+      }
+    }
+  };
+  floatx16 acc1[2];
+#pragma unroll
+  for (int ni = 0; ni < 2; ++ni)
+#pragma unroll
+    for (int q = 0; q < 16; ++q) acc1[ni][q] = 0.f;
+  auto w3_issue = [&](int half, int s2) __attribute__((always_inline)) {
+#pragma unroll
+    for (int i = 0; i < 2; ++i) {
+      const int row = 8 * (wave + NW * i) + lrow8;
+      const float *src = p.wt3 + (size_t)(128 * half + row) * 128 + 32 * s2 + 4 * (lpos ^ ((row >> 1) & 7));
+      __builtin_amdgcn_global_load_lds((gptr_t)src, (lptr_t)(lds + W3B + (s2 & 1) * 16384 + 8 * (wave + NW * i) * ROWB), 16, 0, 0);
+    }
+  };
+  const int rot = (3 - (KT - 1) % 3) % 3;
+  int bi = rot, bc = rot;
+  issue_stage(bi); bi = bi == 2 ? 0 : bi + 1;
+  issue_stage(bi); bi = bi == 2 ? 0 : bi + 1;
+  for (int kt = 0; kt < KT; ++kt) {
+    if (kt + 1 < KT) asm volatile("s_waitcnt vmcnt(4)" ::: "memory");
+    else asm volatile("s_waitcnt vmcnt(0)" ::: "memory");
+    __builtin_amdgcn_s_barrier();
+    asm volatile("" ::: "memory");
+    if (kt + 2 < KT) {
+      issue_stage(bi); bi = bi == 2 ? 0 : bi + 1;
+    } else if (kt + 1 == KT) {
+      w3_issue(0, 0);
+    }
+    __builtin_amdgcn_sched_barrier(0);
+    stage_mma<false, 2>(lds + bc * SB + (wm * 32 + r) * ROWB, lds + bc * SB + 16384 + (wn * 64 + r) * ROWB, sw, h, acc1);
+    bc = bc == 2 ? 0 : bc + 1;
+    __builtin_amdgcn_sched_barrier(0);
+  }
+
+  __syncthreads();
+#pragma unroll
+  for (int ni = 0; ni < 2; ++ni) {
+    const float bmid = p.bias2[64 * wn + 32 * ni + r];
+#pragma unroll
+    for (int q = 0; q < 16; ++q) {
+      const int R = wm * 32 + (q & 3) + 8 * (q >> 2) + 4 * h;
+      const float v = fmaxf(acc1[ni][q] + bmid, 0.f);
+      *reinterpret_cast<float *>(lds + ((2 * wn + ni) * BM + R) * ROWB + 16 * ((r >> 2) ^ ((R >> 1) & 7)) + 4 * (r & 3)) = v;
+    }
+  }
+  w3_issue(0, 1);
+
+  float *Cs = reinterpret_cast<float *>(lds + W3B);
+  const int col4 = tid & 31, row0 = tid >> 5;
+  auto lds_barrier = [&]() __attribute__((always_inline)) {
+    asm volatile("s_waitcnt lgkmcnt(0)" ::: "memory");
+    __builtin_amdgcn_s_barrier();
+    asm volatile("" ::: "memory");
+  };
+  const int nhalves = p.Cout / 128;
+  for (int half = 0; half < nhalves; ++half) {
+    floatx16 acc2[2];
+#pragma unroll
+    for (int ni = 0; ni < 2; ++ni)
+#pragma unroll
+      for (int q = 0; q < 16; ++q) acc2[ni][q] = 0.f;
+#pragma unroll
+    for (int s2 = 0; s2 < 4; ++s2) {
+      if (s2 < 3) asm volatile("s_waitcnt vmcnt(2) lgkmcnt(0)" ::: "memory");
+      else asm volatile("s_waitcnt vmcnt(0) lgkmcnt(0)" ::: "memory");
+      __builtin_amdgcn_s_barrier();
+      asm volatile("" ::: "memory");
+      stage_mma<false, 2>(lds + (s2 * BM + wm * 32 + r) * ROWB, lds + W3B + (s2 & 1) * 16384 + (wn * 64 + r) * ROWB, sw, h, acc2);
+      if (s2 < 2) {
+        lds_barrier();
+        w3_issue(half, s2 + 2);
+      }
+    }
+    const int n = 128 * half + 4 * col4;
+    const float4 bias4 = *reinterpret_cast<const float4 *>(p.bias3 + n);
+#pragma unroll
+    for (int rho = 0; rho < 2; ++rho) {
+      float4 rv[4];
+#pragma unroll
+      for (int i = 0; i < 4; ++i) {
+        const int mr = m0 + 64 * rho + row0 + 16 * i;
+        const int m = mr < p.M ? mr : p.M - 1;
+        size_t roff;
+        if (RES == 1) {
+          roff = (size_t)m * p.res_ld + n;
+        } else {
+          const int wo = m % p.Wo;
+          const int t = m / p.Wo;
+          const int ho = t % p.Ho;
+          const int b = t / p.Ho;
+          roff = (((size_t)b * p.res_H + (size_t)ho * p.res_stride) * p.res_W + (size_t)wo * p.res_stride) * p.res_ld + n;
+        }
+        rv[i] = load4(p.res + roff);
+      }
+      lds_barrier();
+      if ((wm >> 1) == rho) {
+#pragma unroll
+        for (int ni = 0; ni < 2; ++ni)
+#pragma unroll
+          for (int q = 0; q < 16; ++q)
+            Cs[((wm & 1) * 32 + (q & 3) + 8 * (q >> 2) + 4 * h) * 128 + wn * 64 + ni * 32 + r] = acc2[ni][q];
+      }
+      lds_barrier();
+#pragma unroll
+      for (int i = 0; i < 4; ++i) {
+        const int row = row0 + 16 * i;
+        const int m = m0 + 64 * rho + row;
+        if (m < p.M) {
+          float4 v = *reinterpret_cast<const float4 *>(Cs + row * 128 + 4 * col4);
+          v.x = fmaxf(v.x + bias4.x + rv[i].x, 0.f);
+          v.y = fmaxf(v.y + bias4.y + rv[i].y, 0.f);
+          v.z = fmaxf(v.z + bias4.z + rv[i].z, 0.f);
+          v.w = fmaxf(v.w + bias4.w + rv[i].w, 0.f);
+          store4(p.y + (size_t)m * p.Cout + n, v);
+        }
+      }
+    }
+    if (half + 1 < nhalves) {
+      lds_barrier();
+      w3_issue(half + 1, 0);
+      w3_issue(half + 1, 1);
+    }
+  }
+}
+
+template <int RES>
+__global__ __launch_bounds__(512) __attribute__((amdgpu_waves_per_eu(4, 4)))
+void conv3x3_1x1_c128h_kernel(ConvFused128Dev p) {
+  constexpr int NW = 8;
+  constexpr int TM = 64;
+  constexpr int SB = 24576;
+  __shared__ __attribute__((aligned(16))) char lds[65536];
+  const int tid = threadIdx.x;
+  const int lane = tid & 63, wave = tid >> 6;
+  const int wm = wave >> 2, wn = wave & 3;
+  const int r = lane & 31, h = lane >> 5;
+  const int lrow8 = lane >> 3, lpos = lane & 7;
+  const int sw = (r >> 1) & 7;
+  const int K1 = 9 * p.Cin;
+  const int KT = K1 / 32;
+
+  typedef const __attribute__((address_space(1))) void *gptr_t;
+  typedef __attribute__((address_space(3))) void *lptr_t;
+
+  const int m0 = xcd_remap(blockIdx.x, p.mtiles) * TM;
+
+  long a_off;
+  unsigned a_mask;
+  const float *wsrc[2];
+  {
+    const int row = 8 * wave + lrow8;
+    const int chunk = lpos ^ ((row >> 1) & 7);
+    const int m = m0 + row;
+    const int mm = m < p.M ? m : 0;
+    const int wo = mm % p.Wo;
+    const int t = mm / p.Wo;
+    const int ho = t % p.Ho;
+    const int b = t / p.Ho;
+    const int hi0 = ho * p.stride - 1, wi0 = wo * p.stride - 1;
+    a_off = (((long)b * p.H + hi0) * p.W + wi0) * p.ldx + 4 * chunk;
+    unsigned mk = 0;
+    if (m < p.M) {
+#pragma unroll
+      for (int q = 0; q < 3; ++q) {
+        if (hi0 + q >= 0 && hi0 + q < p.H) mk |= 1u << q;
+        if (wi0 + q >= 0 && wi0 + q < p.W) mk |= 16u << q;
+      }
+    }
+    a_mask = mk;
+  }
+#pragma unroll
+  for (int i = 0; i < 2; ++i) {
+    const int row = 8 * (wave + NW * i) + lrow8;
+    wsrc[i] = p.wt2 + (size_t)row * K1 + 4 * (lpos ^ ((row >> 1) & 7));
+  }
+  int s_kh = 0, s_kw = 0, s_c0 = 0;
+  auto issue_stage = [&](int buf) __attribute__((always_inline)) {
+    const float *xa = p.x + ((long)s_kh * p.W + s_kw) * p.ldx + s_c0;
+    const int wk = (s_kh * 3 + s_kw) * p.Cin + s_c0;
+    char *As = lds + buf * SB, *Bs = As + 8192;
+    const bool ok = ((a_mask >> s_kh) & (a_mask >> (4 + s_kw)) & 1u) != 0;
+    const void *src = ok ? static_cast<const void *>(xa + a_off) : static_cast<const void *>(&g_zero16f);
+    __builtin_amdgcn_global_load_lds((gptr_t)src, (lptr_t)(As + 8 * wave * ROWB), 16, 0, 0);
+#pragma unroll
+    for (int i = 0; i < 2; ++i)
+      __builtin_amdgcn_global_load_lds((gptr_t)(wsrc[i] + wk), (lptr_t)(Bs + 8 * (wave + NW * i) * ROWB), 16, 0, 0);
+    if (++s_kw == 3) {
+      s_kw = 0;
+      if (++s_kh == 3) {
+        s_kh = 0;
+        s_c0 += 32;
+      }
+    }
+  };
+  floatx16 acc1v[1];
+#pragma unroll
+  for (int q = 0; q < 16; ++q) acc1v[0][q] = 0.f;
+  auto compute_stage = [&](int buf) __attribute__((always_inline)) {
+    stage_mma<false, 1>(lds + buf * SB + (wm * 32 + r) * ROWB, lds + buf * SB + 8192 + (wn * 32 + r) * ROWB, sw, h, acc1v);
+  };
+  auto w3_dst = [](int s2) { return (s2 & 1) ? 32768 : 49152; };
+  auto w3_issue = [&](int half, int s2) __attribute__((always_inline)) {
+#pragma unroll
+    for (int i = 0; i < 2; ++i) {
+      const int row = 8 * (wave + NW * i) + lrow8;
+      const float *src = p.wt3 + (size_t)(128 * half + row) * 128 + 32 * s2 + 4 * (lpos ^ ((row >> 1) & 7));
+      __builtin_amdgcn_global_load_lds((gptr_t)src, (lptr_t)(lds + w3_dst(s2) + 8 * (wave + NW * i) * ROWB), 16, 0, 0);
+    }
+  };
+  issue_stage(0);
+  issue_stage(1);
+  asm volatile("s_waitcnt vmcnt(3)" ::: "memory");
+  __builtin_amdgcn_s_barrier();
+  asm volatile("" ::: "memory");
+  __builtin_amdgcn_sched_barrier(0);
+  compute_stage(0);
+  __builtin_amdgcn_sched_barrier(0);
+  for (int kt = 1; kt < KT - 1; ++kt) {
+    __syncthreads();
+    issue_stage((kt + 1) & 1);
+    __builtin_amdgcn_sched_barrier(0);
+    compute_stage(kt & 1);
+    __builtin_amdgcn_sched_barrier(0);
+  }
+  __syncthreads();
+  w3_issue(0, 0);
+  __builtin_amdgcn_sched_barrier(0);
+  compute_stage((KT - 1) & 1);
+
+  const float bmid = p.bias2[32 * wn + r];
+  __syncthreads();
+#pragma unroll
+  for (int q = 0; q < 16; ++q) {
+    const int R = wm * 32 + (q & 3) + 8 * (q >> 2) + 4 * h;
+    const float v = fmaxf(acc1v[0][q] + bmid, 0.f);
+    *reinterpret_cast<float *>(lds + (wn * TM + R) * ROWB + 16 * ((r >> 2) ^ ((R >> 1) & 7)) + 4 * (r & 3)) = v;
+  }
+  w3_issue(0, 1);
+
+  float *Cs = reinterpret_cast<float *>(lds + 32768);
+  const int col4 = tid & 31, row0 = tid >> 5;
+  auto lds_barrier = [&]() __attribute__((always_inline)) {
+    asm volatile("s_waitcnt lgkmcnt(0)" ::: "memory");
+    __builtin_amdgcn_s_barrier();
+    asm volatile("" ::: "memory");
+  };
+  const int nhalves = p.Cout / 128;
+  for (int half = 0; half < nhalves; ++half) {
+    floatx16 acc2[1];
+#pragma unroll
+    for (int q = 0; q < 16; ++q) acc2[0][q] = 0.f;
+    const int n = 128 * half + 4 * col4;
+    float4 rv[4];
+#pragma unroll
+    for (int i = 0; i < 4; ++i) {
+      const int mr = m0 + row0 + 16 * i;
+      const int m = mr < p.M ? mr : p.M - 1;
+      size_t roff;
+      if (RES == 1) {
+        roff = (size_t)m * p.res_ld + n;
+      } else {
+        const int wo = m % p.Wo;
+        const int t = m / p.Wo;
+        const int ho = t % p.Ho;
+        const int b = t / p.Ho;
+        roff = (((size_t)b * p.res_H + (size_t)ho * p.res_stride) * p.res_W + (size_t)wo * p.res_stride) * p.res_ld + n;
+      }
+      rv[i] = load4(p.res + roff);
+    }
+#pragma unroll
+    for (int s2 = 0; s2 < 4; ++s2) {
+      if (s2 < 3) asm volatile("s_waitcnt vmcnt(2) lgkmcnt(0)" ::: "memory");
+      else asm volatile("s_waitcnt vmcnt(0) lgkmcnt(0)" ::: "memory");
+      __builtin_amdgcn_s_barrier();
+      asm volatile("" ::: "memory");
+      stage_mma<false, 1>(lds + (s2 * TM + wm * 32 + r) * ROWB, lds + w3_dst(s2) + (wn * 32 + r) * ROWB, sw, h, acc2);
+      if (s2 < 2) {
+        lds_barrier();
+        w3_issue(half, s2 + 2);
+      }
+    }
+    const float4 bias4 = *reinterpret_cast<const float4 *>(p.bias3 + n);
+    lds_barrier();
+#pragma unroll
+    for (int q = 0; q < 16; ++q) Cs[(wm * 32 + (q & 3) + 8 * (q >> 2) + 4 * h) * 128 + wn * 32 + r] = acc2[0][q];
+    lds_barrier();
+#pragma unroll
+    for (int i = 0; i < 4; ++i) {
+      const int row = row0 + 16 * i;
+      const int m = m0 + row;
+      if (m < p.M) {
+        float4 v = *reinterpret_cast<const float4 *>(Cs + row * 128 + 4 * col4);
+        v.x = fmaxf(v.x + bias4.x + rv[i].x, 0.f);
+        v.y = fmaxf(v.y + bias4.y + rv[i].y, 0.f);
+        v.z = fmaxf(v.z + bias4.z + rv[i].z, 0.f);
+        v.w = fmaxf(v.w + bias4.w + rv[i].w, 0.f);
+        store4(p.y + (size_t)m * p.Cout + n, v);
+      }
+    }
+    if (half + 1 < nhalves) {
+      lds_barrier();
+      w3_issue(half + 1, 0);
+      w3_issue(half + 1, 1);
+    }
+  }
+}
+
 struct ConvFusedF16Dev {
   const _Float16 *x;
   const _Float16 *wt2;
@@ -801,15 +1186,52 @@
 int g_fused_hreuse = 1;
 
 int g_fuse_conv = 1;
+int g_fuse_block2 = 0;
+int g_c128_tile = 64;
 
 }
 
 void set_fuse_conv(int v) { g_fuse_conv = v; }
+void set_fuse_block2(int v) { g_fuse_block2 = v; }
+void set_c128_tile(int v) { g_c128_tile = v == 128 ? 128 : 64; }
 int get_fuse_conv() { return g_fuse_conv; }
 void set_fused_hreuse(int v) { g_fused_hreuse = v; }
 bool conv_fusable(int prec, int Cin, int Cmid, int Cout, int ksize) {
   if (prec == kF16) return g_fuse_conv != 0 && ksize == 3 && Cmid == CMID && Cin % 64 == 0 && Cout % 64 == 0;
+  if (Cmid == 128) return g_fuse_conv != 0 && g_fuse_block2 != 0 && prec == kF32 && ksize == 3 && Cin % 32 == 0 && Cin >= 64 && Cout % 128 == 0;
   return g_fuse_conv != 0 && (prec == kF32 || prec == kF32S) && ksize == 3 && Cmid == CMID && Cin % 32 == 0 && Cin >= 64 && Cout % 128 == 0;
+}
+
+static int launch_conv3x3_1x1_c128(const ConvFused &p, hipStream_t s) {
+  DVSG_REQUIRE(!p.pieces && !p.f16 && !p.x3 && !p.sc_x && p.res, "conv3x3_1x1 (Cmid 128): exact float32 with a residual tensor only");
+  DVSG_REQUIRE(p.Cin % 32 == 0 && p.Cin >= 64 && p.Cout % 128 == 0, "conv3x3_1x1 (Cmid 128): Cin=%d must be a multiple of 32 (>= 64), "
+               "Cout=%d of 128", p.Cin, p.Cout);
+  const int ldx = p.ldx > 0 ? p.ldx : p.Cin, res_ld = p.res_ld > 0 ? p.res_ld : p.Cout;
+  DVSG_REQUIRE(ldx >= p.Cin && ldx % 4 == 0 && res_ld >= p.Cout && res_ld % 4 == 0, "conv3x3_1x1 (Cmid 128): row strides %d, %d", ldx, res_ld);
+  const long M = (long)p.B * p.Ho * p.Wo;
+  DVSG_REQUIRE(M > 0 && M < (1L << 31) - BM, "conv3x3_1x1: M=%ld out of range", M);
+  const int res = p.res_stride == 1 && p.res_H == p.Ho && p.res_W == p.Wo ? 1 : 2;
+  DVSG_REQUIRE(res == 1 || res_ld == p.Cout, "conv3x3_1x1 (Cmid 128): a subsampled residual must be dense");
+  ConvFused128Dev d;
+  d.x = p.x; d.wt2 = p.wt2; d.bias2 = p.bias2; d.wt3 = p.wt3; d.bias3 = p.bias3; d.res = p.res; d.y = p.y;
+  d.H = p.H; d.W = p.W; d.Cin = p.Cin; d.ldx = ldx; d.Ho = p.Ho; d.Wo = p.Wo; d.Cout = p.Cout; d.res_ld = res_ld;
+  d.stride = p.stride;
+  d.res_H = p.res_H; d.res_W = p.res_W; d.res_stride = p.res_stride;
+  d.M = (int)M;
+  d.mtiles = (int)((M + BM - 1) / BM);
+  ProfScope prof(kClsFused, s, 2.0 * (double)M * 128 * (9.0 * p.Cin) + 2.0 * (double)M * p.Cout * 128,
+                 4.0 * ((double)p.B * p.H * p.W * p.Cin + 128.0 * 9 * p.Cin + (double)p.Cout * 128 + 2.0 * (double)M * p.Cout));
+  if (g_c128_tile == 64) {
+    d.mtiles = (int)((M + 63) / 64);
+    const dim3 grid(d.mtiles), block(512);
+    if (res == 1) hipLaunchKernelGGL((conv3x3_1x1_c128h_kernel<1>), grid, block, 0, s, d);
+    else hipLaunchKernelGGL((conv3x3_1x1_c128h_kernel<2>), grid, block, 0, s, d);
+    return check_launch("conv3x3_1x1_c128h_kernel");
+  }
+  const dim3 grid(d.mtiles), block(512);
+  if (res == 1) hipLaunchKernelGGL((conv3x3_1x1_c128_kernel<1>), grid, block, 0, s, d);
+  else hipLaunchKernelGGL((conv3x3_1x1_c128_kernel<2>), grid, block, 0, s, d);
+  return check_launch("conv3x3_1x1_c128_kernel");
 }
 
 static int launch_conv3x3_1x1_f16(const ConvFused &p, hipStream_t s) {
@@ -853,6 +1275,9 @@
 }
 
 int launch_conv3x3_1x1(const ConvFused &p, hipStream_t s) {
+  DVSG_REQUIRE(p.cmid == 64 || p.cmid == 128, "conv3x3_1x1: middle width %d (64 or 128)", p.cmid);
+  if (p.cmid == 128) return launch_conv3x3_1x1_c128(p, s);
+  DVSG_REQUIRE((p.ldx == 0 || p.ldx == p.Cin) && (p.res_ld == 0 || p.res_ld == p.Cout), "conv3x3_1x1 (Cmid 64): dense tensors only");
   if (p.f16) return launch_conv3x3_1x1_f16(p, s);
   if (p.x3) return launch_conv3x3_1x1_x3(p, s);
   DVSG_REQUIRE(p.Cin % 32 == 0 && p.Cin >= 64 && p.Cout % 128 == 0, "conv3x3_1x1: Cin=%d must be a multiple of 32 (>= 64), Cout=%d of 128",
diff --git a/coupe/dvsg_amd/csrc/locnet.hip b/coupe/dvsg_amd/csrc/locnet.hip
--- a/coupe/dvsg_amd/csrc/locnet.hip
+++ b/coupe/dvsg_amd/csrc/locnet.hip
@@ -304,6 +304,7 @@
 int g_x3_conv1 = 1;
 int g_x3_fuse = 3;
 int g_concat_sc = 1;
+int g_pool_conv1 = 1;
 
 struct Workspace {
   char *bufA, *bufB, *bufS, *r1, *r2;
@@ -319,15 +320,16 @@
   size_t big_el = std::max((size_t)d.H1 * d.W1 * 64, (size_t)d.Hp * d.Wp * 64);
   size_t small_el = 0;
   {
-    int h = d.Hp, w = d.Wp;
+    int h = d.Hp, w = d.Wp, depth_in = 64;
     for (const BlockSpec &bs : kBlocks)
       for (int u = 1; u <= bs.units; ++u) {
         const int stride = u == bs.units ? bs.last_stride : 1;
         const int ho = (h - 1) / stride + 1, wo = (w - 1) / stride + 1;
         small_el = std::max(small_el, (size_t)h * w * bs.base);
         big_el = std::max(big_el, (size_t)ho * wo * bs.base * 4);
-        if (u == 1) big_el = std::max(big_el, (size_t)h * w * bs.base * 5);
+        if (u == 1 && depth_in > 64) big_el = std::max(big_el, (size_t)h * w * bs.base * 5);
         h = ho; w = wo;
+        depth_in = 4 * bs.base;
       }
   }
   const size_t big = align256((size_t)B * big_el * sizeof(float));
@@ -462,15 +464,19 @@
 
   DVSG_RUN(launch_zero_tickets(ws.splitk_counters, (size_t)kMaxConvLaunches * kSplitKMaxTiles, s));
   int launch_idx = 0;
-  {
-  MarkerRange mr("dvsg/conv1");
-  DVSG_RUN(launch_conv1(gprec == kF32X && g_x3_conv1 ? kF32X : prec, src, src_kind, net->conv1.wt, net->conv1.wt16, net->conv1.wt32s,
-                        net->conv1.wt3x, net->conv1.bias, ws.bufA, B, H, W, d.H1, d.W1, s));
-  }
-  DVSG_TAP(0, ws.bufA, d.H1, d.W1, 64);
-  {
-  MarkerRange mr("dvsg/pool1");
-  DVSG_RUN(launch_maxpool(prec, ws.bufA, ws.bufB, B, d.H1, d.W1, 64, d.Hp, d.Wp, d.pad_top, d.pad_left, s));
+  if (gprec == kF32 && g_pool_conv1 && stop_stage != 0 && !g_calib.on) {
+    MarkerRange mr("dvsg/conv1");
+    DVSG_RUN(launch_conv1_maxpool(src, src_kind, net->conv1.wt, net->conv1.bias, reinterpret_cast<float *>(ws.bufB), B, H, W, d.H1,
+                                  d.W1, d.Hp, d.Wp, d.pad_top, d.pad_left, s));
+  } else {
+    {
+    MarkerRange mr("dvsg/conv1");
+    DVSG_RUN(launch_conv1(gprec == kF32X && g_x3_conv1 ? kF32X : prec, src, src_kind, net->conv1.wt, net->conv1.wt16, net->conv1.wt32s,
+                          net->conv1.wt3x, net->conv1.bias, ws.bufA, B, H, W, d.H1, d.W1, s));
+    }
+    DVSG_TAP(0, ws.bufA, d.H1, d.W1, 64);
+    MarkerRange mr("dvsg/pool1");
+    DVSG_RUN(launch_maxpool(prec, ws.bufA, ws.bufB, B, d.H1, d.W1, 64, d.Hp, d.Wp, d.pad_top, d.pad_left, s));
   }
   DVSG_TAP(1, ws.bufB, d.Hp, d.Wp, 64);
 
@@ -491,7 +497,7 @@
     DVSG_RUN(calib_record(calib_slot, X, (long)B * h * w, u.c1.cin, s));
     const bool x3_fused = gprec == kF32X && g_x3_fuse == 3;
     const bool x3_unfused = gprec == kF32X && (g_x3_fuse == 0 || (g_x3_fuse == 1 && !u.has_shortcut));
-    const bool fuse23 = !x3_unfused && conv_fusable(prec, u.c2.cin, u.c2.cout, u.c3.cout, u.c2.ksize) &&
+    const bool fuse23 = !x3_unfused && (u.c2.cout == 64 || gprec == kF32) && conv_fusable(prec, u.c2.cin, u.c2.cout, u.c3.cout, u.c2.ksize) &&
                         (prec != kF16 || (f16_pairs(net, u.block, kKindC2) && f16_pairs(net, u.block, kKindC3) &&
                                           (!u.has_shortcut || f16_pairs(net, u.block, kKindSc))));
     const bool fuse_sc = fuse23 && !x3_fused && u.has_shortcut && u.stride == 1 && u.shortcut.cin == 64 && u.shortcut.cout == 256 &&
@@ -526,7 +532,9 @@
       f.pieces = pcs;
       f.f16 = prec == kF16;
       f.x3 = x3_fused;
-      f.x = reinterpret_cast<const float *>(ws.r1); f.wt2 = wts_of(u.c2); f.bias2 = u.c2.bias; f.wt3 = wts_of(u.c3); f.bias3 = u.c3.bias;
+      f.cmid = u.c2.cout;
+      f.ldx = c2_ldx; f.res_ld = res_ld;
+      f.x = static_cast<const float *>(c2_in); f.wt2 = wts_of(u.c2); f.bias2 = u.c2.bias; f.wt3 = wts_of(u.c3); f.bias3 = u.c3.bias;
       f.res = static_cast<const float *>(res); f.y = reinterpret_cast<float *>(Y);
       f.B = B; f.H = h; f.W = w; f.Cin = u.c2.cin; f.Ho = ho; f.Wo = wo; f.Cout = u.c3.cout;
       f.stride = u.c2.stride; f.res_H = res_h; f.res_W = res_w; f.res_stride = res_stride;
@@ -931,6 +939,22 @@
   return launch_conv3x3_1x1(f, as_stream(stream));
 }
 
+int dvsg_conv3x3_1x1_c128_f32(const float *x, int ldx, const float *wt2, const float *bias2, const float *wt3, const float *bias3,
+                              const float *res, int res_ld, float *y, int B, int H, int W, int Cin, int Cout, int stride,
+                              int res_stride, void *stream) {
+  DVSG_REQUIRE(x && wt2 && bias2 && wt3 && bias3 && res && y, "dvsg_conv3x3_1x1_c128_f32: NULL pointer");
+  DVSG_REQUIRE(B > 0 && H > 0 && W > 0 && (stride == 1 || stride == 2) && res_stride >= 1 && ldx >= 0 && res_ld >= 0,
+               "dvsg_conv3x3_1x1_c128_f32: bad shape B=%d H=%d W=%d stride=%d res_stride=%d", B, H, W, stride, res_stride);
+  ConvFused f;
+  f.cmid = 128;
+  f.x = x; f.ldx = ldx; f.wt2 = wt2; f.bias2 = bias2; f.wt3 = wt3; f.bias3 = bias3; f.res = res; f.res_ld = res_ld; f.y = y;
+  f.B = B; f.H = H; f.W = W; f.Cin = Cin; f.Cout = Cout;
+  f.Ho = (H - 1) / stride + 1; f.Wo = (W - 1) / stride + 1;
+  f.stride = stride;
+  f.res_H = (f.Ho - 1) * res_stride + 1; f.res_W = (f.Wo - 1) * res_stride + 1; f.res_stride = res_stride;
+  return launch_conv3x3_1x1(f, as_stream(stream));
+}
+
 int dvsg_conv3x3_1x1_f32x3(const float *x, const void *wt2_packed, const float *bias2, const void *wt3_packed, const float *bias3,
                            const float *res, float *y, int B, int H, int W, int Cin, int Cout, int stride, int res_stride,
                            void *stream) {
@@ -992,6 +1016,18 @@
   }
   if (std::strcmp(name, "fuse_conv") == 0) {
     set_fuse_conv(value);
+    return DVSG_OK;
+  }
+  if (std::strcmp(name, "c128_tile") == 0) {
+    set_c128_tile(value);
+    return DVSG_OK;
+  }
+  if (std::strcmp(name, "fuse_block2") == 0) {
+    set_fuse_block2(value);
+    return DVSG_OK;
+  }
+  if (std::strcmp(name, "pool_conv1") == 0) {
+    g_pool_conv1 = value != 0;
     return DVSG_OK;
   }
   if (std::strcmp(name, "concat_sc") == 0) {
diff --git a/include/dvsg_amd.h b/include/dvsg_amd.h
--- a/include/dvsg_amd.h
+++ b/include/dvsg_amd.h
@@ -171,6 +171,10 @@
                          const float *res, float *y, int B, int H, int W, int Cin, int Cout, int stride, int res_stride,
                          void *stream);
 
+int dvsg_conv3x3_1x1_c128_f32(const float *x, int ldx, const float *wt2, const float *bias2, const float *wt3, const float *bias3,
+                              const float *res, int res_ld, float *y, int B, int H, int W, int Cin, int Cout, int stride,
+                              int res_stride, void *stream);
+
 int dvsg_debug_set_option(const char *name, int value);
 int dvsg_debug_calibrate_f16_weights(dvsg_locnet_t *net, const float *patches, int B, int H, int W, int mode, void *workspace,
                                      size_t workspace_bytes, void *stream);
```

Result: no change. 745.3 (median of 6 runs) (+0.1%).
